# TengdaHan/CoCLR

Measured on AMD Instinct MI355X. Metric: clips/sec (whole node) S3D-InfoNCE seq_len=32 bs=32/GPU, higher is better.
Workload: dtype fp32

## Files before the change

### coclr_amd/_lib.py

```python
import ctypes as C
import os

_HERE = os.path.dirname(os.path.abspath(__file__))
LIB_PATH = os.environ.get("COCLR_LIB_PATH") or os.path.join(_HERE, "libcoclr_hip.so")
ABI_VERSION = 22

i32, i64, f32, f64, vp = C.c_int32, C.c_int64, C.c_float, C.c_double, C.c_void_p


class ConvDesc(C.Structure):
    _fields_ = [(n, i32) for n in (
        "N", "Cin", "Cout", "Ti", "Hi", "Wi", "To", "Ho", "Wo", "kt", "kh", "kw",
        "st", "sh", "sw", "pt", "ph", "pw", "dt", "dh", "dw")] + [
        ("x_nstride", i64), ("y_nstride", i64)] + [(n, i32) for n in (
        "ys_t", "ys_h", "ys_w", "yo_t", "yo_h", "yo_w", "yT", "yH", "yW", "Nx", "algo")]


class PoolDesc(C.Structure):
    _fields_ = [(n, i32) for n in (
        "N", "C", "Ti", "Hi", "Wi", "To", "Ho", "Wo", "kt", "kh", "kw",
        "st", "sh", "sw", "pt", "ph", "pw")] + [("x_nstride", i64), ("y_nstride", i64)]


class ConvCall(C.Structure):
    _fields_ = [("d", C.POINTER(ConvDesc)), ("x", vp), ("w_packed", vp), ("y", vp), ("stats", vp),
                ("bias", vp), ("ep_scale", vp), ("ep_shift", vp), ("n_index", vp), ("relu", i32),
                ("accumulate", i32), ("bwd_y", vp), ("bwd_scale", vp), ("bwd_shift", vp), ("bwd_mean", vp),
                ("bwd_invstd", vp), ("bwd_relu", i32), ("in_relu", i32), ("in_scale", vp), ("in_shift", vp)]


class BnFwdCall(C.Structure):
    _fields_ = [(n, vp) for n in ("sum", "sumsq", "gamma", "beta", "running_mean", "running_var",
                                  "num_batches_tracked", "mean", "invstd", "scale", "shift", "y", "z")] + [
        ("count", f64), ("S", i64), ("y_nstride", i64), ("z_nstride", i64), ("C", i32), ("ntiles", i32),
        ("N", i32), ("relu", i32), ("momentum", f32), ("eps", f32)]


class BnBwdCall(C.Structure):
    _fields_ = [(n, vp) for n in ("dz", "y", "scale", "shift", "mean", "invstd", "sums_ws", "dy", "dgamma",
                                  "dbeta")] + [
        ("S", i64), ("dz_nstride", i64), ("y_nstride", i64), ("dy_nstride", i64), ("N", i32), ("C", i32),
        ("relu", i32), ("training", i32), ("part", vp * 2), ("part_ntiles", i32 * 2)]


class GemmEpilogue(C.Structure):
    _fields_ = [("mode", i32), ("S", i32), ("a", vp), ("lda", i64), ("b", vp), ("y", vp), ("inv_norm", vp),
                ("out2", vp), ("f", f32), ("rowsum", vp)]


_P = C.POINTER
_SIGNATURES = {
    "coclr_abi_version": [],
    "coclr_conv_packed_size": [i32, i32, i32, i32, _P(i64)],
    "coclr_conv_pack_weights": [vp, vp, i32, i32, i32, i64, i64, i32, i32, i32, i32, i32, i32, i32, vp],
    "coclr_conv_pack_describe": [vp, vp, i32, i32, i32, i64, i64, i32, i32, i32, i32, i32, i32, i32,
                                 _P(i64), _P(i32)],
    "coclr_conv_pack_batch": [vp, vp, i32, vp],
    "coclr_conv3d_ntiles": [_P(ConvDesc), _P(i32)],
    "coclr_conv3d_bwd_sums_ok": [_P(ConvDesc), _P(i32)],
    "coclr_conv3d_fwd": [_P(ConvDesc), vp, vp, vp, vp, vp, vp, vp, vp, i32, i32, vp],
    "coclr_conv3d_fwd_multi": [_P(ConvCall), i32, vp],
    "coclr_conv3d_wgrad_workspace": [_P(ConvDesc), _P(i64)],
    "coclr_conv3d_wgrad": [_P(ConvDesc), vp, vp, vp, vp, i64, i64, i32, i32, vp],
    "coclr_conv3d_wgrad_multi": [_P(ConvDesc), vp, vp, vp, vp, i32, vp, i64, i64, i32, i32, vp],
    "coclr_conv3d_wgrad_bn_ok": [_P(ConvDesc), _P(i32)],
    "coclr_conv3d_wgrad_bn": [_P(ConvDesc), vp, vp, vp, i64, vp, i32, vp, vp, i64, i64, i32, i32, vp],
    "coclr_bn_finalize": [vp, vp, i32, i32, f64, vp, vp, vp, vp, vp, f32, f32, vp, vp, vp, vp, vp],
    "coclr_bn_finalize_apply": [vp, vp, i32, i32, f64, vp, vp, vp, vp, vp, f32, f32, vp, vp, vp, vp,
                                vp, vp, i32, i64, i64, i64, i32, vp],
    "coclr_bn_finalize_apply_multi": [_P(BnFwdCall), i32, vp],
    "coclr_bn_act_backward_multi": [_P(BnBwdCall), i32, vp],
    "coclr_bn_eval_affine": [vp, vp, vp, vp, f32, i32, vp, vp, vp, vp, vp],
    "coclr_bn_act_apply": [vp, vp, vp, vp, vp, i32, i32, i64, i64, i64, i64, i32, vp],
    "coclr_bn_backward_workspace": [i32, i32, _P(i64)],
    "coclr_bn_act_backward": [vp, vp, vp, vp, vp, vp, vp, vp, vp, vp, vp, vp, i32, i32, i64,
                              i64, i64, i64, i64, i64, i32, i32, i32, vp],
    "coclr_bn_act_backward_coeffs": [vp, vp, vp, vp, vp, vp, vp, vp, vp, vp, i32, i32, i64, i64, i64, i32,
                                     i32, vp],
    "coclr_maxpool3d_fwd": [_P(PoolDesc), vp, vp, vp, vp, vp, i32, vp],
    "coclr_maxpool3d_bwd": [_P(PoolDesc), vp, vp, vp, i64, i64, i32, vp],
    "coclr_bn_act_backward_pooled": [_P(PoolDesc), vp, vp, vp, vp, vp, vp, vp, vp, vp, vp, vp, i64, i64, i64,
                                     i32, i32, vp],
    "coclr_bn_act_backward_pooled_fits": [_P(PoolDesc), _P(i32)],
    "coclr_global_avgpool_fwd": [vp, vp, i64, i64, vp],
    "coclr_global_avgpool_bwd": [vp, vp, i64, i64, vp],
    "coclr_gemm_workspace": [i32, i32, i32, i32, _P(i64)],
    "coclr_gemm": [vp, i64, i64, vp, i64, i64, vp, i64, vp, i32, i32, i32, f32, i32, i32, i32, vp,
                   vp],
    "coclr_gemm_fused": [vp, i64, i64, vp, i64, i64, vp, i64, vp, i32, i32, i32, f32, i32, i32, vp,
                         _P(GemmEpilogue), vp],
    "coclr_l2norm_fwd": [vp, vp, vp, i32, i32, f32, vp],
    "coclr_l2norm_bwd": [vp, vp, vp, vp, i32, i32, vp],
    "coclr_nce_logits_fwd": [vp, vp, vp, vp, i32, i32, i32, f32, vp],
    "coclr_nce_logits_bwd": [vp, vp, vp, vp, vp, i32, i32, i32, f32, i32, vp],
    "coclr_momentum_update": [vp, i32, f32, f32, vp],
    "coclr_queue_enqueue": [vp, vp, i32, i32, i32, vp, vp],
    "coclr_queue_fill_i64": [vp, vp, i64, i32, i32, vp, vp],
    "coclr_queue_advance": [vp, i32, i32, vp],
    "coclr_positive_mask": [vp, vp, vp, vp, i32, i32, i32, vp],
    "coclr_mine_positives": [vp, vp, vp, vp, vp, vp, vp, vp, vp, i32, i32, i32, i32, vp],
    "coclr_gather_rows": [vp, vp, vp, i32, i64, i64, vp],
    "coclr_pull_rows": [vp, vp, i32, i64, vp],
    "coclr_relu_fwd": [vp, vp, i64, vp],
    "coclr_relu_bwd": [vp, vp, vp, i64, vp],
    "coclr_colsum": [vp, vp, i32, i32, vp],
    "coclr_sigmoid_fwd": [vp, vp, i64, vp],
    "coclr_sigmoid_bwd": [vp, vp, vp, i64, vp],
    "coclr_plane_scale": [vp, vp, vp, vp, i32, i32, i64, i64, i64, i32, vp],
    "coclr_plane_dot": [vp, vp, vp, i32, i32, i64, i64, i64, vp],
    "coclr_adam_step": [vp, i32, vp, vp, vp, i32, f32, f32, vp],
    "coclr_sgd_step": [vp, i32, vp, vp],
    "coclr_nce_loss_fwd": [vp, vp, vp, vp, vp, vp, i32, i32, i32, i32, i32, i32, vp],
    "coclr_nce_loss_bwd": [vp, vp, vp, vp, vp, vp, vp, i32, i32, i32, vp],
    "coclr_stage_clips": [vp, i32, vp, i32, i32, i32, i64, _P(f32), _P(f32), vp],
    "coclr_colstats_workspace": [i32, i32, _P(i64)],
    "coclr_bn1d_stats": [vp, vp, vp, i32, i32, vp],
    "coclr_center_rows": [vp, vp, vp, i32, i32, vp],
    "coclr_retrieval_hits": [vp, vp, vp, vp, i32, vp, vp, i32, i32, i32, vp],
    "coclr_segment_softmax_accum": [vp, _P(i32), _P(f32), vp, i32, i32, i32, i32, vp],
    "coclr_segment_accum": [vp, _P(i32), _P(f32), vp, i32, i32, i32, i32, vp],
}

EXPORTED_SYMBOLS = tuple(_SIGNATURES)

_lib = None


class HipLibraryError(RuntimeError):
    pass


def load():
    global _lib
    if _lib is not None:
        return _lib
    import torch
    if not os.path.exists(LIB_PATH):
        raise HipLibraryError(
            "coclr_amd: %s not found -- build it with `python -c 'import __graft_entry__ as g; "
            "g.build()'` (or coclr_amd/csrc/build.sh). There is no fallback path." % LIB_PATH)
    lib = C.CDLL(LIB_PATH)
    for name, argtypes in _SIGNATURES.items():
        fn = getattr(lib, name)
        fn.argtypes = argtypes
        fn.restype = C.c_int
    got = lib.coclr_abi_version()
    if got != ABI_VERSION:
        raise HipLibraryError("coclr_amd: ABI version mismatch (lib %d, python %d); rebuild" %
                              (got, ABI_VERSION))
    _lib = lib
    return lib


CALLS = [0]


def check(rc, what, detail=None):
    CALLS[0] += 1
    if rc != 0:
        if detail is not None:
            what = "%s %s" % (what, detail)
        raise HipLibraryError("coclr_amd: %s failed with hipError %d" % (what, rc))
```

### coclr_amd/backbone/s3dg.py

```python
import os

import torch
import torch.nn as nn

from .. import engine

_SPLIT_MODE = os.environ.get("COCLR_SPLIT_STAGES", "auto")


def _split_stages():
    if _SPLIT_MODE in ("0", "1"):
        return _SPLIT_MODE == "1"
    import torch.distributed as dist
    return dist.is_available() and dist.is_initialized() and dist.get_world_size() > 1


class _Emitter(nn.Module):

    def forward(self, x, **kw):
        return engine.run_module(self, x, **kw)


def _conv_bn(cin, cout, kernel, stride, padding):
    conv = nn.Conv3d(cin, cout, kernel_size=kernel, stride=stride, padding=padding, bias=False)
    bn = nn.BatchNorm3d(cout)
    return conv, bn


def _init_conv_bn(conv, bn):
    conv.weight.data.normal_(mean=0, std=0.01)
    bn.weight.data.fill_(1)
    bn.bias.data.zero_()


class BasicConv3d(_Emitter):

    def __init__(self, in_planes, out_planes, kernel_size, stride, padding=0):
        super().__init__()
        self.conv, self.bn = _conv_bn(in_planes, out_planes, kernel_size, stride, padding)
        self.relu = nn.ReLU(inplace=True)
        _init_conv_bn(self.conv, self.bn)

    def _emit(self, run, x, out=None, n_index=None):
        return engine.conv_bn_act(run, x, self.conv, self.bn, relu=True, out=out, n_index=n_index)

    def _emit_gen(self, run, x, out=None):
        return (yield from engine.conv_bn_act_gen(run, x, self.conv, self.bn, relu=True, out=out))


class STConv3d(_Emitter):

    def __init__(self, in_planes, out_planes, kernel_size, stride, padding=0):
        super().__init__()
        if isinstance(stride, tuple):
            t_stride, s_stride = stride[0], stride[-1]
        else:
            t_stride = s_stride = stride
        self.conv1 = nn.Conv3d(in_planes, out_planes, kernel_size=(1, kernel_size, kernel_size),
                               stride=(1, s_stride, s_stride), padding=(0, padding, padding),
                               bias=False)
        self.conv2 = nn.Conv3d(out_planes, out_planes, kernel_size=(kernel_size, 1, 1),
                               stride=(t_stride, 1, 1), padding=(padding, 0, 0), bias=False)
        self.bn1 = nn.BatchNorm3d(out_planes)
        self.bn2 = nn.BatchNorm3d(out_planes)
        self.relu = nn.ReLU(inplace=True)
        self.conv1.weight.data.normal_(mean=0, std=0.01)
        self.conv2.weight.data.normal_(mean=0, std=0.01)
        for bn in (self.bn1, self.bn2):
            bn.weight.data.fill_(1)
            bn.bias.data.zero_()

    def _emit(self, run, x, out=None, n_index=None):
        mid = engine.conv_bn_act(run, x, self.conv1, self.bn1, relu=True, n_index=n_index)
        return engine.conv_bn_act(run, mid, self.conv2, self.bn2, relu=True, out=out)

    def _emit_gen(self, run, x, out=None):
        mid = yield from engine.conv_bn_act_gen(run, x, self.conv1, self.bn1, relu=True)
        return (yield from engine.conv_bn_act_gen(run, mid, self.conv2, self.bn2, relu=True, out=out))


class SelfGating(_Emitter):
    def __init__(self, input_dim):
        super().__init__()
        self.fc = nn.Linear(input_dim, input_dim)

    def _emit(self, run, x, out=None):
        return engine.self_gating(run, x, self.fc, out=out)


class _Pool(nn.MaxPool3d):

    def forward(self, x):
        return engine.run_module(self, x)

    def _emit(self, run, x):
        return engine.max_pool(run, x, self.kernel_size, self.stride, self.padding)


class _Chain(nn.Sequential):

    def forward(self, x, **kw):
        return engine.run_module(self, x, **kw)

    def _emit(self, run, x, out=None, n_index=None):
        mods = list(self)
        for i, m in enumerate(mods):
            kw = {}
            if i == 0 and n_index is not None:
                kw["n_index"] = n_index
            if i == len(mods) - 1 and out is not None:
                kw["out"] = out
            x = m._emit(run, x, **kw)
        return x


class SepInception(_Emitter):

    def __init__(self, in_planes, out_planes, gating=False):
        super().__init__()
        assert isinstance(out_planes, list) and len(out_planes) == 6
        b0, b1a, b1b, b2a, b2b, b3b = out_planes
        self.branch0 = _Chain(BasicConv3d(in_planes, b0, kernel_size=1, stride=1))
        self.branch1 = _Chain(BasicConv3d(in_planes, b1a, kernel_size=1, stride=1),
                              STConv3d(b1a, b1b, kernel_size=3, stride=1, padding=1))
        self.branch2 = _Chain(BasicConv3d(in_planes, b2a, kernel_size=1, stride=1),
                              STConv3d(b2a, b2b, kernel_size=3, stride=1, padding=1))
        self.branch3 = _Chain(_Pool(kernel_size=(3, 3, 3), stride=1, padding=1),
                              BasicConv3d(in_planes, b3b, kernel_size=1, stride=1))
        self._widths = (b0, b1b, b2b, b3b)
        self.out_channels = sum(self._widths)
        self.gating = gating
        if gating:
            self.gating_b0 = SelfGating(b0)
            self.gating_b1 = SelfGating(b1b)
            self.gating_b2 = SelfGating(b2b)
            self.gating_b3 = SelfGating(b3b)

    def _emit(self, run, x):
        N, _, T, H, W = x.shape
        odim = (T, H, W)
        block = run.empty(N, self.out_channels, *odim)
        dst, c0 = [], 0
        for width in self._widths:
            dst.append(engine.Val(block, c0, width))
            c0 += width
        b0, b1a, b2a = self.branch0[0], self.branch1[0], self.branch2[0]
        head_units = [(b0.conv, b0.bn, None if self.gating else dst[0]), (b1a.conv, b1a.bn, None),
                      (b2a.conv, b2a.bn, None)]
        tails = (None, self.branch1[1], self.branch2[1])
        if engine.PAIR_UNITS and not self.gating:
            pooled = self.branch3[0]._emit(run, x)
            heads, _ = engine.drive_pair(run, engine.pointwise_group_gen(run, x, head_units),
                                         self.branch3[1]._emit_gen(run, pooled, out=dst[3]))
            engine.drive_pair(run, tails[1]._emit_gen(run, heads[1], out=dst[1]),
                              tails[2]._emit_gen(run, heads[2], out=dst[2]))
            return engine.Val(block)
        heads = engine.pointwise_group(run, x, head_units)
        if self.gating:
            getattr(self, "gating_b0")._emit(run, heads[0], out=dst[0])
        for i in (1, 2, 3):
            if i == 3:
                y = self.branch3._emit(run, x, out=None if self.gating else dst[3])
            else:
                y = tails[i]._emit(run, heads[i], out=None if self.gating else dst[i])
            if self.gating:
                getattr(self, "gating_b%d" % i)._emit(run, y, out=dst[i])
        return engine.Val(block)


_INCEPTION = {
    "Mixed_3b": (192, [64, 96, 128, 16, 32, 32]),
    "Mixed_3c": (256, [128, 128, 192, 32, 96, 64]),
    "Mixed_4b": (480, [192, 96, 208, 16, 48, 64]),
    "Mixed_4c": (512, [160, 112, 224, 24, 64, 64]),
    "Mixed_4d": (512, [128, 128, 256, 24, 64, 64]),
    "Mixed_4e": (512, [112, 144, 288, 32, 64, 64]),
    "Mixed_4f": (528, [256, 160, 320, 32, 128, 128]),
    "Mixed_5b": (832, [256, 160, 320, 32, 128, 128]),
    "Mixed_5c": (832, [384, 192, 384, 48, 128, 128]),
}


class S3D(_Emitter):
    def __init__(self, input_channel=3, gating=False, slow=False):
        super().__init__()
        self.gating = gating
        self.slow = slow

        stem_stride = (1, 2, 2) if slow else 2
        self.Conv_1a = STConv3d(input_channel, 64, kernel_size=7, stride=stem_stride, padding=3)
        self.block1 = _Chain(self.Conv_1a)

        self.MaxPool_2a = _Pool(kernel_size=(1, 3, 3), stride=(1, 2, 2), padding=(0, 1, 1))
        self.Conv_2b = BasicConv3d(64, 64, kernel_size=1, stride=1)
        self.Conv_2c = STConv3d(64, 192, kernel_size=3, stride=1, padding=1)
        self.block2 = _Chain(self.MaxPool_2a, self.Conv_2b, self.Conv_2c)

        self.MaxPool_3a = _Pool(kernel_size=(1, 3, 3), stride=(1, 2, 2), padding=(0, 1, 1))
        self._add_inceptions("Mixed_3b", "Mixed_3c")
        self.block3 = _Chain(self.MaxPool_3a, self.Mixed_3b, self.Mixed_3c)

        self.MaxPool_4a = _Pool(kernel_size=(3, 3, 3), stride=(2, 2, 2), padding=(1, 1, 1))
        self._add_inceptions("Mixed_4b", "Mixed_4c", "Mixed_4d", "Mixed_4e", "Mixed_4f")
        self.block4 = _Chain(self.MaxPool_4a, self.Mixed_4b, self.Mixed_4c, self.Mixed_4d,
                             self.Mixed_4e, self.Mixed_4f)

        self.MaxPool_5a = _Pool(kernel_size=(2, 2, 2), stride=(2, 2, 2), padding=(0, 0, 0))
        self._add_inceptions("Mixed_5b", "Mixed_5c")
        self.block5 = _Chain(self.MaxPool_5a, self.Mixed_5b, self.Mixed_5c)

    def _add_inceptions(self, *names):
        for name in names:
            cin, widths = _INCEPTION[name]
            setattr(self, name, SepInception(in_planes=cin, out_planes=list(widths),
                                             gating=self.gating))

    def _emit(self, run, x, n_index=None):
        x = self.block1._emit(run, x, n_index=n_index)
        for blk in (self.block2, self.block3, self.block4, self.block5):
            x = blk._emit(run, x)
        return x

    def _stage_groups(self):
        groups = self.__dict__.get("_coclr_groups")
        if groups is None:
            b2, b3, b4, b5 = list(self.block2), list(self.block3), list(self.block4), list(self.block5)
            groups = self.__dict__["_coclr_groups"] = [
                _Group(list(self.block1) + b2[:1]), _Group(b2[1:] + b3[:1]), _Group(b3[1:] + b4[:1]),
                _Group(b4[1:] + b5[:1]), _Group(b5[1:])]
            for grp in groups[1:]:
                grp.__dict__["_coclr_defer_join"] = True
        return groups

    def forward(self, x, n_index=None):
        if not (torch.is_grad_enabled() and _split_stages()):
            return engine.run_module(self, x, n_index=n_index) if n_index is not None \
                else engine.run_module(self, x)
        groups = self._stage_groups()
        x = engine.run_module(groups[0], x, n_index=n_index) if n_index is not None \
            else engine.run_module(groups[0], x)
        for grp in groups[1:]:
            x = engine.run_module(grp, x)
        return x


class _Group:

    def __init__(self, mods):
        self.mods = mods

    def parameters(self):
        for m in self.mods:
            yield from m.parameters()

    def modules(self):
        for m in self.mods:
            yield from m.modules()

    def _emit(self, run, x, n_index=None):
        for i, m in enumerate(self.mods):
            x = m._emit(run, x, n_index=n_index) if (i == 0 and n_index is not None) else m._emit(run, x)
        return x
```

### coclr_amd/csrc/bn.hip

```cpp
#include "common.h"
#include "../../include/coclr_hip.h"

namespace {


__global__ void __launch_bounds__(256)
bn_finalize_kernel(const float* __restrict__ sum, const float* __restrict__ sumsq, int C,
                   int ntiles, double count,
                   const float* __restrict__ gamma, const float* __restrict__ beta,
                   float* running_mean, float* running_var, int64_t* num_batches_tracked,
                   float momentum, float eps, float* mean_out, float* invstd_out,
                   float* scale_out, float* shift_out) {
  __shared__ double red[4];
  const int c = blockIdx.x;
  const float* ps = sum + (long)c * ntiles;
  const float* pq = sumsq + (long)c * ntiles;
  double s = 0.0, q = 0.0;
  for (int i = threadIdx.x; i < ntiles; i += 256) { s += (double)ps[i]; q += (double)pq[i]; }
  s = block256_sum_d(s, red);
  q = block256_sum_d(q, red);
  if (threadIdx.x == 0) {
    const double mean = s / count;
    double var = q / count - mean * mean;
    if (var < 0.0) var = 0.0;
    const float invstd = (float)(1.0 / sqrt(var + (double)eps));
    const float g = gamma ? gamma[c] : 1.f, b = beta ? beta[c] : 0.f;
    const float sc = g * invstd;
    mean_out[c] = (float)mean;
    invstd_out[c] = invstd;
    scale_out[c] = sc;
    shift_out[c] = b - (float)mean * sc;
    if (running_mean) {
      const double unbiased = count > 1.0 ? var * count / (count - 1.0) : var;
      running_mean[c] = (1.f - momentum) * running_mean[c] + momentum * (float)mean;
      running_var[c] = (1.f - momentum) * running_var[c] + momentum * (float)unbiased;
    }
    if (c == 0 && num_batches_tracked) *num_batches_tracked += 1;
  }
}

__global__ void bn_eval_affine_kernel(const float* __restrict__ gamma, const float* __restrict__ beta,
                                      const float* __restrict__ rm, const float* __restrict__ rv,
                                      float eps, int C, float* mean_out, float* invstd_out,
                                      float* scale_out, float* shift_out) {
  const int c = blockIdx.x * blockDim.x + threadIdx.x;
  if (c >= C) return;
  const float invstd = 1.f / sqrtf(rv[c] + eps);
  const float sc = gamma[c] * invstd;
  mean_out[c] = rm[c];
  invstd_out[c] = invstd;
  scale_out[c] = sc;
  shift_out[c] = beta[c] - rm[c] * sc;
}

typedef float nt_f32x4 __attribute__((ext_vector_type(4)));

inline long bn_nt_bytes() {
  const char* e = getenv("COCLR_BN_NT_MB");
  const long mb = e ? atol(e) : 0;
  return mb < 0 ? -1 : (mb << 20);
}

__device__ __forceinline__ float4 ld4(const float* p, int i, bool nt) {
  if (nt) {
    const nt_f32x4 t = __builtin_nontemporal_load(reinterpret_cast<const nt_f32x4*>(p) + i);
    return make_float4(t.x, t.y, t.z, t.w);
  }
  return reinterpret_cast<const float4*>(p)[i];
}
__device__ __forceinline__ void st4(float* p, int i, const float4& w, bool nt) {
  if (nt) {
    nt_f32x4 t; t.x = w.x; t.y = w.y; t.z = w.z; t.w = w.w;
    __builtin_nontemporal_store(t, reinterpret_cast<nt_f32x4*>(p) + i);
  } else {
    reinterpret_cast<float4*>(p)[i] = w;
  }
}

template <bool VEC, bool NT = false>
__global__ void __launch_bounds__(256)
bn_act_apply_kernel(const float* __restrict__ y, const float* __restrict__ scale,
                    const float* __restrict__ shift, const float* __restrict__ res, float* z,
                    int N, int C, int S, long y_nstride, long z_nstride, long res_nstride,
                    int relu) {
  const int c = blockIdx.y % C, sg = blockIdx.y / C, nsg = gridDim.y / C;
  const float sc = scale[c], sf = shift[c];
  for (int n = sg; n < N; n += nsg) {
    const float* yp = y + (long)n * y_nstride + (long)c * S;
    float* zp = z + (long)n * z_nstride + (long)c * S;
    const float* rp = res ? res + (long)n * res_nstride + (long)c * S : nullptr;
    if (VEC) {
      const int S4 = S >> 2, stride = gridDim.x * 256;
      for (int i0 = blockIdx.x * 256 + threadIdx.x; i0 < S4; i0 += 4 * stride) {
        float4 v[4], r[4];
#pragma unroll
        for (int k = 0; k < 4; ++k) {
          const int i = i0 + k * stride;
          if (i < S4) {
            if (NT) {
              const nt_f32x4 t = __builtin_nontemporal_load(reinterpret_cast<const nt_f32x4*>(yp) + i);
              v[k] = make_float4(t.x, t.y, t.z, t.w);
            } else {
              v[k] = reinterpret_cast<const float4*>(yp)[i];
            }
            if (rp) r[k] = reinterpret_cast<const float4*>(rp)[i];
          }
        }
#pragma unroll
        for (int k = 0; k < 4; ++k) {
          const int i = i0 + k * stride;
          if (i < S4) {
            float4 w = v[k];
            w.x = fmaf(w.x, sc, sf); w.y = fmaf(w.y, sc, sf);
            w.z = fmaf(w.z, sc, sf); w.w = fmaf(w.w, sc, sf);
            if (rp) { w.x += r[k].x; w.y += r[k].y; w.z += r[k].z; w.w += r[k].w; }
            if (relu) {
              w.x = fmaxf(w.x, 0.f); w.y = fmaxf(w.y, 0.f);
              w.z = fmaxf(w.z, 0.f); w.w = fmaxf(w.w, 0.f);
            }
            if (NT) {
              nt_f32x4 t; t.x = w.x; t.y = w.y; t.z = w.z; t.w = w.w;
              __builtin_nontemporal_store(t, reinterpret_cast<nt_f32x4*>(zp) + i);
            } else {
              reinterpret_cast<float4*>(zp)[i] = w;
            }
          }
        }
      }
    } else {
      for (int i = blockIdx.x * 256 + threadIdx.x; i < S; i += gridDim.x * 256) {
        float v = fmaf(yp[i], sc, sf);
        if (rp) v += rp[i];
        if (relu) v = fmaxf(v, 0.f);
        zp[i] = v;
      }
    }
  }
}


template <bool VEC>
__global__ void __launch_bounds__(256)
bn_act_bwd_reduce_kernel(const float* __restrict__ dz, const float* __restrict__ y,
                         const float* __restrict__ z, const float* __restrict__ scale,
                         const float* __restrict__ shift, const float* __restrict__ mean,
                         const float* __restrict__ invstd, double* sums, int N, int C, int S,
                         long dz_nstride, long y_nstride, long z_nstride, int relu_nt) {
  __shared__ double red[4];
  const int relu = relu_nt & 1;
  const bool nt = (relu_nt & 2) != 0;
  const int c = blockIdx.x;
  const float sc = scale[c], sf = shift[c], mu = mean[c], is = invstd[c];
  double sg = 0.0, sgx = 0.0;
  for (int n = blockIdx.y; n < N; n += gridDim.y) {
    const float* dzp = dz + (long)n * dz_nstride + (long)c * S;
    const float* yp = y + (long)n * y_nstride + (long)c * S;
    const float* zp = z ? z + (long)n * z_nstride + (long)c * S : nullptr;
    float ag = 0.f, agx = 0.f;
    if (VEC) {
      const int S4 = S >> 2;
      for (int i0 = threadIdx.x; i0 < S4; i0 += 512) {
        float4 dd[2], vv[2], zq[2];
        bool ok[2];
#pragma unroll
        for (int k = 0; k < 2; ++k) {
          const int i = i0 + k * 256;
          ok[k] = i < S4;
          if (ok[k]) {
            dd[k] = ld4(dzp, i, nt);
            vv[k] = ld4(yp, i, nt);
            if (relu && zp) zq[k] = reinterpret_cast<const float4*>(zp)[i];
          }
        }
#pragma unroll
        for (int k = 0; k < 2; ++k) {
          if (!ok[k]) continue;
          const float4 d = dd[k], v = vv[k];
          float g0 = d.x, g1 = d.y, g2 = d.z, g3 = d.w;
          if (relu) {
            if (zp) {
              const float4 zz = zq[k];
              g0 = zz.x > 0.f ? g0 : 0.f; g1 = zz.y > 0.f ? g1 : 0.f;
              g2 = zz.z > 0.f ? g2 : 0.f; g3 = zz.w > 0.f ? g3 : 0.f;
            } else {
              g0 = fmaf(v.x, sc, sf) > 0.f ? g0 : 0.f; g1 = fmaf(v.y, sc, sf) > 0.f ? g1 : 0.f;
              g2 = fmaf(v.z, sc, sf) > 0.f ? g2 : 0.f; g3 = fmaf(v.w, sc, sf) > 0.f ? g3 : 0.f;
            }
          }
          ag += (g0 + g1) + (g2 + g3);
          agx += g0 * ((v.x - mu) * is) + g1 * ((v.y - mu) * is) + g2 * ((v.z - mu) * is) +
                 g3 * ((v.w - mu) * is);
        }
      }
    } else {
      for (int i = threadIdx.x; i < S; i += 256) {
        float g = dzp[i];
        const float v = yp[i];
        if (relu) g = (zp ? zp[i] > 0.f : fmaf(v, sc, sf) > 0.f) ? g : 0.f;
        ag += g;
        agx += g * ((v - mu) * is);
      }
    }
    sg += (double)ag;
    sgx += (double)agx;
  }
  sg = block256_sum_d(sg, red);
  sgx = block256_sum_d(sgx, red);
  if (threadIdx.x == 0) {
    sums[((long)c * gridDim.y + blockIdx.y) * 2] = sg;
    sums[((long)c * gridDim.y + blockIdx.y) * 2 + 1] = sgx;
  }
}

__global__ void __launch_bounds__(256)
bn_bwd_fold_kernel(const float* __restrict__ p0, int n0, const float* __restrict__ p1, int n1, int C,
                   double* sums) {
  __shared__ double red[4];
  const int c = blockIdx.x;
  double sg = 0.0, sgx = 0.0;
  for (int i = threadIdx.x; i < n0; i += 256) {
    sg += (double)p0[(long)c * n0 + i];
    sgx += (double)p0[((long)C + c) * n0 + i];
  }
  if (p1)
    for (int i = threadIdx.x; i < n1; i += 256) {
      sg += (double)p1[(long)c * n1 + i];
      sgx += (double)p1[((long)C + c) * n1 + i];
    }
  sg = block256_sum_d(sg, red);
  sgx = block256_sum_d(sgx, red);
  if (threadIdx.x == 0) { sums[(long)c * 2] = sg; sums[(long)c * 2 + 1] = sgx; }
}

template <bool VEC>
__global__ void __launch_bounds__(256)
bn_act_bwd_apply_kernel(const float* __restrict__ dz, const float* __restrict__ y,
                        const float* __restrict__ z, const float* __restrict__ scale,
                        const float* __restrict__ shift, const float* __restrict__ mean,
                        const float* __restrict__ invstd, const double* __restrict__ sums,
                        int groups, double count, int training, float* dgamma, float* dbeta,
                        float* dy, float* dres, int N, int C, int S, long dz_nstride,
                        long y_nstride, long dy_nstride, long z_nstride, long dres_nstride,
                        int relu_nt, int dres_accumulate) {
  __shared__ double tot[2];
  const int relu = relu_nt & 1;
  const bool nt = (relu_nt & 2) != 0;
  const int c = blockIdx.y % C, sgrp = blockIdx.y / C, nsg = gridDim.y / C;
  if (threadIdx.x < 64) {
    double a0 = 0.0, a1 = 0.0;
    for (int g = threadIdx.x; g < groups; g += 64) {
      a0 += sums[((long)c * groups + g) * 2];
      a1 += sums[((long)c * groups + g) * 2 + 1];
    }
    a0 = wave_sum_d(a0);
    a1 = wave_sum_d(a1);
    if (threadIdx.x == 0) { tot[0] = a0; tot[1] = a1; }
  }
  __syncthreads();
  const double sg = tot[0], sgx = tot[1];
  const float sc = scale[c], sf = shift[c];
  float A = sc, B = 0.f, D = 0.f;
  if (training) {
    const float mg = (float)(sg / count), mgx = (float)(sgx / count);
    B = -sc * invstd[c] * mgx;
    D = sc * (mean[c] * invstd[c] * mgx - mg);
  }
  if (sgrp == 0 && blockIdx.x == 0 && threadIdx.x == 0) {
    if (dgamma) dgamma[c] = (float)sgx;
    if (dbeta) dbeta[c] = (float)sg;
  }
  for (int n = sgrp; n < N; n += nsg) {
    const float* dzp = dz + (long)n * dz_nstride + (long)c * S;
    const float* yp = y + (long)n * y_nstride + (long)c * S;
    const float* zp = z ? z + (long)n * z_nstride + (long)c * S : nullptr;
    float* dyp = dy + (long)n * dy_nstride + (long)c * S;
    float* drp = dres ? dres + (long)n * dres_nstride + (long)c * S : nullptr;
    if (VEC) {
      const int S4 = S >> 2, stride = gridDim.x * 256;
      for (int i0 = blockIdx.x * 256 + threadIdx.x; i0 < S4; i0 += 2 * stride) {
        float4 dd[2], vv[2], zq[2];
        bool ok[2];
#pragma unroll
        for (int k = 0; k < 2; ++k) {
          const int i = i0 + k * stride;
          ok[k] = i < S4;
          if (ok[k]) {
            dd[k] = ld4(dzp, i, nt);
            vv[k] = ld4(yp, i, nt);
            if (relu && zp) zq[k] = reinterpret_cast<const float4*>(zp)[i];
          }
        }
#pragma unroll
        for (int k = 0; k < 2; ++k) {
          if (!ok[k]) continue;
          const int i = i0 + k * stride;
          const float4 v = vv[k];
          float4 g = dd[k];
          if (relu) {
            if (zp) {
              const float4 zz = zq[k];
              g.x = zz.x > 0.f ? g.x : 0.f; g.y = zz.y > 0.f ? g.y : 0.f;
              g.z = zz.z > 0.f ? g.z : 0.f; g.w = zz.w > 0.f ? g.w : 0.f;
            } else {
              g.x = fmaf(v.x, sc, sf) > 0.f ? g.x : 0.f; g.y = fmaf(v.y, sc, sf) > 0.f ? g.y : 0.f;
              g.z = fmaf(v.z, sc, sf) > 0.f ? g.z : 0.f; g.w = fmaf(v.w, sc, sf) > 0.f ? g.w : 0.f;
            }
          }
          if (drp) {
            float4 r = g;
            if (dres_accumulate) {
              const float4 o = reinterpret_cast<const float4*>(drp)[i];
              r.x += o.x; r.y += o.y; r.z += o.z; r.w += o.w;
            }
            reinterpret_cast<float4*>(drp)[i] = r;
          }
          float4 o;
          o.x = fmaf(A, g.x, fmaf(B, v.x, D)); o.y = fmaf(A, g.y, fmaf(B, v.y, D));
          o.z = fmaf(A, g.z, fmaf(B, v.z, D)); o.w = fmaf(A, g.w, fmaf(B, v.w, D));
          st4(dyp, i, o, nt);
        }
      }
    } else {
      for (int i = blockIdx.x * 256 + threadIdx.x; i < S; i += gridDim.x * 256) {
        float g = dzp[i];
        const float v = yp[i];
        if (relu) g = (zp ? zp[i] > 0.f : fmaf(v, sc, sf) > 0.f) ? g : 0.f;
        if (drp) drp[i] = dres_accumulate ? drp[i] + g : g;
        dyp[i] = fmaf(A, g, fmaf(B, v, D));
      }
    }
  }
}

__global__ void __launch_bounds__(64)
bn_bwd_coeffs_kernel(const float* __restrict__ scale, const float* __restrict__ shift,
                     const float* __restrict__ mean, const float* __restrict__ invstd,
                     const double* __restrict__ sums, int groups, double count, int training, int C,
                     float* __restrict__ coef, float* dgamma, float* dbeta) {
  const int c = blockIdx.x;
  double a0 = 0.0, a1 = 0.0;
  for (int g = threadIdx.x; g < groups; g += 64) {
    a0 += sums[((long)c * groups + g) * 2];
    a1 += sums[((long)c * groups + g) * 2 + 1];
  }
  a0 = wave_sum_d(a0);
  a1 = wave_sum_d(a1);
  if (threadIdx.x != 0) return;
  const double sg = a0, sgx = a1;
  const float sc = scale[c];
  float A = sc, B = 0.f, D = 0.f;
  if (training) {
    const float mg = (float)(sg / count), mgx = (float)(sgx / count);
    B = -sc * invstd[c] * mgx;
    D = sc * (mean[c] * invstd[c] * mgx - mg);
  }
  coef[c] = A; coef[C + c] = B; coef[2 * C + c] = D; coef[3 * C + c] = sc; coef[4 * C + c] = shift[c];
  if (dgamma) dgamma[c] = (float)sgx;
  if (dbeta) dbeta[c] = (float)sg;
}


template <bool VEC>
__device__ __forceinline__ void
bn_fwd_fused_body(const int c, const float* __restrict__ sum, const float* __restrict__ sumsq, int ntiles,
                  double count, const float* __restrict__ gamma, const float* __restrict__ beta,
                  float* running_mean, float* running_var, int64_t* num_batches_tracked,
                  float momentum, float eps, float* mean_out, float* invstd_out, float* scale_out,
                  float* shift_out, const float* __restrict__ y, float* z, int N, int S,
                  long y_nstride, long z_nstride, int relu) {
  __shared__ double red[4];
  __shared__ float coef[2];
  const float* ps = sum + (long)c * ntiles;
  const float* pq = sumsq + (long)c * ntiles;
  double s = 0.0, q = 0.0;
  for (int i = threadIdx.x; i < ntiles; i += 256) { s += (double)ps[i]; q += (double)pq[i]; }
  s = block256_sum_d(s, red);
  q = block256_sum_d(q, red);
  if (threadIdx.x == 0) {
    const double mean = s / count;
    double var = q / count - mean * mean;
    if (var < 0.0) var = 0.0;
    const float invstd = (float)(1.0 / sqrt(var + (double)eps));
    const float g = gamma ? gamma[c] : 1.f, b = beta ? beta[c] : 0.f;
    const float sc = g * invstd, sf = b - (float)mean * sc;
    mean_out[c] = (float)mean;
    invstd_out[c] = invstd;
    scale_out[c] = sc;
    shift_out[c] = sf;
    coef[0] = sc; coef[1] = sf;
    if (running_mean) {
      const double unbiased = count > 1.0 ? var * count / (count - 1.0) : var;
      running_mean[c] = (1.f - momentum) * running_mean[c] + momentum * (float)mean;
      running_var[c] = (1.f - momentum) * running_var[c] + momentum * (float)unbiased;
    }
    if (c == 0 && num_batches_tracked) *num_batches_tracked += 1;
  }
  __syncthreads();
  const float sc = coef[0], sf = coef[1];
  if (VEC) {
    const int S4 = S >> 2, total = N * S4;
    for (int e0 = threadIdx.x; e0 < total; e0 += 1024) {
      float4 v[4];
      long zo[4];
#pragma unroll
      for (int k = 0; k < 4; ++k) {
        const int e = e0 + k * 256;
        zo[k] = -1;
        if (e < total) {
          const int n = e / S4, i = e - n * S4;
          v[k] = reinterpret_cast<const float4*>(y + (long)n * y_nstride + (long)c * S)[i];
          zo[k] = (long)n * z_nstride + (long)c * S + 4 * i;
        }
      }
#pragma unroll
      for (int k = 0; k < 4; ++k) {
        if (zo[k] < 0) continue;
        float4 w = v[k];
        w.x = fmaf(w.x, sc, sf); w.y = fmaf(w.y, sc, sf); w.z = fmaf(w.z, sc, sf); w.w = fmaf(w.w, sc, sf);
        if (relu) {
          w.x = fmaxf(w.x, 0.f); w.y = fmaxf(w.y, 0.f); w.z = fmaxf(w.z, 0.f); w.w = fmaxf(w.w, 0.f);
        }
        *reinterpret_cast<float4*>(z + zo[k]) = w;
      }
    }
  } else {
    const int total = N * S;
    for (int e = threadIdx.x; e < total; e += 256) {
      const int n = e / S, i = e - n * S;
      float v = fmaf(y[(long)n * y_nstride + (long)c * S + i], sc, sf);
      if (relu) v = fmaxf(v, 0.f);
      z[(long)n * z_nstride + (long)c * S + i] = v;
    }
  }
}

template <bool VEC>
__global__ void __launch_bounds__(256)
bn_fwd_fused_kernel(const float* __restrict__ sum, const float* __restrict__ sumsq, int ntiles,
                    double count, const float* __restrict__ gamma, const float* __restrict__ beta,
                    float* running_mean, float* running_var, int64_t* num_batches_tracked,
                    float momentum, float eps, float* mean_out, float* invstd_out, float* scale_out,
                    float* shift_out, const float* __restrict__ y, float* z, int N, int S,
                    long y_nstride, long z_nstride, int relu) {
  bn_fwd_fused_body<VEC>((int)blockIdx.x, sum, sumsq, ntiles, count, gamma, beta, running_mean, running_var,
                         num_batches_tracked, momentum, eps, mean_out, invstd_out, scale_out, shift_out, y,
                         z, N, S, y_nstride, z_nstride, relu);
}

struct BnFwdUnit {
  const float* sum; const float* sumsq; const float* gamma; const float* beta;
  float* running_mean; float* running_var; int64_t* nbt;
  float* mean; float* invstd; float* scale; float* shift;
  const float* y; float* z;
  double count;
  long y_nstride, z_nstride;
  int C, ntiles, N, S, relu;
  float momentum, eps;
};
struct BnFwdTable { BnFwdUnit u[4]; int n; };

template <bool VEC>
__global__ void __launch_bounds__(256)
bn_fwd_fused_multi_kernel(const BnFwdTable t) {
  int c = (int)blockIdx.x;
#define COCLR_BN_FWD_UNIT(k)                                                                              \
  if (k < t.n) {                                                                                         \
    if (c < t.u[k].C) {                                                                                  \
      bn_fwd_fused_body<VEC>(c, t.u[k].sum, t.u[k].sumsq, t.u[k].ntiles, t.u[k].count, t.u[k].gamma,     \
                             t.u[k].beta, t.u[k].running_mean, t.u[k].running_var, t.u[k].nbt,           \
                             t.u[k].momentum, t.u[k].eps, t.u[k].mean, t.u[k].invstd, t.u[k].scale,      \
                             t.u[k].shift, t.u[k].y, t.u[k].z, t.u[k].N, t.u[k].S, t.u[k].y_nstride,     \
                             t.u[k].z_nstride, t.u[k].relu);                                             \
      return;                                                                                            \
    }                                                                                                    \
    c -= t.u[k].C;                                                                                       \
  }
  COCLR_BN_FWD_UNIT(0)
  COCLR_BN_FWD_UNIT(1)
  COCLR_BN_FWD_UNIT(2)
  COCLR_BN_FWD_UNIT(3)
#undef COCLR_BN_FWD_UNIT
}

template <bool VEC>
__device__ __forceinline__ void
bn_bwd_fused_body(const int c, const float* __restrict__ dz, const float* __restrict__ y,
                  const float* __restrict__ scale, const float* __restrict__ shift,
                  const float* __restrict__ mean, const float* __restrict__ invstd, int training,
                  float* dgamma, float* dbeta, float* dy, int N, int S, long dz_nstride,
                  long y_nstride, long dy_nstride, int relu) {
  __shared__ double red[4];
  const float sc = scale[c], sf = shift[c], mu = mean[c], is = invstd[c];
  double sg = 0.0, sgx = 0.0;
  if (VEC) {
    const int S4 = S >> 2, total = N * S4;
    float ag = 0.f, agx = 0.f;
    for (int e0 = threadIdx.x; e0 < total; e0 += 1024) {
      float4 dd[4], vv[4];
#pragma unroll
      for (int k = 0; k < 4; ++k) {
        const int e = e0 + k * 256;
        if (e < total) {
          const int n = e / S4, i = e - n * S4;
          dd[k] = reinterpret_cast<const float4*>(dz + (long)n * dz_nstride + (long)c * S)[i];
          vv[k] = reinterpret_cast<const float4*>(y + (long)n * y_nstride + (long)c * S)[i];
        }
      }
#pragma unroll
      for (int k = 0; k < 4; ++k) {
        const int e = e0 + k * 256;
        if (e >= total) break;
        const float4 d = dd[k], v = vv[k];
        float g0 = d.x, g1 = d.y, g2 = d.z, g3 = d.w;
        if (relu) {
          g0 = fmaf(v.x, sc, sf) > 0.f ? g0 : 0.f; g1 = fmaf(v.y, sc, sf) > 0.f ? g1 : 0.f;
          g2 = fmaf(v.z, sc, sf) > 0.f ? g2 : 0.f; g3 = fmaf(v.w, sc, sf) > 0.f ? g3 : 0.f;
        }
        ag += (g0 + g1) + (g2 + g3);
        agx += g0 * ((v.x - mu) * is) + g1 * ((v.y - mu) * is) + g2 * ((v.z - mu) * is) +
               g3 * ((v.w - mu) * is);
        if ((e & 0xfff) == 0xfff) { sg += (double)ag; sgx += (double)agx; ag = agx = 0.f; }
      }
    }
    sg += (double)ag; sgx += (double)agx;
  } else {
    const int total = N * S;
    for (int e = threadIdx.x; e < total; e += 256) {
      const int n = e / S, i = e - n * S;
      float g = dz[(long)n * dz_nstride + (long)c * S + i];
      const float v = y[(long)n * y_nstride + (long)c * S + i];
      if (relu) g = fmaf(v, sc, sf) > 0.f ? g : 0.f;
      sg += (double)g;
      sgx += (double)(g * ((v - mu) * is));
    }
  }
  sg = block256_sum_d(sg, red);
  sgx = block256_sum_d(sgx, red);
  float A = sc, B = 0.f, D = 0.f;
  if (training) {
    const double count = (double)N * (double)S;
    const float mg = (float)(sg / count), mgx = (float)(sgx / count);
    B = -sc * is * mgx;
    D = sc * (mu * is * mgx - mg);
  }
  if (threadIdx.x == 0) {
    if (dgamma) dgamma[c] = (float)sgx;
    if (dbeta) dbeta[c] = (float)sg;
  }
  if (VEC) {
    const int S4 = S >> 2, total = N * S4;
    for (int e0 = threadIdx.x; e0 < total; e0 += 1024) {
      float4 dd[4], vv[4];
      long yo[4];
#pragma unroll
      for (int k = 0; k < 4; ++k) {
        const int e = e0 + k * 256;
        yo[k] = -1;
        if (e < total) {
          const int n = e / S4, i = e - n * S4;
          dd[k] = reinterpret_cast<const float4*>(dz + (long)n * dz_nstride + (long)c * S)[i];
          vv[k] = reinterpret_cast<const float4*>(y + (long)n * y_nstride + (long)c * S)[i];
          yo[k] = (long)n * dy_nstride + (long)c * S + 4 * i;
        }
      }
#pragma unroll
      for (int k = 0; k < 4; ++k) {
        if (yo[k] < 0) continue;
        const float4 v = vv[k];
        float4 g = dd[k];
        if (relu) {
          g.x = fmaf(v.x, sc, sf) > 0.f ? g.x : 0.f; g.y = fmaf(v.y, sc, sf) > 0.f ? g.y : 0.f;
          g.z = fmaf(v.z, sc, sf) > 0.f ? g.z : 0.f; g.w = fmaf(v.w, sc, sf) > 0.f ? g.w : 0.f;
        }
        float4 o;
        o.x = fmaf(A, g.x, fmaf(B, v.x, D)); o.y = fmaf(A, g.y, fmaf(B, v.y, D));
        o.z = fmaf(A, g.z, fmaf(B, v.z, D)); o.w = fmaf(A, g.w, fmaf(B, v.w, D));
        *reinterpret_cast<float4*>(dy + yo[k]) = o;
      }
    }
  } else {
    const int total = N * S;
    for (int e = threadIdx.x; e < total; e += 256) {
      const int n = e / S, i = e - n * S;
      float g = dz[(long)n * dz_nstride + (long)c * S + i];
      const float v = y[(long)n * y_nstride + (long)c * S + i];
      if (relu) g = fmaf(v, sc, sf) > 0.f ? g : 0.f;
      dy[(long)n * dy_nstride + (long)c * S + i] = fmaf(A, g, fmaf(B, v, D));
    }
  }
}

template <bool VEC>
__global__ void __launch_bounds__(256)
bn_bwd_fused_kernel(const float* __restrict__ dz, const float* __restrict__ y,
                    const float* __restrict__ scale, const float* __restrict__ shift,
                    const float* __restrict__ mean, const float* __restrict__ invstd, int training,
                    float* dgamma, float* dbeta, float* dy, int N, int S, long dz_nstride,
                    long y_nstride, long dy_nstride, int relu) {
  bn_bwd_fused_body<VEC>((int)blockIdx.x, dz, y, scale, shift, mean, invstd, training, dgamma, dbeta, dy, N, S,
                         dz_nstride, y_nstride, dy_nstride, relu);
}

struct BnBwdUnit {
  const float* dz; const float* y; const float* scale; const float* shift; const float* mean;
  const float* invstd;
  float* dgamma; float* dbeta; float* dy;
  long dz_nstride, y_nstride, dy_nstride;
  int C, N, S, relu, training;
};
struct BnBwdTable { BnBwdUnit u[4]; int n; };

template <bool VEC>
__global__ void __launch_bounds__(256)
bn_bwd_fused_multi_kernel(const BnBwdTable t) {
  int c = (int)blockIdx.x;
#define COCLR_BN_BWD_UNIT(k)                                                                              \
  if (k < t.n) {                                                                                         \
    if (c < t.u[k].C) {                                                                                  \
      bn_bwd_fused_body<VEC>(c, t.u[k].dz, t.u[k].y, t.u[k].scale, t.u[k].shift, t.u[k].mean,            \
                             t.u[k].invstd, t.u[k].training, t.u[k].dgamma, t.u[k].dbeta, t.u[k].dy,     \
                             t.u[k].N, t.u[k].S, t.u[k].dz_nstride, t.u[k].y_nstride,                    \
                             t.u[k].dy_nstride, t.u[k].relu);                                            \
      return;                                                                                            \
    }                                                                                                    \
    c -= t.u[k].C;                                                                                       \
  }
  COCLR_BN_BWD_UNIT(0)
  COCLR_BN_BWD_UNIT(1)
  COCLR_BN_BWD_UNIT(2)
  COCLR_BN_BWD_UNIT(3)
#undef COCLR_BN_BWD_UNIT
}

constexpr long kSmallChannel = 32768;

inline dim3 plane_grid(int N, int C, int S) {
  int gx = cdiv(S >> 2 ? S >> 2 : S, 256 * 4);
  if (gx < 1) gx = 1;
  if (gx > 64) gx = 64;
  int nsg = N;
  if (S < 4096) {
    const long per = 4096 / S;
    nsg = cdiv(N, per);
  }
  if ((long)nsg * C > 65535) nsg = 65535 / C;
  if (nsg < 1) nsg = 1;
  while ((long)gx * nsg * C > 262144 && gx > 1) gx >>= 1;
  return dim3(gx, nsg * C);
}

inline int reduce_groups(int N, int S) {
  if (S >= 4096) return N;
  int g = cdiv(N, 4096 / S);
  return g < 1 ? 1 : g;
}

}

extern "C" int coclr_bn_finalize(const float* sum, const float* sumsq, int C, int ntiles,
                                 double count, const float* gamma, const float* beta,
                                 float* running_mean, float* running_var,
                                 int64_t* num_batches_tracked, float momentum, float eps, float* mean,
                                 float* invstd, float* scale, float* shift, void* stream) {
  if (C <= 0 || ntiles <= 0) return COCLR_EINVAL;
  hipLaunchKernelGGL(bn_finalize_kernel, dim3(C), dim3(256), 0, (hipStream_t)stream, sum, sumsq, C,
                     ntiles, count, gamma, beta, running_mean, running_var, num_batches_tracked,
                     momentum, eps, mean, invstd, scale, shift);
  COCLR_LAUNCH_CHECK();
  return 0;
}

extern "C" int coclr_bn_finalize_apply(const float* sum, const float* sumsq, int C, int ntiles,
                                       double count, const float* gamma, const float* beta,
                                       float* running_mean, float* running_var,
                                       int64_t* num_batches_tracked, float momentum, float eps,
                                       float* mean, float* invstd, float* scale, float* shift,
                                       const float* y, float* z, int N, int64_t S, int64_t y_nstride,
                                       int64_t z_nstride, int relu, void* stream_) {
  hipStream_t stream = (hipStream_t)stream_;
  if (C <= 0 || ntiles <= 0 || N <= 0 || S <= 0 || !y || !z) return COCLR_EINVAL;
  if ((long)N * S > kSmallChannel) {
    int rc = coclr_bn_finalize(sum, sumsq, C, ntiles, count, gamma, beta, running_mean, running_var,
                               num_batches_tracked, momentum, eps, mean, invstd, scale, shift, stream_);
    if (rc) return rc;
    return coclr_bn_act_apply(y, scale, shift, nullptr, z, N, C, S, y_nstride, z_nstride, 0, relu,
                              stream_);
  }
  const bool vec = (S % 4 == 0) && (y_nstride % 4 == 0) && (z_nstride % 4 == 0);
  if (vec)
    hipLaunchKernelGGL(bn_fwd_fused_kernel<true>, dim3(C), dim3(256), 0, stream, sum, sumsq, ntiles,
                       count, gamma, beta, running_mean, running_var, num_batches_tracked, momentum,
                       eps, mean, invstd, scale, shift, y, z, N, (int)S, (long)y_nstride,
                       (long)z_nstride, relu);
  else
    hipLaunchKernelGGL(bn_fwd_fused_kernel<false>, dim3(C), dim3(256), 0, stream, sum, sumsq, ntiles,
                       count, gamma, beta, running_mean, running_var, num_batches_tracked, momentum,
                       eps, mean, invstd, scale, shift, y, z, N, (int)S, (long)y_nstride,
                       (long)z_nstride, relu);
  COCLR_LAUNCH_CHECK();
  return 0;
}

extern "C" int coclr_bn_finalize_apply_multi(const coclr_bn_fwd_call* calls, int n, void* stream_) {
  hipStream_t stream = (hipStream_t)stream_;
  if (!calls || n < 1) return COCLR_EINVAL;
  const char* env = getenv("COCLR_PAIR");
  const bool fuse = !(env && env[0] == '0');
  int i = 0;
  while (i < n) {
    BnFwdTable t;
    t.n = 0;
    long blocks = 0;
    bool vec0 = false;
    int j = i;
    for (; j < n && t.n < 4; ++j) {
      const coclr_bn_fwd_call& c = calls[j];
      if (c.C <= 0 || c.ntiles <= 0 || c.N <= 0 || c.S <= 0 || !c.y || !c.z) return COCLR_EINVAL;
      const bool small = (long)c.N * c.S <= kSmallChannel;
      const bool vec = (c.S % 4 == 0) && (c.y_nstride % 4 == 0) && (c.z_nstride % 4 == 0);
      if (!small || !fuse) break;
      if (t.n == 0) vec0 = vec;
      else if (vec != vec0) break;
      BnFwdUnit& u = t.u[t.n++];
      u.sum = c.sum; u.sumsq = c.sumsq; u.gamma = c.gamma; u.beta = c.beta;
      u.running_mean = c.running_mean; u.running_var = c.running_var; u.nbt = c.num_batches_tracked;
      u.mean = c.mean; u.invstd = c.invstd; u.scale = c.scale; u.shift = c.shift;
      u.y = c.y; u.z = c.z; u.count = c.count;
      u.y_nstride = (long)c.y_nstride; u.z_nstride = (long)c.z_nstride;
      u.C = c.C; u.ntiles = c.ntiles; u.N = c.N; u.S = (int)c.S; u.relu = c.relu;
      u.momentum = c.momentum; u.eps = c.eps;
      blocks += c.C;
    }
    if (t.n >= 2) {
      if (vec0)
        hipLaunchKernelGGL(bn_fwd_fused_multi_kernel<true>, dim3((unsigned)blocks), dim3(256), 0, stream, t);
      else
        hipLaunchKernelGGL(bn_fwd_fused_multi_kernel<false>, dim3((unsigned)blocks), dim3(256), 0, stream, t);
      COCLR_LAUNCH_CHECK();
      i = j;
      continue;
    }
    const coclr_bn_fwd_call& c = calls[i];
    int rc = coclr_bn_finalize_apply(c.sum, c.sumsq, c.C, c.ntiles, c.count, c.gamma, c.beta,
                                     c.running_mean, c.running_var, c.num_batches_tracked, c.momentum,
                                     c.eps, c.mean, c.invstd, c.scale, c.shift, c.y, c.z, c.N, c.S,
                                     c.y_nstride, c.z_nstride, c.relu, stream_);
    if (rc) return rc;
    ++i;
  }
  return 0;
}

extern "C" int coclr_bn_eval_affine(const float* gamma, const float* beta, const float* running_mean,
                                    const float* running_var, float eps, int C, float* mean,
                                    float* invstd, float* scale, float* shift, void* stream) {
  if (C <= 0) return COCLR_EINVAL;
  hipLaunchKernelGGL(bn_eval_affine_kernel, dim3(cdiv(C, 256)), dim3(256), 0, (hipStream_t)stream,
                     gamma, beta, running_mean, running_var, eps, C, mean, invstd, scale, shift);
  COCLR_LAUNCH_CHECK();
  return 0;
}

extern "C" int coclr_bn_act_apply(const float* y, const float* scale, const float* shift,
                                  const float* residual, float* z, int N, int C, int64_t S,
                                  int64_t y_nstride, int64_t z_nstride, int64_t res_nstride,
                                  int relu, void* stream) {
  if (N <= 0 || C <= 0 || S <= 0) return COCLR_EINVAL;
  const bool vec = (S % 4 == 0) && (y_nstride % 4 == 0) && (z_nstride % 4 == 0) &&
                   (!residual || res_nstride % 4 == 0);
  dim3 grid = plane_grid(N, C, (int)S);
  static const long nt_bytes = bn_nt_bytes();
  if (vec && nt_bytes >= 0 && (long)N * C * S * 4 >= nt_bytes)
    hipLaunchKernelGGL((bn_act_apply_kernel<true, true>), grid, dim3(256), 0, (hipStream_t)stream, y, scale,
                       shift, residual, z, N, C, (int)S, (long)y_nstride, (long)z_nstride,
                       (long)res_nstride, relu);
  else if (vec)
    hipLaunchKernelGGL(bn_act_apply_kernel<true>, grid, dim3(256), 0, (hipStream_t)stream, y, scale,
                       shift, residual, z, N, C, (int)S, (long)y_nstride, (long)z_nstride,
                       (long)res_nstride, relu);
  else
    hipLaunchKernelGGL(bn_act_apply_kernel<false>, grid, dim3(256), 0, (hipStream_t)stream, y, scale,
                       shift, residual, z, N, C, (int)S, (long)y_nstride, (long)z_nstride,
                       (long)res_nstride, relu);
  COCLR_LAUNCH_CHECK();
  return 0;
}

extern "C" int coclr_bn_backward_workspace(int N, int C, int64_t* doubles) {
  if (N <= 0 || C <= 0) return COCLR_EINVAL;
  *doubles = (int64_t)2 * C * N;
  return 0;
}

extern "C" int coclr_bn_act_backward(const float* dz, const float* y, const float* z,
                                     const float* scale, const float* shift, const float* mean,
                                     const float* invstd, double* sums_ws, float* dy, float* dres,
                                     float* dgamma, float* dbeta, int N, int C, int64_t S,
                                     int64_t dz_nstride, int64_t y_nstride, int64_t dy_nstride,
                                     int64_t z_nstride, int64_t dres_nstride, int relu,
                                     int training, int dres_accumulate, void* stream_) {
  hipStream_t stream = (hipStream_t)stream_;
  if (N <= 0 || C <= 0 || S <= 0) return COCLR_EINVAL;
  const bool vec = (S % 4 == 0) && (dz_nstride % 4 == 0) && (y_nstride % 4 == 0) &&
                   (dy_nstride % 4 == 0) && (!z || z_nstride % 4 == 0) &&
                   (!dres || dres_nstride % 4 == 0);
  if (!z && !dres && (long)N * S <= kSmallChannel) {
    if (vec)
      hipLaunchKernelGGL(bn_bwd_fused_kernel<true>, dim3(C), dim3(256), 0, stream, dz, y, scale, shift,
                         mean, invstd, training, dgamma, dbeta, dy, N, (int)S, (long)dz_nstride,
                         (long)y_nstride, (long)dy_nstride, relu);
    else
      hipLaunchKernelGGL(bn_bwd_fused_kernel<false>, dim3(C), dim3(256), 0, stream, dz, y, scale,
                         shift, mean, invstd, training, dgamma, dbeta, dy, N, (int)S,
                         (long)dz_nstride, (long)y_nstride, (long)dy_nstride, relu);
    COCLR_LAUNCH_CHECK();
    return 0;
  }
  static const long nt_bytes_b = bn_nt_bytes();
  relu = relu ? 1 : 0;
  if (nt_bytes_b >= 0 && vec && (long)N * C * S * 4 >= nt_bytes_b) relu |= 2;
  const int groups = reduce_groups(N, (int)S);
  dim3 rgrid(C, groups);
  if (vec)
    hipLaunchKernelGGL(bn_act_bwd_reduce_kernel<true>, rgrid, dim3(256), 0, stream, dz, y, z, scale,
                       shift, mean, invstd, sums_ws, N, C, (int)S, (long)dz_nstride,
                       (long)y_nstride, (long)z_nstride, relu);
  else
    hipLaunchKernelGGL(bn_act_bwd_reduce_kernel<false>, rgrid, dim3(256), 0, stream, dz, y, z,
                       scale, shift, mean, invstd, sums_ws, N, C, (int)S, (long)dz_nstride,
                       (long)y_nstride, (long)z_nstride, relu);
  COCLR_LAUNCH_CHECK();
  const double count = (double)N * (double)S;
  dim3 grid = plane_grid(N, C, (int)S);
  if (vec)
    hipLaunchKernelGGL(bn_act_bwd_apply_kernel<true>, grid, dim3(256), 0, stream, dz, y, z, scale,
                       shift, mean, invstd, sums_ws, groups, count, training, dgamma, dbeta, dy, dres,
                       N, C, (int)S, (long)dz_nstride, (long)y_nstride, (long)dy_nstride,
                       (long)z_nstride, (long)dres_nstride, relu, dres_accumulate);
  else
    hipLaunchKernelGGL(bn_act_bwd_apply_kernel<false>, grid, dim3(256), 0, stream, dz, y, z, scale,
                       shift, mean, invstd, sums_ws, groups, count, training, dgamma, dbeta, dy, dres,
                       N, C, (int)S, (long)dz_nstride, (long)y_nstride, (long)dy_nstride,
                       (long)z_nstride, (long)dres_nstride, relu, dres_accumulate);
  COCLR_LAUNCH_CHECK();
  return 0;
}

extern "C" int coclr_bn_act_backward_coeffs(const float* dz, const float* y, const float* scale,
                                            const float* shift, const float* mean, const float* invstd,
                                            double* sums_ws, float* coef, float* dgamma, float* dbeta,
                                            int N, int C, int64_t S, int64_t dz_nstride, int64_t y_nstride,
                                            int relu, int training, void* stream_) {
  hipStream_t stream = (hipStream_t)stream_;
  if (N <= 0 || C <= 0 || S <= 0 || !coef || !sums_ws) return COCLR_EINVAL;
  const bool vec = (S % 4 == 0) && (dz_nstride % 4 == 0) && (y_nstride % 4 == 0);
  static const long nt_bytes_c = bn_nt_bytes();
  relu = relu ? 1 : 0;
  if (nt_bytes_c >= 0 && vec && (long)N * C * S * 4 >= nt_bytes_c) relu |= 2;
  const int groups = reduce_groups(N, (int)S);
  dim3 rgrid(C, groups);
  const float* noz = nullptr;
  if (vec)
    hipLaunchKernelGGL(bn_act_bwd_reduce_kernel<true>, rgrid, dim3(256), 0, stream, dz, y, noz, scale,
                       shift, mean, invstd, sums_ws, N, C, (int)S, (long)dz_nstride, (long)y_nstride, 0L,
                       relu);
  else
    hipLaunchKernelGGL(bn_act_bwd_reduce_kernel<false>, rgrid, dim3(256), 0, stream, dz, y, noz, scale,
                       shift, mean, invstd, sums_ws, N, C, (int)S, (long)dz_nstride, (long)y_nstride, 0L,
                       relu);
  COCLR_LAUNCH_CHECK();
  hipLaunchKernelGGL(bn_bwd_coeffs_kernel, dim3(C), dim3(64), 0, stream, scale, shift, mean, invstd, sums_ws,
                     groups, (double)N * (double)S, training, C, coef, dgamma, dbeta);
  COCLR_LAUNCH_CHECK();
  return 0;
}

namespace {
int bn_backward_from_partials(const coclr_bn_bwd_call& c, hipStream_t stream) {
  if (!c.sums_ws || c.part_ntiles[0] <= 0 || (c.part[1] && c.part_ntiles[1] <= 0)) return COCLR_EINVAL;
  hipLaunchKernelGGL(bn_bwd_fold_kernel, dim3(c.C), dim3(256), 0, stream, c.part[0], c.part_ntiles[0],
                     c.part[1], c.part[1] ? c.part_ntiles[1] : 0, c.C, c.sums_ws);
  COCLR_LAUNCH_CHECK();
  const bool vec = (c.S % 4 == 0) && (c.dz_nstride % 4 == 0) && (c.y_nstride % 4 == 0) &&
                   (c.dy_nstride % 4 == 0);
  const double count = (double)c.N * (double)c.S;
  dim3 grid = plane_grid(c.N, c.C, (int)c.S);
  const float* nof = nullptr;
  float* nod = nullptr;
  if (vec)
    hipLaunchKernelGGL(bn_act_bwd_apply_kernel<true>, grid, dim3(256), 0, stream, c.dz, c.y, nof, c.scale,
                       c.shift, c.mean, c.invstd, c.sums_ws, 1, count, c.training, c.dgamma, c.dbeta, c.dy, nod,
                       c.N, c.C, (int)c.S, (long)c.dz_nstride, (long)c.y_nstride, (long)c.dy_nstride, 0L, 0L,
                       c.relu, 0);
  else
    hipLaunchKernelGGL(bn_act_bwd_apply_kernel<false>, grid, dim3(256), 0, stream, c.dz, c.y, nof, c.scale,
                       c.shift, c.mean, c.invstd, c.sums_ws, 1, count, c.training, c.dgamma, c.dbeta, c.dy, nod,
                       c.N, c.C, (int)c.S, (long)c.dz_nstride, (long)c.y_nstride, (long)c.dy_nstride, 0L, 0L,
                       c.relu, 0);
  COCLR_LAUNCH_CHECK();
  return 0;
}
}

extern "C" int coclr_bn_act_backward_multi(const coclr_bn_bwd_call* calls, int n, void* stream_) {
  hipStream_t stream = (hipStream_t)stream_;
  if (!calls || n < 1) return COCLR_EINVAL;
  const char* env = getenv("COCLR_PAIR");
  const bool fuse = !(env && env[0] == '0');
  int i = 0;
  while (i < n) {
    BnBwdTable t;
    t.n = 0;
    long blocks = 0;
    bool vec0 = false;
    int j = i;
    for (; j < n && t.n < 4; ++j) {
      const coclr_bn_bwd_call& c = calls[j];
      if (c.N <= 0 || c.C <= 0 || c.S <= 0 || !c.dz || !c.y || !c.dy) return COCLR_EINVAL;
      const bool small = (long)c.N * c.S <= kSmallChannel;
      const bool vec = (c.S % 4 == 0) && (c.dz_nstride % 4 == 0) && (c.y_nstride % 4 == 0) &&
                       (c.dy_nstride % 4 == 0);
      if (!small || !fuse || c.part[0]) break;
      if (t.n == 0) vec0 = vec;
      else if (vec != vec0) break;
      BnBwdUnit& u = t.u[t.n++];
      u.dz = c.dz; u.y = c.y; u.scale = c.scale; u.shift = c.shift; u.mean = c.mean; u.invstd = c.invstd;
      u.dgamma = c.dgamma; u.dbeta = c.dbeta; u.dy = c.dy;
      u.dz_nstride = (long)c.dz_nstride; u.y_nstride = (long)c.y_nstride; u.dy_nstride = (long)c.dy_nstride;
      u.C = c.C; u.N = c.N; u.S = (int)c.S; u.relu = c.relu; u.training = c.training;
      blocks += c.C;
    }
    if (t.n >= 2) {
      if (vec0)
        hipLaunchKernelGGL(bn_bwd_fused_multi_kernel<true>, dim3((unsigned)blocks), dim3(256), 0, stream, t);
      else
        hipLaunchKernelGGL(bn_bwd_fused_multi_kernel<false>, dim3((unsigned)blocks), dim3(256), 0, stream, t);
      COCLR_LAUNCH_CHECK();
      i = j;
      continue;
    }
    const coclr_bn_bwd_call& c = calls[i];
    if (c.part[0]) {
      int rc = bn_backward_from_partials(c, stream);
      if (rc) return rc;
      ++i;
      continue;
    }
    int rc = coclr_bn_act_backward(c.dz, c.y, nullptr, c.scale, c.shift, c.mean, c.invstd, c.sums_ws, c.dy,
                                   nullptr, c.dgamma, c.dbeta, c.N, c.C, c.S, c.dz_nstride, c.y_nstride,
                                   c.dy_nstride, 0, 0, c.relu, c.training, 0, stream_);
    if (rc) return rc;
    ++i;
  }
  return 0;
}
```

### coclr_amd/engine.py

```python
import os
import weakref

import torch

from . import ops
from . import plan as _plan


_PACK_STORE = {}
BATCH_PACK = os.environ.get("COCLR_BATCH_PACK", "1") != "0"
WGRAD_STREAM = os.environ.get("COCLR_WGRAD_STREAM", "1") != "0"
DECISION_PROBE = None


def _probe_relu(bn, y, scale, shift, residual=None):
    sh = (1, -1, 1, 1, 1)
    z = torch.addcmul(shift.double().view(sh), y.double(), scale.double().view(sh)).float()
    if residual is not None:
        z = z + residual
    DECISION_PROBE("relu", bn, z > 0)


_SIDE = {}
_PENDING_SIDE = {}
DEFER_JOIN = os.environ.get("COCLR_DEFER_JOIN", "1") != "0"
DEFERRED = [0]
_SIDE_EVENTS = {}
_CALLBACK_QUEUED = {}


def _note(fn):
    fn()
    if _plan._ACTIVE is not None:
        rec = _plan.active()
        if rec is not None:
            rec.py(fn)


def side_stream_of(device):
    return _SIDE.get(device)


def side_events_for(params):
    evs = []
    for p in params:
        ev = _SIDE_EVENTS.pop(id(p), None)
        if ev is not None and not any(ev is e for e in evs):
            evs.append(ev)
    return evs


def _end_of_backward(device):
    _CALLBACK_QUEUED[device] = False
    _PENDING_SIDE.pop(device, None)
    if device in _SIDE:
        torch.cuda.current_stream(device).wait_stream(_SIDE[device])


_SIDE_PRIORITY = int(os.environ.get("COCLR_WGRAD_PRIORITY", "-1"))
_SIDE_WINDOW = int(os.environ.get("COCLR_SIDE_WINDOW", "12"))


_GRAD_SLOTS = {}
_SLOTS_VERIFIED = set()


def set_grad_slot(param, view):
    _SLOTS_VERIFIED.discard(id(param))
    if view is None:
        _GRAD_SLOTS.pop(id(param), None)
        return
    _GRAD_SLOTS[id(param)] = (weakref.ref(param), view)
    if len(_GRAD_SLOTS) > 8192:
        for k_ in [k_ for k_, v_ in _GRAD_SLOTS.items() if v_[0]() is None]:
            del _GRAD_SLOTS[k_]


_HEAD_SLOTS_OUT = set()


def new_pass(device):
    _CALLBACK_QUEUED[device] = False
    _HEAD_SLOTS_OUT.clear()


def grad_out_for(p):
    slot = _GRAD_SLOTS.get(id(p)) if _GRAD_SLOTS else None
    if slot is not None and slot[0]() is p and p.grad is None and id(p) not in _HEAD_SLOTS_OUT:
        v = slot[1]
        if v.device == p.device and v.shape == p.shape and v.dtype == p.dtype:
            _HEAD_SLOTS_OUT.add(id(p))
            return v.view_as(v)
    return torch.empty_like(p)


class PackPlan:

    def __init__(self):
        self.requests = {}
        self.table = None
        self.blockmap = None
        self.dirty = False

    def note(self, key, args, kw):
        if key not in self.requests:
            self.requests[key] = (args, kw)
            self.dirty = True

    def reset(self):
        self.requests.clear()
        self.table = self.blockmap = None
        self.dirty = False

    def build(self, device):
        rows, bmap = [], []
        self._ptrs = []
        for i, (args, kw) in enumerate(self.requests.values()):
            row, nb = ops.conv_pack_describe(*args, **kw)
            rows.append(row)
            bmap.extend((i, b) for b in range(nb))
            self._ptrs.append((args[0], args[0].data_ptr(), args[1], args[1].data_ptr()))
        self.table = torch.tensor(rows, dtype=torch.int64).to(device)
        self.blockmap = torch.tensor(bmap, dtype=torch.int32).to(device)
        self.dirty = False

    def launch(self, device):
        if not self.requests:
            return False
        capturing = device.type == "cuda" and torch.cuda.is_current_stream_capturing()
        if self.dirty or self.table is None:
            if capturing:
                return False
            self.build(device)
        for w, wp, buf, bp in self._ptrs:
            if w.data_ptr() != wp or buf.data_ptr() != bp:
                self.reset()
                return False
        ops.conv_pack_batch(self.table, self.blockmap, list(self.requests.values()))
        return True


def _stream_key(device):
    if device.type != "cuda":
        return 0
    return torch.cuda.current_stream(device).cuda_stream


def _plan_for(module, save, device):
    if not BATCH_PACK:
        return None
    plans = module.__dict__.get("_coclr_packplans")
    if plans is None:
        plans = module.__dict__["_coclr_packplans"] = {}
    stream = _stream_key(device)
    key = (bool(save), stream, device)
    plan = plans.get(key)
    if plan is None:
        plan = plans[key] = PackPlan()
    return plan


class Val:
    __slots__ = ("base", "c0", "C", "lazy")

    def __init__(self, base, c0=0, C=None):
        self.base = base
        self.c0 = c0
        self.C = base.shape[1] - c0 if C is None else C
        self.lazy = None

    @property
    def whole(self):
        return self.c0 == 0 and self.C == self.base.shape[1]

    def view(self):
        v = self.base if self.whole else self.base[:, self.c0:self.c0 + self.C]
        if self.lazy is not None:
            if self.lazy == "consumed":
                raise RuntimeError("coclr_amd: activation was consumed in fused form (its tensor "
                                   "was never written) and cannot be read again")
            y, scale, shift, relu = self.lazy
            self.lazy = None
            ops.bn_act_apply(y, scale, shift, None, v, relu)
        return v

    @property
    def shape(self):
        b = self.base.shape
        return (b[0], self.C, b[2], b[3], b[4])


def _triple(v):
    return tuple(v) if isinstance(v, (tuple, list)) else (v, v, v)


class Run:

    def __init__(self, device, save, need_input_grad=False):
        self.device = device
        self.save = save
        self.need_input_grad = need_input_grad
        self.tape = []
        self.pooled = {}
        self.bn_src = {}
        self.bn_parts = {}
        self.grad_writes = {}
        self.grads = {}
        self.param_grads = {}
        self._slots_out = set()
        self.no_grad_bases = set()
        self.out = None
        self.plan = None
        self.batched = False
        self._side_used = False
        self._side_keep = []
        self._side_windows = []
        self._side_calls = 0
        if device.type == "cuda" and device.index is not None and \
                device.index != torch.cuda.current_device():
            raise RuntimeError("coclr_amd: tensors live on %s but the current device is cuda:%d; "
                               "call torch.cuda.set_device first" % (device, torch.cuda.current_device()))

    def begin(self, module):
        self.plan = _plan_for(module, self.save, self.device)
        if self.plan is not None:
            self.batched = self.plan.launch(self.device)

    def empty(self, *shape, dtype=torch.float32):
        return torch.empty(shape, dtype=dtype, device=self.device)

    def needs_grad(self, val):
        return self.save and id(val.base) not in self.no_grad_bases

    def grad_target(self, val):
        if not val.whole:
            raise RuntimeError("coclr_amd: gradient into a channel slice is not supported")
        self.grad_writes[id(val.base)] = self.grad_writes.get(id(val.base), 0) + 1
        g = self.grads.get(id(val.base))
        if g is None:
            g = torch.empty_like(val.base)
            self.grads[id(val.base)] = g
            return g, False
        return g, True

    def grad_of(self, val):
        g = self.grads.get(id(val.base))
        if g is None:
            raise RuntimeError("coclr_amd: activation has no gradient (unused output?)")
        return g if val.whole else g[:, val.c0:val.c0 + val.C]

    def grad_out(self, p):
        slot = _GRAD_SLOTS.get(id(p)) if _GRAD_SLOTS else None
        if slot is not None and slot[0]() is p and p.grad is None and id(p) not in self.param_grads \
                and id(p) not in self._slots_out:
            v = slot[1]
            if v.device == p.device and v.shape == p.shape and v.dtype == p.dtype:
                self._slots_out.add(id(p))
                return v.view_as(v)
        return torch.empty_like(p)

    def add_param_grad(self, p, g):
        old = self.param_grads.get(id(p))
        if old is not None and _plan._ACTIVE is not None and _plan.active() is not None:
            _plan.active().taint("a parameter used twice in one pass (its gradients are added by an ATen launch)")
        self.param_grads[id(p)] = g if old is None else old.add_(g)

    def record(self, fn):
        self.tape.append(fn)

    def backward(self, dout, defer_join=False):
        out = self.out
        self.grads[id(out.base)] = dout.contiguous()
        while self.tape:
            _run_closure(self.tape.pop(), self)
        if defer_join and self._side_used and self.param_grads and \
                all(k in self._slots_out and k in _SLOTS_VERIFIED for k in self.param_grads):
            self.defer_side()
        else:
            self.join_side()
        return self.grads

    def side_stream(self, *inputs):
        if not (WGRAD_STREAM and self.device.type == "cuda"):
            return None
        st = _SIDE.get(self.device)
        if st is None:
            st = _SIDE[self.device] = torch.cuda.Stream(device=self.device, priority=_SIDE_PRIORITY)
        cur = torch.cuda.current_stream(self.device)
        _note(lambda st=st, cur=cur: st.wait_stream(cur))
        self._side_calls += 1
        if _SIDE_WINDOW and self._side_calls % _SIDE_WINDOW == 0 and self._side_keep and \
                not torch.cuda.is_current_stream_capturing() and \
                not (_plan._ACTIVE is not None and _plan.active() is not None):
            ev = torch.cuda.Event()
            ev.record(st)
            self._side_windows.append((ev, self._side_keep))
            self._side_keep = []
            while self._side_windows and self._side_windows[0][0].query():
                self._side_windows.pop(0)
        self._side_keep.extend(inputs)
        self._side_used = True
        return st

    def join_side(self):
        pending = _PENDING_SIDE.get(self.device)
        if self._side_used or pending:
            dev, keys = self.device, tuple(self.param_grads)

            def join(dev=dev, keys=keys):
                _PENDING_SIDE.pop(dev, None)
                torch.cuda.current_stream(dev).wait_stream(_SIDE[dev])
                if _SIDE_EVENTS:
                    for k in keys:
                        _SIDE_EVENTS.pop(k, None)
            _note(join)
            self._side_used = False
        elif _SIDE_EVENTS:
            for k in self.param_grads:
                _SIDE_EVENTS.pop(k, None)
        self._side_keep = []
        self._side_windows = []

    def defer_side(self):
        keep = _PENDING_SIDE.setdefault(self.device, [])
        keep.extend(self._side_keep)
        for _, ts in self._side_windows:
            keep.extend(ts)
        self._side_keep = []
        self._side_windows = []
        self._side_used = False
        dev, keys = self.device, tuple(self.param_grads)

        def publish(dev=dev, keys=keys):
            DEFERRED[0] += 1
            ev = torch.cuda.Event()
            ev.record(_SIDE[dev])
            for k in keys:
                _SIDE_EVENTS[k] = ev
            if not _CALLBACK_QUEUED.get(dev):
                _CALLBACK_QUEUED[dev] = True
                torch.autograd.Variable._execution_engine.queue_callback(lambda: _end_of_backward(dev))
        _note(publish)

    def _packed_buffer(self, owner, tag, n, zero):
        store = _PACK_STORE.get(id(owner))
        if store is None or store[0]() is not owner:
            store = _PACK_STORE[id(owner)] = (weakref.ref(owner), {})
            if len(_PACK_STORE) > 4096:
                for k_ in [k_ for k_, v_ in _PACK_STORE.items() if v_[0]() is None]:
                    del _PACK_STORE[k_]
        key = (tag, n, _stream_key(self.device), self.device)
        buf = store[1].get(key)
        if buf is None:
            buf = (torch.zeros if zero else torch.empty)(n, dtype=torch.float32, device=self.device)
            store[1][key] = buf
        return buf

    def pack(self, w, transpose, kt_slice=None, taps=None, tap_base=0, tap_step=1, algo=0):
        cout, cin, kt, kh, kw = w.shape
        if algo >= 1 and taps is not None:
            vt = {3: 6, 4: 5}[taps]
            n = ops.conv_packed_size(cin, cout, vt, transpose)
            packed = self._packed_buffer(w, ("wino", bool(transpose), vt, tap_base, tap_step), n, False)
            self._relayout(w, packed, (cout, cin, vt, cin * kt * kh * kw, kt * kh * kw, tap_base,
                                       int(bool(transpose)) | 2, tap_step), {})
            return packed
        if algo >= 1:
            vt = (6 if algo == 2 else 4) if kt == 3 else (9 if kt == 7 else 16)
            n = ops.conv_packed_size(cin, cout, vt, transpose)
            packed = self._packed_buffer(w, ("wino", bool(transpose), vt), n, False)
            self._relayout(w, packed, (cout, cin, vt, cin * kt * kh * kw, kt * kh * kw, 0,
                                       int(bool(transpose)) | 2, 1), {})
            return packed
        if taps is not None:
            base = tap_base
        elif kt_slice is None:
            taps, base = kt * kh * kw, 0
        else:
            taps, base = kh * kw, kt_slice * kh * kw
        n = ops.conv_packed_size(cin, cout, taps, transpose)
        packed = self._packed_buffer(w, (bool(transpose), taps, base, tap_step), n, False)
        self._relayout(w, packed, (cout, cin, taps, cin * kt * kh * kw, kt * kh * kw, base,
                                   int(bool(transpose)), tap_step), {})
        return packed

    def pack_concat(self, weights, transpose):
        cin = weights[0].shape[1]
        ctot = sum(w.shape[0] for w in weights)
        n = ops.conv_packed_size(cin, ctot, 1, transpose)
        packed = self._packed_buffer(weights[0], ("cat", bool(transpose), ctot), n, True)
        c0 = 0
        for w in weights:
            cout = w.shape[0]
            if transpose:
                self._relayout(w, packed, (cout, cin, 1, cin, 1, 0, 1, 1),
                               dict(row0=c0, rows_total=ctot, col0=0, cols_total=cin))
            else:
                self._relayout(w, packed, (cout, cin, 1, cin, 1, 0, 0, 1),
                               dict(row0=0, rows_total=cin, col0=c0, cols_total=ctot))
            c0 += cout
        return packed

    def _relayout(self, w, packed, args, kw):
        plan = self.plan
        if plan is not None:
            key = (id(w), packed.data_ptr(), args, tuple(sorted(kw.items())))
            if self.batched and key in plan.requests:
                return
            plan.note(key, (w, packed) + args, kw)
        ops.conv_pack_weights(w, packed, *args, **kw)



_SLICED = {}


def _sliced_geoms(N, Cin, Cout, idim, k, s, p):
    key = (N, Cin, Cout, tuple(idim), k, s, p)
    g = _SLICED.get(key)
    if g is None:
        odim = ops.ConvGeom(N, Cin, Cout, idim, k, s, p).odim
        g = _SLICED[key] = [ops.ConvGeom(N, Cin, Cout, idim, (1, k[1], k[2]), s,
                                         (p[0] - t, p[1], p[2]), odim=odim) for t in range(k[0])]
    return g


def _is_plain_pointwise(k, s):
    return k == (1, 1, 1) and s != (1, 1, 1)


PAIR_UNITS = os.environ.get("COCLR_PAIR_UNITS", "1") != "0"


def _exec(req):
    kind, c = req
    if kind == "conv":
        stats = nt = None
        if c.get("want_stats"):
            nt = c["geom"].ntiles()
            stats = torch.empty(2 * c["geom"].Cout * nt, dtype=torch.float32, device=c["y"].device)
        if c.get("bwd_bn") is not None or c.get("in_affine") is not None:
            c["stats"] = stats
            ops.conv_fwd_multi([c])
        else:
            ops.conv_fwd(c["geom"], c["x"], c["w"], c["y"], stats=stats, n_index=c.get("n_index"),
                         accumulate=c.get("accumulate", False))
        return stats, nt
    if kind == "bn_fwd":
        if len(c) > 1:
            ops.bn_finalize_apply_multi(c)
            return None
        u = c[0]
        gamma, beta, rm, rv, nbt, momentum, eps = u["bn"]
        mean, invstd, scale, shift = u["small"]
        ops.bn_finalize_apply(u["stats"], u["C"], u["ntiles"], u["count"], gamma, beta, rm, rv, nbt, momentum,
                              eps, mean, invstd, scale, shift, u["y"], u["z"], u["relu"], c0=u.get("c0", 0),
                              c_total=u.get("c_total"))
        return None
    if kind == "bn_bwd":
        if len(c) > 1:
            ops.bn_act_backward_multi(c)
            return None
        u = c[0]
        if u.get("partials"):
            ops.bn_act_backward_multi(c)
            return None
        ops.bn_act_backward(u["dz"], u["y"], None, u["scale"], u["shift"], u["mean"], u["invstd"], u["sums"],
                            u["dy"], None, u["dgamma"], u["dbeta"], u["relu"], u["training"])
        return None
    raise RuntimeError("coclr_amd: unknown launch request %r" % (kind,))


def _exec_pair(ra, rb):
    kind = ra[0]
    if kind != rb[0]:
        return _exec(ra), _exec(rb)
    ca, cb = ra[1], rb[1]
    if kind == "conv":
        res = [(None, None), (None, None)]
        for i, c in enumerate((ca, cb)):
            if c.get("want_stats"):
                nt = c["geom"].ntiles()
                c["stats"] = torch.empty(2 * c["geom"].Cout * nt, dtype=torch.float32, device=c["y"].device)
                res[i] = (c["stats"], nt)
        ops.conv_fwd_multi([ca, cb])
        return res[0], res[1]
    if kind == "bn_fwd":
        ops.bn_finalize_apply_multi(list(ca) + list(cb))
        return None, None
    if kind == "bn_bwd":
        ops.bn_act_backward_multi(list(ca) + list(cb))
        return None, None
    return _exec(ra), _exec(rb)


def _drive(gen):
    try:
        req = next(gen)
        while True:
            req = gen.send(_exec(req))
    except StopIteration as e:
        return e.value


def _run_closure(fn, run):
    r = fn(run)
    if r is not None and hasattr(r, "send"):
        _drive(r)


class _PairedBackward:
    __slots__ = ("fa", "fb")

    def __init__(self, fa, fb):
        self.fa, self.fb = fa, fb

    def __call__(self, run):
        ga, gb = self.fa(run), self.fb(run)
        ga = ga if ga is not None and hasattr(ga, "send") else None
        gb = gb if gb is not None and hasattr(gb, "send") else None
        if ga is not None and gb is not None:
            drive_pair(run, ga, gb)
        else:
            for g in (ga, gb):
                if g is not None:
                    _drive(g)


def drive_pair(run, ga, gb):
    main_tape = run.tape
    tapes = ([], [])
    gens = [ga, gb]
    reqs, vals, done = [None, None], [None, None], [False, False]

    def advance(i, first, value=None):
        run.tape = tapes[i]
        try:
            reqs[i] = next(gens[i]) if first else gens[i].send(value)
        except StopIteration as e:
            done[i], vals[i], reqs[i] = True, e.value, None
        finally:
            run.tape = main_tape

    advance(0, True)
    advance(1, True)
    while not (done[0] and done[1]):
        if not done[0] and not done[1]:
            ra, rb = _exec_pair(reqs[0], reqs[1])
            advance(0, False, ra)
            advance(1, False, rb)
        else:
            i = 0 if not done[0] else 1
            advance(i, False, _exec(reqs[i]))
    ta, tb = tapes
    n = min(len(ta), len(tb))
    main_tape.extend(_PairedBackward(fa, fb) for fa, fb in zip(ta, tb))
    main_tape.extend(ta[n:] + tb[n:])
    return vals[0], vals[1]


def conv_bn_act(run, x, conv, bn, relu=True, out=None, residual=None, n_index=None):
    return _drive(conv_bn_act_gen(run, x, conv, bn, relu=relu, out=out, residual=residual, n_index=n_index))


def conv_bn_act_gen(run, x, conv, bn, relu=True, out=None, residual=None, n_index=None):
    w = conv.weight
    k = tuple(w.shape[2:])
    s, p = _triple(conv.stride), _triple(conv.padding)
    if conv.bias is not None or _triple(conv.dilation) != (1, 1, 1) or conv.groups != 1:
        raise NotImplementedError("coclr_amd: backbone convs are bias-free, dense, undilated")
    if _is_plain_pointwise(k, s):
        x = subsample(run, x, s)
        s = (1, 1, 1)
    N = n_index.shape[0] if n_index is not None else x.shape[0]
    Cin, idim = x.shape[1], x.shape[2:]
    Cout = w.shape[0]
    if w.shape[1] != Cin:
        raise ValueError("coclr_amd: conv expects %d input channels, got %d" % (w.shape[1], Cin))
    training = bn.training or (bn.running_mean is None)

    sliced = k[0] > 3 and k[1] > 1
    if sliced:
        geoms = _sliced_geoms(N, Cin, Cout, idim, k, s, p)
    else:
        geoms = [ops.conv_geom(N, Cin, Cout, idim, k, s, p)]
        if n_index is not None and geoms[0].algo and k[1] > 1:
            geoms = [ops.ConvGeom(N, Cin, Cout, idim, k, s, p)]
    in_affine = None
    if IN_AFFINE and x.lazy is not None and x.lazy != "consumed" and x.whole and not run.save and \
            n_index is None and not sliced and want_in_affine(geoms[0], training or run.save):
        ysrc, sc_in, sh_in, relu_in = x.lazy
        x.lazy = "consumed"
        xv, in_affine = ysrc, (sc_in, sh_in, relu_in)
    else:
        xv = x.view()
    odim = geoms[0].odim
    want_y = training or run.save or residual is not None

    small = run.empty(4, Cout)
    mean, invstd, scale, shift = small[0], small[1], small[2], small[3]
    lazy_ok = out is None
    if out is None:
        out = Val(run.empty(N, Cout, *odim))
    zv = out.base if out.whole else out.view()
    y = None
    if want_y:
        y = run.empty(N, Cout, *odim)
        stats = ntiles = None
        for t, g in enumerate(geoms):
            last = t == len(geoms) - 1
            res = yield ("conv", dict(geom=g, x=xv, w=run.pack(w, False, t if sliced else None, algo=g.algo),
                                      y=y, want_stats=training and last, n_index=n_index, accumulate=t > 0,
                                      in_affine=in_affine))
            if training and last:
                stats, ntiles = res
        count = N * odim[0] * odim[1] * odim[2]
        lazy = LAZY_APPLY and residual is None and lazy_ok and count > ops.SMALL_CHANNEL
        if training:
            if bn.momentum is None:
                raise NotImplementedError("coclr_amd: cumulative-average BatchNorm momentum")
            if residual is None and not lazy:
                yield ("bn_fwd", [dict(stats=stats, C=Cout, ntiles=ntiles, count=count,
                                       bn=(bn.weight, bn.bias, bn.running_mean, bn.running_var,
                                           bn.num_batches_tracked, float(bn.momentum), float(bn.eps)),
                                       small=(mean, invstd, scale, shift), y=y, z=zv, relu=relu)])
            else:
                ops.bn_finalize(stats, Cout, ntiles, count, bn.weight, bn.bias,
                                bn.running_mean, bn.running_var, bn.num_batches_tracked,
                                float(bn.momentum), float(bn.eps), mean, invstd, scale, shift)
        else:
            ops.bn_eval_affine(bn.weight, bn.bias, bn.running_mean, bn.running_var, float(bn.eps),
                               Cout, mean, invstd, scale, shift)
        if lazy:
            out.lazy = (y, scale, shift, relu)
        elif not (training and residual is None):
            ops.bn_act_apply(y, scale, shift, residual.view() if residual is not None else None, zv,
                             relu)
    else:
        ops.bn_eval_affine(bn.weight, bn.bias, bn.running_mean, bn.running_var, float(bn.eps),
                           Cout, mean, invstd, scale, shift)
        for t, g in enumerate(geoms):
            last = t == len(geoms) - 1
            ops.conv_fwd(g, xv, run.pack(w, False, t if sliced else None, algo=g.algo), zv,
                         ep_scale=scale if last else None, ep_shift=shift if last else None,
                         relu=relu and last, n_index=n_index, accumulate=t > 0)

    if run.save and DECISION_PROBE is not None and relu:
        _probe_relu(bn, y, scale, shift, residual.view() if residual is not None else None)

    if run.save:
        x_needs = run.needs_grad(x)
        if n_index is not None and x_needs:
            raise NotImplementedError("coclr_amd: gathered conv input cannot require grad")
        if FUSE_BN_REDUCE and training and residual is None and out.whole and \
                N * odim[0] * odim[1] * odim[2] > ops.SMALL_CHANNEL:
            run.bn_src[id(out.base)] = (y, scale, shift, mean, invstd, relu)

        def backward(run):
            dgb = (run.grad_out(bn.weight), run.grad_out(bn.bias))
            sums = run.empty(ops.bn_backward_workspace(N, Cout), dtype=torch.float64)
            pooled = run.pooled.pop(id(out.base), None)
            fused = WGRAD_BN and pooled is None and residual is None and not x_needs and not sliced and \
                w.requires_grad and id(out.base) not in run.bn_parts and geoms[0].wgrad_bn_ok()
            dy = None if fused else torch.empty_like(y)
            if fused:
                coef = run.empty(5, Cout)
                dz = run.grad_of(out)
                ops.bn_act_backward_coeffs(dz, y, scale, shift, mean, invstd, sums, coef, dgb[0], dgb[1], relu,
                                           training)
            elif pooled is not None:
                ops.bn_act_backward_pooled(pooled[0], pooled[1], pooled[2], y, scale, shift, mean,
                                           invstd, sums, dy, dgb[0], dgb[1], relu, training)
            elif residual is None:
                parts = run.bn_parts.pop(id(out.base), None)
                if parts is not None and run.grad_writes.get(id(out.base), 0) != 1:
                    parts = None
                yield ("bn_bwd", [dict(dz=run.grad_of(out), y=y, scale=scale, shift=shift, mean=mean,
                                       invstd=invstd, sums=sums, dy=dy, dgamma=dgb[0], dbeta=dgb[1], relu=relu,
                                       training=training, partials=parts)])
            else:
                dz = run.grad_of(out)
                dres = None
                dres_acc = False
                if run.needs_grad(residual):
                    dres, dres_acc = run.grad_target(residual)
                ops.bn_act_backward(dz, y, zv, scale, shift, mean, invstd, sums, dy, dres, dgb[0], dgb[1],
                                    relu, training, dres_acc)
            if bn.weight.requires_grad:
                run.add_param_grad(bn.weight, dgb[0])
            if bn.bias.requires_grad:
                run.add_param_grad(bn.bias, dgb[1])
            if fused:
                with torch.cuda.stream(run.side_stream(dz, y, coef, xv)):
                    dw = run.grad_out(w)
                    kk = w.shape[2] * w.shape[3] * w.shape[4]
                    ops.conv_wgrad_bn(geoms[0], xv, dz, y, coef, relu, dw, run.empty(geoms[0].wgrad_workspace()),
                                      Cin * kk, kk)
                run.add_param_grad(w, dw)
            elif w.requires_grad:
                with torch.cuda.stream(run.side_stream(dy, xv)):
                    dw = run.grad_out(w)
                    kk = w.shape[2] * w.shape[3] * w.shape[4]
                    for t, g in enumerate(geoms):
                        ws = run.empty(g.wgrad_workspace())
                        ops.conv_wgrad(g, xv, dy, dw, ws, Cin * kk, kk,
                                       t * k[1] * k[2] if sliced else 0)
                run.add_param_grad(w, dw)
            if x_needs:
                if sliced:
                    raise NotImplementedError("coclr_amd: dgrad of the sliced stem conv")
                dx, acc = run.grad_target(x)
                src = run.bn_src.get(id(x.base)) if (not acc and x.whole) else None
                phases = geoms[0].dgrad_phases()
                if phases is not None:
                    if src is not None and not (len(phases) <= 2 and all(ph[0].bwd_sums_ok() for ph in phases)):
                        src = None
                    for pg, k0, nk, step in phases:
                        wp = run.pack(w, True, taps=nk, tap_base=k0, tap_step=step, algo=pg.algo)
                        if src is not None:
                            nt = pg.ntiles()
                            st = torch.empty(2 * pg.Cout * nt, dtype=torch.float32, device=dx.device)
                            ops.conv_fwd_multi([dict(geom=pg, x=dy, w=wp, y=dx, stats=st, bwd_bn=src)])
                            run.bn_parts.setdefault(id(x.base), []).append((st, nt))
                        else:
                            ops.conv_fwd(pg, dy, wp, dx, accumulate=acc)
                else:
                    dg = geoms[0].dgrad()
                    if src is not None and not dg.bwd_sums_ok():
                        src = None
                    res = yield ("conv", dict(geom=dg, x=dy, w=run.pack(w, True, algo=dg.algo), y=dx,
                                              accumulate=acc, want_stats=src is not None, bwd_bn=src))
                    if src is not None:
                        run.bn_parts.setdefault(id(x.base), []).append(res)

        run.record(backward)
    elif y is not None:
        del y
    return out


LAZY_APPLY = os.environ.get("COCLR_LAZY_APPLY", "1") != "0"
WGRAD_BN = os.environ.get("COCLR_WGRAD_BN", "1") != "0"
IN_AFFINE = os.environ.get("COCLR_IN_AFFINE", "1") != "0"


def want_in_affine(geom, keeps_y):
    return keeps_y and geom.k == (7, 1, 1) and geom.algo == 1
FUSE_BN_REDUCE = os.environ.get("COCLR_FUSE_BN_REDUCE", "0") != "0"
POOLED_BACKWARD = os.environ.get("COCLR_POOLED_BACKWARD", "1") != "0"
FUSE_POINTWISE = True


def pointwise_group(run, x, units):
    return _drive(pointwise_group_gen(run, x, units))


def pointwise_group_gen(run, x, units):
    training = all(bn.training or bn.running_mean is None for _, bn, _ in units)
    if not (training or run.save) or len(units) == 1 or not FUSE_POINTWISE:
        res = []
        for conv, bn, out in units:
            res.append((yield from conv_bn_act_gen(run, x, conv, bn, relu=True, out=out)))
        return res
    for conv, bn, _ in units:
        if tuple(conv.weight.shape[2:]) != (1, 1, 1) or _triple(conv.stride) != (1, 1, 1) or \
                _triple(conv.padding) != (0, 0, 0) or conv.bias is not None or \
                (bn.training or bn.running_mean is None) != training:
            raise NotImplementedError("coclr_amd: pointwise_group takes plain 1x1x1 conv units")
    N, Cin, idim = x.shape[0], x.shape[1], x.shape[2:]
    widths = [conv.weight.shape[0] for conv, _, _ in units]
    Ccat = sum(widths)
    weights = [conv.weight for conv, _, _ in units]
    geom = ops.conv_geom(N, Cin, Ccat, idim, (1, 1, 1), (1, 1, 1), (0, 0, 0))
    xv = x.view()
    y = run.empty(N, Ccat, *idim)
    ntiles = geom.ntiles()
    stats, _ = yield ("conv", dict(geom=geom, x=xv, w=run.pack_concat(weights, False), y=y,
                                   want_stats=training))
    count = N * idim[0] * idim[1] * idim[2]
    outs, saved = [], []
    c0 = 0
    fwd_units = []
    for (conv, bn, out), C_ in zip(units, widths):
        small = run.empty(4, C_)
        mean, invstd, scale, shift = small[0], small[1], small[2], small[3]
        if training:
            if bn.momentum is None:
                raise NotImplementedError("coclr_amd: cumulative-average BatchNorm momentum")
            if out is None:
                out = Val(run.empty(N, C_, *idim))
            fwd_units.append(dict(stats=stats, C=C_, ntiles=ntiles, count=count,
                                  bn=(bn.weight, bn.bias, bn.running_mean, bn.running_var,
                                      bn.num_batches_tracked, float(bn.momentum), float(bn.eps)),
                                  small=(mean, invstd, scale, shift), y=y[:, c0:c0 + C_], z=out.view(),
                                  relu=True, c0=c0, c_total=Ccat))
        else:
            ops.bn_eval_affine(bn.weight, bn.bias, bn.running_mean, bn.running_var, float(bn.eps),
                               C_, mean, invstd, scale, shift)
            if out is None:
                out = Val(run.empty(N, C_, *idim))
            ops.bn_act_apply(y[:, c0:c0 + C_], scale, shift, None, out.view(), True)
        outs.append(out)
        saved.append((c0, C_, mean, invstd, scale, shift))
        c0 += C_
    if fwd_units:
        yield ("bn_fwd", fwd_units)
    if run.save and DECISION_PROBE is not None:
        for (conv, bn, _), (c0_, C_, mean, invstd, scale, shift) in zip(units, saved):
            _probe_relu(bn, y[:, c0_:c0_ + C_], scale, shift)

    if run.save:
        x_needs = run.needs_grad(x)

        def backward(run):
            dy = torch.empty_like(y)
            bwd_units, dgbs = [], []
            for (conv, bn, _), out, (c0, C_, mean, invstd, scale, shift) in zip(units, outs, saved):
                dgb = (run.grad_out(bn.weight), run.grad_out(bn.bias))
                sums = run.empty(ops.bn_backward_workspace(N, C_), dtype=torch.float64)
                bwd_units.append(dict(dz=run.grad_of(out), y=y[:, c0:c0 + C_], scale=scale, shift=shift,
                                      mean=mean, invstd=invstd, sums=sums, dy=dy[:, c0:c0 + C_],
                                      dgamma=dgb[0], dbeta=dgb[1], relu=True, training=training))
                dgbs.append(dgb)
            yield ("bn_bwd", bwd_units)
            for (conv, bn, _), dgb in zip(units, dgbs):
                if bn.weight.requires_grad:
                    run.add_param_grad(bn.weight, dgb[0])
                if bn.bias.requires_grad:
                    run.add_param_grad(bn.bias, dgb[1])
            if any(w.requires_grad for w in weights):
                with torch.cuda.stream(run.side_stream(dy, xv)):
                    ws = run.empty(geom.wgrad_workspace())
                    if len(weights) <= 4:
                        dws = [run.grad_out(w) for w in weights]
                        ops.conv_wgrad(geom, xv, dy, dws, ws, Cin, 1, 0)
                    else:
                        dw = run.empty(Ccat, Cin, 1, 1, 1)
                        ops.conv_wgrad(geom, xv, dy, dw, ws, Cin, 1, 0)
                        dws = list(torch.split(dw, widths))
                for w, dw in zip(weights, dws):
                    if w.requires_grad:
                        run.add_param_grad(w, dw)
            if x_needs:
                dx, acc = run.grad_target(x)
                yield ("conv", dict(geom=geom.dgrad(), x=dy, w=run.pack_concat(weights, True), y=dx,
                                    accumulate=acc))

        run.record(backward)
    return outs



def max_pool(run, x, kernel, stride, padding):
    N, Cc = x.shape[0], x.shape[1]
    g = ops.pool_geom(N, Cc, x.shape[2:], _triple(kernel), _triple(stride), _triple(padding))
    y = run.empty(N, Cc, *g.odim)
    need = run.needs_grad(x)
    idx = run.empty(N, Cc, *g.odim, dtype=torch.int32) if need else None
    fused = False
    if x.lazy is not None and x.whole:
        ysrc, scale, shift, relu = x.lazy
        x.lazy = "consumed"
        ops.maxpool_fwd(g, ysrc, y, idx, in_scale=scale, in_shift=shift, in_relu=relu)
        fused = POOLED_BACKWARD and ops.pooled_backward_fits(g)
    else:
        ops.maxpool_fwd(g, x.view(), y, idx)
    out = Val(y)
    if need and DECISION_PROBE is not None and tuple(g.k) != (1, 1, 1):
        DECISION_PROBE("pool", None, idx)
    if need:
        xid = id(x.base)

        def backward(run):
            if fused:
                run.pooled[xid] = (g, run.grad_of(out), idx)
                return
            dx, acc = run.grad_target(x)
            ops.maxpool_bwd(g, run.grad_of(out), idx, dx, accumulate=acc)
        run.record(backward)
    elif run.save:
        run.no_grad_bases.add(id(y))
    return out


def subsample(run, x, stride):
    return max_pool(run, x, (1, 1, 1), stride, (0, 0, 0))



def self_gating(run, x, fc, out=None):
    xv = x.view()
    N, C_ = xv.shape[0], xv.shape[1]
    S = xv.shape[2] * xv.shape[3] * xv.shape[4]
    if not xv.is_contiguous():
        raise NotImplementedError("coclr_amd: self gating expects a dense input")
    a5 = run.empty(N, C_, 1, 1, 1)
    ops.global_avgpool_fwd(xv, a5)
    a = a5.view(N, C_)
    s_ = run.empty(N, C_)
    W_ = fc.weight
    ops.gemm(a, C_, 1, W_, 1, C_, s_, C_, fc.bias, N, C_, C_)
    wgt = run.empty(N, C_)
    ops.sigmoid_fwd(s_, wgt)
    if out is None:
        out = Val(torch.empty_like(xv))
    ops.plane_scale(xv, wgt, None, out.view())
    if run.save:
        def backward(run):
            dout = run.grad_of(out)
            dwgt = run.empty(N, C_)
            ops.plane_dot(dout, xv, dwgt)
            ds = run.empty(N, C_)
            ops.sigmoid_bwd(dwgt, wgt, ds)
            if fc.weight.requires_grad:
                dW = torch.empty_like(W_)
                ops.gemm(ds, 1, C_, a, C_, 1, dW, C_, None, C_, C_, N)
                db = run.empty(C_)
                ops.colsum(ds, db)
                run.add_param_grad(fc.weight, dW)
                run.add_param_grad(fc.bias, db)
            if run.needs_grad(x):
                back = run.empty(N, C_)
                ops.gemm(ds, C_, 1, W_, C_, 1, back, C_, None, N, C_, C_, alpha=1.0 / S)
                g, acc = run.grad_target(x)
                ops.plane_scale(dout, wgt, back, g, accumulate=acc)
        run.record(backward)
    return out



class EngineFn(torch.autograd.Function):

    @staticmethod
    def forward(ctx, module, kwargs, x, *params):
        need_dx = x.requires_grad
        new_pass(x.device)
        run = Run(x.device, save=True, need_input_grad=need_dx)
        xin = Val(x if _dense5(x) else x.contiguous())
        if not need_dx:
            run.no_grad_bases.add(id(xin.base))
        run.begin(module)
        run.out = module._emit(run, xin, **kwargs)
        ctx.run = run
        ctx.xin = xin
        ctx.params = params
        ctx.need_dx = need_dx
        ctx.module_defer = getattr(module, "__dict__", {}).get("_coclr_defer_join", False)
        out = run.out.view()
        return out.detach() if out.is_contiguous() else out.contiguous()

    @staticmethod
    def backward(ctx, dout):
        run = ctx.run
        if run is None:
            raise RuntimeError("coclr_amd: backbone backward called twice (graph not retained)")
        ctx.run = None
        run.backward(dout, defer_join=DEFER_JOIN and bool(ctx.module_defer))
        dx = run.grads.pop(id(ctx.xin.base), None) if ctx.need_dx else None
        grads = tuple(run.param_grads.pop(id(p), None) if p.requires_grad else None
                      for p in ctx.params)
        run.param_grads.clear()
        run.grads.clear()
        return (None, None, dx) + grads


PLAN = os.environ.get("COCLR_PLAN", "1") != "0" and hasattr(torch.cuda, "MemPool") and \
    hasattr(torch.cuda, "use_mem_pool")
_PLAN_WARMUP = 4
_PLAN_MAX_SHAPES = 3
PLAN_STATS = {"recorded": 0, "replayed": 0, "disabled": [], "infer_recorded": 0, "infer_replayed": 0}
_STATIC_PTRS = set()


class _PlanEntry:
    __slots__ = ("sig", "seen", "pool", "fwd", "bwd", "run", "xin", "x_ptr", "x_span", "x_refs", "x_fixed",
                 "out", "dout", "grads", "dx", "params", "need_dx", "version", "disabled", "static_dout", "defer",
                 "stream")

    def __init__(self, sig):
        self.sig, self.seen = sig, 0
        self.pool = self.fwd = self.bwd = self.run = self.xin = None
        self.x_ptr = self.x_span = 0
        self.x_refs, self.x_fixed = None, False
        self.out = self.dout = self.grads = self.dx = None
        self.params, self.need_dx = (), False
        self.version = 0
        self.disabled = False
        self.static_dout = None
        self.defer = False
        self.stream = 0


def _plan_signature(module, x, params):
    bns = module.__dict__.get("_coclr_bn_list")
    if bns is None:
        bns = module.__dict__["_coclr_bn_list"] = [
            m for m in module.modules() if isinstance(m, torch.nn.modules.batchnorm._BatchNorm)]
    slots = tuple(_GRAD_SLOTS[id(p)][1].data_ptr() if id(p) in _GRAD_SLOTS else 0 for p in params)
    return (tuple(x.shape), x.dtype, x.device, bool(x.requires_grad),
            tuple(p.data_ptr() for p in params), tuple(bool(p.requires_grad) for p in params), slots,
            tuple((m.training, m.momentum, m.eps, m.running_mean.data_ptr()) for m in bns),
            tuple(x.stride()), WGRAD_STREAM, DEFER_JOIN, PAIR_UNITS, FUSE_BN_REDUCE, LAZY_APPLY, POOLED_BACKWARD,
        BATCH_PACK, tuple(id(p) in _SLOTS_VERIFIED for p in params))


def _plan_drop(ent):
    for t in (ent.out, ent.dx):
        if t is not None:
            _STATIC_PTRS.discard(t.data_ptr())


def _plan_entry(module, x, params, kwargs):
    if kwargs or not x.is_cuda or x.dim() != 5 or not _dense5(x) or DECISION_PROBE is not None or \
            torch.cuda.is_current_stream_capturing():
        return None
    store = module.__dict__.get("_coclr_plan_entries")
    if store is None:
        store = module.__dict__["_coclr_plan_entries"] = {}
    sig = _plan_signature(module, x, params)
    key = (tuple(x.shape), bool(x.requires_grad))
    ent = store.get(key)
    if ent is None and len(store) >= _PLAN_MAX_SHAPES:
        return None
    if ent is None or ent.sig != sig:
        if ent is not None:
            _plan_drop(ent)
        ent = store[key] = _PlanEntry(sig)
    if ent.disabled:
        return None
    ent.seen += 1
    if ent.seen <= _PLAN_WARMUP:
        return None
    stream = torch.cuda.current_stream(x.device).cuda_stream
    if ent.fwd is not None:
        if stream != ent.stream:
            return None
        if x.data_ptr() != ent.x_ptr and (ent.x_fixed or ent.run is not None):
            return None
    return ent


def _record_forward(ent, module, x, defer):
    dev = x.device
    need_dx = bool(x.requires_grad)
    ent.pool = torch.cuda.MemPool()
    ent.stream = torch.cuda.current_stream(dev).cuda_stream
    rec = _plan.Recorder(ent.stream)
    with torch.cuda.use_mem_pool(ent.pool, device=dev), rec:
        run = Run(dev, save=True, need_input_grad=need_dx)
        xin = Val(x.detach())
        if not need_dx:
            run.no_grad_bases.add(id(xin.base))
        run.begin(module)
        run.out = module._emit(run, xin)
        out = run.out.view()
        if not out.is_contiguous():
            rec.taint("the node's output is a channel slice")
            out = out.contiguous()
    n, c, t, h, w = x.shape
    ent.x_ptr = x.data_ptr()
    ent.x_span = ((n - 1) * x.stride(0) + c * t * h * w) * x.element_size()
    ent.fwd, ent.run, ent.xin, ent.out = rec.plan, run, xin, out
    ent.params, ent.need_dx, ent.defer = None, need_dx, defer
    ent.x_refs = [rec.plan.pointer_refs(ent.x_ptr, ent.x_ptr + ent.x_span), None]
    ent.x_fixed = rec.plan.embedded_refs(ent.x_ptr, ent.x_ptr + ent.x_span)
    if rec.tainted:
        ent.disabled = True
        PLAN_STATS["disabled"].append(rec.tainted)
    PLAN_STATS["recorded"] += 1
    _STATIC_PTRS.add(out.data_ptr())


def _record_backward(ent, dout, params):
    dev = dout.device
    if dout.is_contiguous() and dout.data_ptr() in _STATIC_PTRS:
        static_dout, ent.static_dout = dout.detach(), True
    else:
        static_dout, ent.static_dout = None, None
    run = ent.run
    rec = _plan.Recorder(torch.cuda.current_stream(dev).cuda_stream)
    with torch.cuda.use_mem_pool(ent.pool, device=dev):
        if static_dout is None:
            static_dout = torch.empty(ent.out.shape, dtype=dout.dtype, device=dev)
            static_dout.copy_(dout)
        with rec:
            run.backward(static_dout, defer_join=DEFER_JOIN and ent.defer)
            dx = run.grads.pop(id(ent.xin.base), None) if ent.need_dx else None
            grads = tuple(run.param_grads.pop(id(p), None) if p.requires_grad else None for p in params)
            run.param_grads.clear()
            run.grads.clear()
    if rec.plan.stream != ent.stream:
        rec.taint("backward ran on another stream than the forward")
    ent.bwd, ent.dout, ent.grads, ent.dx = rec.plan, static_dout, grads, dx
    ent.run = None
    ent.x_refs[1] = rec.plan.pointer_refs(ent.x_ptr, ent.x_ptr + ent.x_span)
    ent.x_fixed = ent.x_fixed or rec.plan.embedded_refs(ent.x_ptr, ent.x_ptr + ent.x_span)
    if rec.tainted:
        ent.disabled = True
        PLAN_STATS["disabled"].append(rec.tainted)
    if dx is not None:
        _STATIC_PTRS.add(dx.data_ptr())


class PlanFn(torch.autograd.Function):

    @staticmethod
    def forward(ctx, ent, module, x, *params):
        new_pass(x.device)
        if ent.fwd is None:
            _record_forward(ent, module, x, getattr(module, "__dict__", {}).get("_coclr_defer_join", False))
        else:
            p = x.data_ptr()
            if p != ent.x_ptr:
                ent.fwd.patch(ent.x_refs[0], p)
                if ent.bwd is not None:
                    ent.bwd.patch(ent.x_refs[1], p)
                ent.x_ptr = p
            ent.fwd.replay()
            PLAN_STATS["replayed"] += 1
        ent.version += 1
        ctx.ent, ctx.version, ctx.params = ent, ent.version, params
        return ent.out.detach()

    @staticmethod
    def backward(ctx, dout):
        ent = ctx.ent
        if ent is None:
            raise RuntimeError("coclr_amd: backbone backward called twice (graph not retained)")
        if ctx.version != ent.version:
            raise RuntimeError(
                "coclr_amd: backward through a planned encoder pass whose activations a later forward has "
                "overwritten (two forwards, then two backwards); set COCLR_PLAN=0")
        ctx.ent = None
        params = ctx.params
        if ent.grads is not None:
            for p, g in zip(params, ent.grads):
                if g is not None and p.grad is not None and p.grad.data_ptr() == g.data_ptr():
                    p.grad = p.grad.clone()
        if ent.bwd is None:
            _record_backward(ent, dout, params)
        else:
            if torch.cuda.current_stream(dout.device).cuda_stream != ent.stream:
                raise RuntimeError("coclr_amd: planned backward called on another stream than it was recorded on")
            if ent.static_dout is None or dout.data_ptr() != ent.dout.data_ptr():
                ent.dout.copy_(dout)
            ent.bwd.replay()
        grads = tuple(None if g is None else g.view_as(g) for g in ent.grads)
        dx = ent.dx.view_as(ent.dx) if ent.dx is not None else None
        return (None, None, dx) + grads


def _dense5(t):
    n, c, d, h, w = t.shape
    s = t.stride()
    return s[4] == 1 and s[3] == w and s[2] == h * w and s[1] == d * h * w


PLAN_INFER = os.environ.get("COCLR_PLAN_INFER", "1") != "0" and hasattr(torch.cuda, "MemPool") and \
    hasattr(torch.cuda, "use_mem_pool")
_INFER_MAX_SHAPES = 3
_INFER_STORE = "_coclr_infer_plans"


class _InferEntry:
    __slots__ = ("sig", "seen", "pool", "fwd", "out", "x_ptr", "x_refs", "x_fixed", "disabled", "stream", "keep")

    def __init__(self, sig):
        self.sig, self.seen = sig, 0
        self.pool = self.fwd = self.out = self.x_refs = self.keep = None
        self.x_ptr, self.x_fixed = 0, False
        self.disabled = False
        self.stream = 0


def enable_inference_plans(module):
    module.__dict__.setdefault(_INFER_STORE, {})
    return module


def release_inference_plans(module):
    store = module.__dict__.get(_INFER_STORE)
    if store:
        store.clear()


def inference_plan_pools(module):
    return sum(1 for e in module.__dict__.get(_INFER_STORE, {}).values() if e.pool is not None)


def _bn_list(module):
    bns = module.__dict__.get("_coclr_bn_list")
    if bns is None:
        bns = module.__dict__["_coclr_bn_list"] = [
            m for m in module.modules() if isinstance(m, torch.nn.modules.batchnorm._BatchNorm)]
    return bns


def _infer_signature(module, x, params, bns):
    return (x.dtype, x.device, tuple(p.data_ptr() for p in params),
            tuple((m.momentum, m.eps, m.running_mean.data_ptr(), m.running_var.data_ptr()) for m in bns),
            PAIR_UNITS, LAZY_APPLY, IN_AFFINE, BATCH_PACK)


def _infer_record(ent, module, x):
    dev = x.device
    pool = torch.cuda.MemPool()
    ent.stream = torch.cuda.current_stream(dev).cuda_stream
    rec = _plan.Recorder(ent.stream)
    ent.disabled = True
    with torch.cuda.use_mem_pool(pool, device=dev), rec:
        run = Run(dev, save=False)
        run.begin(module)
        out = module._emit(run, Val(x)).view()
        if not out.is_contiguous():
            rec.taint("the module's output is a channel slice")
    PLAN_STATS["infer_recorded"] += 1
    if rec.tainted:
        PLAN_STATS["disabled"].append(rec.tainted)
        return out.contiguous()
    n, c, t, h, w = x.shape
    lo = x.data_ptr()
    hi = lo + ((n - 1) * x.stride(0) + c * t * h * w) * x.element_size()
    ent.x_ptr, ent.x_refs, ent.x_fixed = lo, rec.plan.pointer_refs(lo, hi), rec.plan.embedded_refs(lo, hi)
    ent.fwd, ent.out, ent.pool = rec.plan, out, pool
    ent.keep = None if run.plan is None else (run.plan.table, run.plan.blockmap)
    ent.disabled = False
    return out.clone()


def _infer_pass(module, x, params):
    if not x.is_cuda or DECISION_PROBE is not None or _plan._ACTIVE is not None or \
            torch.cuda.is_current_stream_capturing():
        return None
    store = module.__dict__[_INFER_STORE]
    bns = _bn_list(module)
    key = (tuple(x.shape), tuple(x.stride()), tuple(m.training for m in bns))
    sig = _infer_signature(module, x, params, bns)
    ent = store.get(key)
    if ent is None and len(store) >= _INFER_MAX_SHAPES:
        return None
    if ent is None or ent.sig != sig:
        ent = store[key] = _InferEntry(sig)
    if ent.disabled:
        return None
    ent.seen += 1
    if ent.seen <= _PLAN_WARMUP:
        return None
    if ent.fwd is None:
        return _infer_record(ent, module, x)
    if torch.cuda.current_stream(x.device).cuda_stream != ent.stream:
        return None
    p = x.data_ptr()
    if p != ent.x_ptr:
        if ent.x_fixed:
            return None
        ent.fwd.patch(ent.x_refs, p)
        ent.x_ptr = p
    ent.fwd.replay()
    PLAN_STATS["infer_replayed"] += 1
    return ent.out.clone()


def run_module(module, x, **kwargs):
    params = module.__dict__.get("_coclr_params")
    if params is None:
        params = module.__dict__["_coclr_params"] = list(module.parameters())
    if torch.is_grad_enabled() and (x.requires_grad or any(p.requires_grad for p in params)):
        if PLAN:
            ent = _plan_entry(module, x, params, kwargs)
            if ent is not None:
                return PlanFn.apply(ent, module, x, *params)
        return EngineFn.apply(module, kwargs, x, *params)
    if not _dense5(x):
        x = x.contiguous()
    if PLAN_INFER and not kwargs and _INFER_STORE in module.__dict__:
        out = _infer_pass(module, x, params)
        if out is not None:
            return out
    run = Run(x.device, save=False)
    xin = Val(x)
    run.begin(module)
    out = module._emit(run, xin, **kwargs).view()
    plan = run.plan
    if plan is not None and plan.dirty and not (
            x.device.type == "cuda" and torch.cuda.is_current_stream_capturing()):
        plan.build(x.device)
    return out if out.is_contiguous() else out.contiguous()
```

### coclr_amd/ops.py

```python
import ctypes as C
import os
import threading

import torch

from . import _lib
from . import plan as _plan
from ._lib import BnBwdCall, BnFwdCall, ConvCall, ConvDesc, PoolDesc


_HANDLE = None
_MAIN_THREAD = threading.get_ident()


def _desc(geom):
    if threading.get_ident() == _MAIN_THREAD:
        return geom.desc
    d = geom.desc_bw
    if d is None:
        d = geom.desc_bw = type(geom.desc).from_buffer_copy(geom.desc)
    return d


def _L():
    global _HANDLE
    if _HANDLE is None:
        _HANDLE = _lib.load()
    if _plan._ACTIVE is not None:
        rec = _plan.active()
        if rec is not None:
            return rec.proxy
    return _HANDLE


_HOST_DELAY = float(os.environ.get("COCLR_HOST_DELAY_US", "0")) * 1e-6


def _stream():
    if _HOST_DELAY:
        import time
        t = time.perf_counter() + _HOST_DELAY
        while time.perf_counter() < t:
            pass
    return torch.cuda.current_stream().cuda_stream


def _p(t, dtype=torch.float32):
    if t is None:
        return None
    if not t.is_cuda:
        raise _lib.HipLibraryError(
            "coclr_amd: kernels need device tensors (got %s); there is no CPU fallback" % t.device)
    if t.dtype != dtype:
        raise TypeError("coclr_amd: expected %s tensor, got %s" % (dtype, t.dtype))
    return t.data_ptr()


def _chk5(t, name):
    n, c, d, h, w = t.shape
    s = t.stride()
    if not (s[4] == 1 and s[3] == w and s[2] == h * w and s[1] == d * h * w) and t.numel() > 0:
        raise ValueError("coclr_amd: %s must be dense in (C,T,H,W); strides %s shape %s" %
                         (name, s, tuple(t.shape)))
    return s[0] if n > 1 else max(s[0], c * d * h * w)


WINOGRAD = os.environ.get("COCLR_WINOGRAD", "1") != "0"
WINOGRAD_HW = os.environ.get("COCLR_WINOGRAD_HW", "1") != "0"
WINOGRAD_T4 = os.environ.get("COCLR_WINO_T4", "1") != "0"
WINOGRAD_POLY7 = os.environ.get("COCLR_WINO_POLY7", "1") != "0"
WINOGRAD_PHASES = os.environ.get("COCLR_WINO_PHASES", "1") != "0"
_WINO_HW_MIN = int(os.environ.get("COCLR_WINO_HW_MIN", "16"))
_WINO_T4_MIN = int(os.environ.get("COCLR_WINO_T4_MIN", "16"))


def winograd_ok(cin, k, s, p, d, lattice, odim=None, idim=None, algo=1):
    k, p = tuple(k), tuple(p)
    if k == (7, 1, 1):
        return (WINOGRAD and WINOGRAD_POLY7 and tuple(s) == (2, 1, 1) and p == (3, 0, 0) and
                tuple(d) == (1, 1, 1) and lattice is None and cin >= 16 and odim is not None and
                idim is not None and idim[0] == 2 * odim[0] and odim[0] >= 8)
    if lattice is not None:
        ys, yo = tuple(lattice[0]), tuple(lattice[1])
        if not (algo == 2 and ys[1:] == (1, 1) and yo[1:] == (0, 0)):
            return False
    if not (WINOGRAD and tuple(s) == (1, 1, 1) and tuple(d) == (1, 1, 1)):
        return False
    if k == (4, 1, 1):
        return algo == 2 and p == (1, 0, 0) and cin >= 16 and odim is not None and idim is not None and \
            odim[0] == idim[0]
    if k == (3, 1, 1):
        return p == (1, 0, 0) and cin >= 16
    if k == (1, 3, 3):
        return (WINOGRAD_HW and p == (0, 1, 1) and cin >= 16 and odim is not None
                and odim[1] % 2 == 0 and odim[2] % 2 == 0 and odim[1] >= 4 and odim[2] >= 4)
    return False


def winograd_pays(cin, k, s, p, odim, idim=None):
    if not winograd_ok(cin, k, s, p, (1, 1, 1), None, odim, idim):
        return False
    if tuple(k) == (7, 1, 1):
        return odim[0] >= 16
    return tuple(k) != (1, 3, 3) or (odim[1] >= _WINO_HW_MIN and odim[2] >= _WINO_HW_MIN)


def winograd_t4_pays(odim):
    return WINOGRAD_T4 and odim[0] >= _WINO_T4_MIN


class ConvGeom:

    __slots__ = ("N", "Cin", "Cout", "idim", "odim", "k", "s", "p", "d", "lattice", "algo", "desc",
                 "desc_bw", "_cache")

    def __init__(self, N, Cin, Cout, idim, k, s, p, d=(1, 1, 1), odim=None, lattice=None, algo=0):
        self.N, self.Cin, self.Cout = int(N), int(Cin), int(Cout)
        self.idim = tuple(int(v) for v in idim)
        self.k, self.s, self.p, self.d = (tuple(int(v) for v in t) for t in (k, s, p, d))
        if odim is None:
            odim = tuple(((self.idim[i] - 1) * self.d[i] + 1 + 2 * self.p[i] - self.k[i]) //
                         self.s[i] + 1 for i in range(3))
        self.odim = tuple(int(v) for v in odim)
        if min(self.odim) <= 0:
            raise ValueError("coclr_amd: convolution output would be empty: in %s k %s s %s p %s" %
                             (self.idim, self.k, self.s, self.p))
        self.lattice = lattice
        lat = (0,) * 9 if lattice is None else tuple(lattice[0]) + tuple(lattice[1]) + \
            tuple(lattice[2])
        self.algo = int(algo)
        if self.algo not in (0, 1, 2):
            raise ValueError("coclr_amd: unknown convolution algorithm %d" % self.algo)
        if self.algo == 2 and self.k not in ((3, 1, 1), (4, 1, 1)):
            raise ValueError("coclr_amd: algorithm 2 is F(4,3) of a (3,1,1) stencil or F(2,4) of a (4,1,1) one")
        if self.algo >= 1 and not winograd_ok(self.Cin, self.k, self.s, self.p, self.d, lattice,
                                              self.odim, self.idim, self.algo):
            raise ValueError("coclr_amd: Winograd needs a (3,1,1) or (1,3,3) stride-1 'same' stencil, or the "
                             "(7,1,1) stride-2 pad-3 temporal stem conv on an even frame count")
        self.desc = ConvDesc(self.N, self.Cin, self.Cout, *self.idim, *self.odim, *self.k,
                             *self.s, *self.p, *self.d, 0, 0, *lat, 0, self.algo)
        self.desc_bw = None
        self._cache = {}

    @property
    def taps(self):
        return self.k[0] * self.k[1] * self.k[2]

    def dgrad(self):
        g = self._cache.get("dgrad")
        if g is None:
            pad = tuple(self.k[i] - 1 - self.p[i] for i in range(3))
            if min(pad) < 0:
                raise ValueError("coclr_amd: padding larger than kernel-1 is not supported")
            algo = self.algo if self.algo >= 1 and winograd_ok(self.Cout, self.k, (1, 1, 1), pad,
                                                               self.s, None, self.idim) else 0
            g = ConvGeom(self.N, self.Cout, self.Cin, self.odim, self.k, (1, 1, 1), pad,
                         d=self.s, odim=self.idim, algo=algo)
            self._cache["dgrad"] = g
        return g

    def dgrad_phases(self):
        g = self._cache.get("phases", False)
        if g is not False:
            return g
        out = None
        axes = [i for i in range(3) if self.s[i] > 1]
        if len(axes) == 1 and self.d == (1, 1, 1):
            ax = axes[0]
            others = [i for i in range(3) if i != ax]
            if all(self.k[i] == 1 and self.p[i] == 0 for i in others) and ax == 0:
                st, K, P = self.s[ax], self.k[ax], self.p[ax]
                out = []
                for phi in range(st):
                    k0 = (phi + P) % st
                    nk = (K - k0 + st - 1) // st
                    m_phi = (self.idim[ax] - phi + st - 1) // st
                    if nk not in (1, 3, 4) or m_phi <= 0:
                        out = None
                        break
                    c = (phi + P - k0) // st
                    kk, pp, od, ys, yo = [1, 1, 1], [0, 0, 0], list(self.idim), [1, 1, 1], [0, 0, 0]
                    kk[ax], pp[ax], od[ax], ys[ax], yo[ax] = nk, nk - 1 - c, m_phi, st, phi
                    lat = (ys, yo, self.idim)
                    algo = 2 if (WINOGRAD_PHASES and winograd_t4_pays(od) and nk in (3, 4) and
                                 winograd_ok(self.Cout, tuple(kk), (1, 1, 1), tuple(pp), (1, 1, 1), lat,
                                             tuple(od), self.odim, 2)) else 0
                    geom = ConvGeom(self.N, self.Cout, self.Cin, self.odim, kk, (1, 1, 1), pp,
                                    odim=od, lattice=lat, algo=algo)
                    out.append((geom, k0, nk, st))
        self._cache["phases"] = out
        return out

    def ntiles(self):
        v = self._cache.get("ntiles")
        if v is None:
            out = C.c_int32(0)
            _lib.check(_L().coclr_conv3d_ntiles(C.byref(self.desc), C.byref(out)),
                       "conv3d_ntiles", self)
            v = self._cache["ntiles"] = out.value
        return v

    def bwd_sums_ok(self):
        v = self._cache.get("bwd_sums_ok")
        if v is None:
            out = C.c_int32(0)
            _lib.check(_L().coclr_conv3d_bwd_sums_ok(C.byref(self.desc), C.byref(out)),
                       "conv3d_bwd_sums_ok", self)
            v = self._cache["bwd_sums_ok"] = bool(out.value)
        return v

    def wgrad_bn_ok(self):
        v = self._cache.get("wgrad_bn_ok")
        if v is None:
            out = C.c_int32(0)
            _lib.check(_L().coclr_conv3d_wgrad_bn_ok(C.byref(self.desc), C.byref(out)),
                       "conv3d_wgrad_bn_ok", self)
            v = self._cache["wgrad_bn_ok"] = bool(out.value)
        return v

    def wgrad_workspace(self):
        v = self._cache.get("wgws")
        if v is None:
            out = C.c_int64(0)
            _lib.check(_L().coclr_conv3d_wgrad_workspace(C.byref(self.desc), C.byref(out)),
                       "conv3d_wgrad_workspace", self)
            v = self._cache["wgws"] = out.value
        return v

    def __repr__(self):
        return "ConvGeom(N=%d, %d->%d, in=%s, out=%s, k=%s, s=%s, p=%s, d=%s)" % (
            self.N, self.Cin, self.Cout, self.idim, self.odim, self.k, self.s, self.p, self.d)


_GEOMS = {}


def conv_geom(N, Cin, Cout, idim, k, s, p):
    key = (N, Cin, Cout, tuple(idim), tuple(k), tuple(s), tuple(p))
    g = _GEOMS.get(key)
    if g is None:
        if len(_GEOMS) > 8192:
            _GEOMS.clear()
        g = ConvGeom(N, Cin, Cout, idim, k, s, p)
        if winograd_pays(Cin, k, s, p, g.odim, g.idim):
            g = ConvGeom(N, Cin, Cout, idim, k, s, p,
                         algo=2 if (tuple(k) == (3, 1, 1) and winograd_t4_pays(g.odim)) else 1)
        _GEOMS[key] = g
    return g


def pool_geom(N, Cc, idim, k, s, p):
    key = ("pool", N, Cc, tuple(idim), tuple(k), tuple(s), tuple(p))
    g = _GEOMS.get(key)
    if g is None:
        g = _GEOMS[key] = PoolGeom(N, Cc, idim, k, s, p)
    return g


class PoolGeom:
    __slots__ = ("N", "C", "idim", "odim", "k", "s", "p", "desc", "desc_bw", "_pooled_fits")

    def __init__(self, N, Cc, idim, k, s, p):
        self.N, self.C = int(N), int(Cc)
        self.idim = tuple(int(v) for v in idim)
        self.k, self.s, self.p = (tuple(int(v) for v in t) for t in (k, s, p))
        self.odim = tuple((self.idim[i] + 2 * self.p[i] - self.k[i]) // self.s[i] + 1
                          for i in range(3))
        if min(self.odim) <= 0:
            raise ValueError("coclr_amd: pooling output would be empty")
        self.desc = PoolDesc(self.N, self.C, *self.idim, *self.odim, *self.k, *self.s, *self.p, 0, 0)
        self.desc_bw = None
        self._pooled_fits = None



_PACKED = {}


def conv_packed_size(cin, cout, taps, transpose):
    key = (cin, cout, taps, bool(transpose))
    v = _PACKED.get(key)
    if v is not None:
        return v
    v = _PACKED[key] = _conv_packed_size(cin, cout, taps, transpose)
    return v


def _conv_packed_size(cin, cout, taps, transpose):
    out = C.c_int64(0)
    _lib.check(_L().coclr_conv_packed_size(cin, cout, taps, int(transpose), C.byref(out)),
               "conv_packed_size")
    return out.value


def conv_pack_weights(w, packed, cout, cin, taps, co_stride, ci_stride, tap_base, transpose,
                      tap_step=1, row0=0, rows_total=0, col0=0, cols_total=0):
    _lib.check(_L().coclr_conv_pack_weights(
        _p(w), _p(packed), cout, cin, taps, co_stride, ci_stride, tap_base, tap_step,
        int(transpose), row0, rows_total, col0, cols_total, _stream()), "conv_pack_weights")


def conv_pack_describe(w, packed, cout, cin, taps, co_stride, ci_stride, tap_base, transpose,
                       tap_step=1, row0=0, rows_total=0, col0=0, cols_total=0):
    entry = (C.c_int64 * 16)()
    nb = C.c_int32()
    _lib.check(_L().coclr_conv_pack_describe(
        _p(w), _p(packed), cout, cin, taps, co_stride, ci_stride, tap_base, tap_step,
        int(transpose), row0, rows_total, col0, cols_total, entry, C.byref(nb)), "conv_pack_describe")
    return list(entry), nb.value


def conv_pack_batch(table, blockmap, requests=None):
    _lib.check(_L().coclr_conv_pack_batch(_p(table, torch.int64), _p(blockmap, torch.int32),
                                          blockmap.shape[0], _stream()), "conv_pack_batch")


def conv_fwd(geom, x, w_packed, y, stats=None, bias=None, ep_scale=None, ep_shift=None,
             n_index=None, relu=False, accumulate=False):
    d = _desc(geom)
    d.x_nstride = _chk5(x, "x")
    d.y_nstride = _chk5(y, "y")
    d.Nx = x.shape[0]
    _lib.check(_L().coclr_conv3d_fwd(
        C.byref(d), _p(x), _p(w_packed), _p(y), _p(stats), _p(bias), _p(ep_scale), _p(ep_shift),
        _p(n_index, torch.int64), int(relu), int(accumulate), _stream()), "conv3d_fwd", geom)


def conv_fwd_multi(calls):
    n = len(calls)
    arr = (ConvCall * n)()
    descs = []
    for i, c in enumerate(calls):
        geom, x, y = c["geom"], c["x"], c["y"]
        d = type(geom.desc).from_buffer_copy(_desc(geom))
        d.x_nstride = _chk5(x, "x")
        d.y_nstride = _chk5(y, "y")
        d.Nx = x.shape[0]
        descs.append(d)
        a = arr[i]
        a.d = C.pointer(d)
        a.x, a.w_packed, a.y = _p(x), _p(c["w"]), _p(y)
        a.stats = _p(c.get("stats"))
        a.bias = a.ep_scale = a.ep_shift = None
        a.n_index = _p(c.get("n_index"), torch.int64)
        a.relu = 0
        a.accumulate = int(bool(c.get("accumulate", False)))
        ia = c.get("in_affine")
        if ia is not None:
            a.in_scale, a.in_shift, a.in_relu = _p(ia[0]), _p(ia[1]), int(bool(ia[2]))
        bb = c.get("bwd_bn")
        if bb is not None:
            by = bb[0]
            if by.shape != y.shape or _chk5(by, "bwd_y") != d.y_nstride or not y.is_contiguous():
                raise ValueError("coclr_amd: bwd_bn's conv output must be laid out like the destination")
            a.bwd_y, a.bwd_scale, a.bwd_shift = _p(by), _p(bb[1]), _p(bb[2])
            a.bwd_mean, a.bwd_invstd, a.bwd_relu = _p(bb[3]), _p(bb[4]), int(bool(bb[5]))
    _lib.check(_L().coclr_conv3d_fwd_multi(arr, n, _stream()), "conv3d_fwd_multi",
               [c["geom"] for c in calls])


def conv_wgrad(geom, x, dy, dw, workspace, co_stride, ci_stride, tap_base, accumulate=False):
    d = _desc(geom)
    d.x_nstride = _chk5(x, "x")
    d.y_nstride = _chk5(dy, "dy")
    if isinstance(dw, (list, tuple)):
        n = len(dw)
        ptrs = (C.c_void_p * n)(*[_p(t) for t in dw])
        ends, tot = [], 0
        for t in dw:
            tot += t.shape[0]
            ends.append(tot)
        _lib.check(_L().coclr_conv3d_wgrad_multi(
            C.byref(d), _p(x), _p(dy), ptrs, (C.c_int32 * n)(*ends), n, _p(workspace), co_stride,
            ci_stride, tap_base, int(accumulate), _stream()), "conv3d_wgrad_multi", geom)
        return
    _lib.check(_L().coclr_conv3d_wgrad(
        C.byref(d), _p(x), _p(dy), _p(dw), _p(workspace), co_stride, ci_stride, tap_base,
        int(accumulate), _stream()), "conv3d_wgrad", geom)


def conv_wgrad_bn(geom, x, dz, y, coef, relu, dw, workspace, co_stride, ci_stride, tap_base=0,
                  accumulate=False):
    d = _desc(geom)
    d.x_nstride = _chk5(x, "x")
    d.y_nstride = _chk5(dz, "dz")
    _lib.check(_L().coclr_conv3d_wgrad_bn(
        C.byref(d), _p(x), _p(dz), _p(y), _chk5(y, "y"), _p(coef), int(relu), _p(dw), _p(workspace),
        co_stride, ci_stride, tap_base, int(accumulate), _stream()), "conv3d_wgrad_bn", geom)



def bn_finalize(stats, C_, ntiles, count, gamma, beta, running_mean, running_var, nbt, momentum,
                eps, mean, invstd, scale, shift, c0=0, c_total=None):
    c_total = C_ if c_total is None else c_total
    base = _p(stats)
    _lib.check(_L().coclr_bn_finalize(
        base + 4 * c0 * ntiles, base + 4 * (c_total + c0) * ntiles, C_, ntiles, float(count),
        _p(gamma), _p(beta), _p(running_mean), _p(running_var), _p(nbt, torch.int64), momentum, eps,
        _p(mean), _p(invstd), _p(scale), _p(shift), _stream()), "bn_finalize")


def bn_finalize_apply(stats, C_, ntiles, count, gamma, beta, running_mean, running_var, nbt,
                      momentum, eps, mean, invstd, scale, shift, y, z, relu, c0=0, c_total=None):
    c_total = C_ if c_total is None else c_total
    base = _p(stats)
    N, _, T, H, W = y.shape
    _lib.check(_L().coclr_bn_finalize_apply(
        base + 4 * c0 * ntiles, base + 4 * (c_total + c0) * ntiles, C_, ntiles, float(count),
        _p(gamma), _p(beta), _p(running_mean), _p(running_var), _p(nbt, torch.int64), momentum, eps,
        _p(mean), _p(invstd), _p(scale), _p(shift), _p(y), _p(z), N, T * H * W, _chk5(y, "y"),
        _chk5(z, "z"), int(relu), _stream()), "bn_finalize_apply")


def bn_finalize_apply_multi(units):
    n = len(units)
    arr = (BnFwdCall * n)()
    for a, u in zip(arr, units):
        C_, ntiles = u["C"], u["ntiles"]
        c0 = u.get("c0", 0)
        c_total = u.get("c_total") or C_
        base = _p(u["stats"])
        gamma, beta, rm, rv, nbt, momentum, eps = u["bn"]
        mean, invstd, scale, shift = u["small"]
        y, z = u["y"], u["z"]
        N, _, T, H, W = y.shape
        a.sum = base + 4 * c0 * ntiles
        a.sumsq = base + 4 * (c_total + c0) * ntiles
        a.gamma, a.beta, a.running_mean, a.running_var = _p(gamma), _p(beta), _p(rm), _p(rv)
        a.num_batches_tracked = _p(nbt, torch.int64)
        a.mean, a.invstd, a.scale, a.shift = _p(mean), _p(invstd), _p(scale), _p(shift)
        a.y, a.z = _p(y), _p(z)
        a.count = float(u["count"])
        a.S = T * H * W
        a.y_nstride, a.z_nstride = _chk5(y, "y"), _chk5(z, "z")
        a.C, a.ntiles, a.N, a.relu = C_, ntiles, N, int(u["relu"])
        a.momentum, a.eps = momentum, eps
    _lib.check(_L().coclr_bn_finalize_apply_multi(arr, n, _stream()), "bn_finalize_apply_multi")


def bn_act_backward_multi(units):
    n = len(units)
    arr = (BnBwdCall * n)()
    for a, u in zip(arr, units):
        y = u["y"]
        N, C_, T, H, W = y.shape
        if u["sums"].numel() < 2 * C_ * N:
            raise ValueError("coclr_amd: bn_act_backward workspace too small")
        a.dz, a.y, a.scale, a.shift = _p(u["dz"]), _p(y), _p(u["scale"]), _p(u["shift"])
        a.mean, a.invstd = _p(u["mean"]), _p(u["invstd"])
        a.sums_ws = _p(u["sums"], torch.float64)
        a.dy, a.dgamma, a.dbeta = _p(u["dy"]), _p(u["dgamma"]), _p(u["dbeta"])
        a.S = T * H * W
        a.dz_nstride, a.y_nstride, a.dy_nstride = _chk5(u["dz"], "dz"), _chk5(y, "y"), _chk5(u["dy"], "dy")
        a.N, a.C, a.relu, a.training = N, C_, int(u["relu"]), int(u["training"])
        parts = u.get("partials")
        if parts:
            if len(parts) > 2:
                raise ValueError("coclr_amd: at most two partial-sum arrays per BatchNorm backward")
            for i, (st, nt) in enumerate(parts):
                if st.numel() != 2 * C_ * nt:
                    raise ValueError("coclr_amd: partial sums do not match the unit's channels")
                a.part[i] = _p(st)
                a.part_ntiles[i] = nt
    _lib.check(_L().coclr_bn_act_backward_multi(arr, n, _stream()), "bn_act_backward_multi")


SMALL_CHANNEL = 32768


def bn_eval_affine(gamma, beta, running_mean, running_var, eps, C_, mean, invstd, scale, shift):
    _lib.check(_L().coclr_bn_eval_affine(
        _p(gamma), _p(beta), _p(running_mean), _p(running_var), eps, C_, _p(mean), _p(invstd),
        _p(scale), _p(shift), _stream()), "bn_eval_affine")


def bn_act_apply(y, scale, shift, residual, z, relu):
    N, C_, T, H, W = y.shape
    S = T * H * W
    _lib.check(_L().coclr_bn_act_apply(
        _p(y), _p(scale), _p(shift), _p(residual), _p(z), N, C_, S, _chk5(y, "y"), _chk5(z, "z"),
        _chk5(residual, "residual") if residual is not None else 0, int(relu), _stream()),
        "bn_act_apply")


def bn_backward_workspace(N, C_):
    return 2 * C_ * N


def bn_act_backward(dz, y, z, scale, shift, mean, invstd, sums_ws, dy, dres, dgamma, dbeta, relu,
                    training, dres_accumulate=False):
    N, C_, T, H, W = y.shape
    S = T * H * W
    if sums_ws.numel() < 2 * C_ * N:
        raise ValueError("coclr_amd: bn_act_backward workspace too small")
    _lib.check(_L().coclr_bn_act_backward(
        _p(dz), _p(y), _p(z), _p(scale), _p(shift), _p(mean), _p(invstd),
        _p(sums_ws, torch.float64), _p(dy), _p(dres), _p(dgamma), _p(dbeta), N, C_, S,
        _chk5(dz, "dz"), _chk5(y, "y"), _chk5(dy, "dy"), _chk5(z, "z") if z is not None else 0,
        _chk5(dres, "dres") if dres is not None else 0, int(relu), int(training),
        int(dres_accumulate), _stream()), "bn_act_backward")


def bn_act_backward_coeffs(dz, y, scale, shift, mean, invstd, sums_ws, coef, dgamma, dbeta, relu, training):
    N, C_, T, H, W = y.shape
    if sums_ws.numel() < 2 * C_ * N:
        raise ValueError("coclr_amd: bn_act_backward workspace too small")
    if coef.numel() < 5 * C_:
        raise ValueError("coclr_amd: bn_act_backward_coeffs needs 5 x C coefficients")
    _lib.check(_L().coclr_bn_act_backward_coeffs(
        _p(dz), _p(y), _p(scale), _p(shift), _p(mean), _p(invstd), _p(sums_ws, torch.float64), _p(coef),
        _p(dgamma), _p(dbeta), N, C_, T * H * W, _chk5(dz, "dz"), _chk5(y, "y"), int(relu), int(training),
        _stream()), "bn_act_backward_coeffs")



def maxpool_fwd(geom, x, y, indices=None, in_scale=None, in_shift=None, in_relu=False):
    d = _desc(geom)
    d.x_nstride = _chk5(x, "x")
    d.y_nstride = _chk5(y, "y")
    _lib.check(_L().coclr_maxpool3d_fwd(C.byref(d), _p(x), _p(y), _p(indices, torch.int32),
                                        _p(in_scale), _p(in_shift), int(in_relu), _stream()),
               "maxpool3d_fwd")


def maxpool_bwd(geom, dy, indices, dx, accumulate=False):
    _lib.check(_L().coclr_maxpool3d_bwd(
        C.byref(_desc(geom)), _p(dy), _p(indices, torch.int32), _p(dx), _chk5(dy, "dy"),
        _chk5(dx, "dx"), int(accumulate), _stream()), "maxpool3d_bwd")


def bn_act_backward_pooled(geom, pool_dy, indices, y, scale, shift, mean, invstd, sums_ws, dy, dgamma,
                           dbeta, relu, training):
    N, C_ = y.shape[0], y.shape[1]
    if sums_ws.numel() < 2 * C_ * N:
        raise ValueError("coclr_amd: bn_act_backward_pooled workspace too small")
    _lib.check(_L().coclr_bn_act_backward_pooled(
        C.byref(_desc(geom)), _p(pool_dy), _p(indices, torch.int32), _p(y), _p(scale), _p(shift),
        _p(mean), _p(invstd), _p(sums_ws, torch.float64), _p(dy), _p(dgamma), _p(dbeta),
        _chk5(pool_dy, "pool_dy"), _chk5(y, "y"), _chk5(dy, "dy"), int(relu), int(training),
        _stream()), "bn_act_backward_pooled")


def pooled_backward_fits(geom):
    v = getattr(geom, "_pooled_fits", None)
    if v is None:
        out = C.c_int32(0)
        _lib.check(_L().coclr_bn_act_backward_pooled_fits(C.byref(geom.desc), C.byref(out)),
                   "bn_act_backward_pooled_fits")
        v = bool(out.value)
        try:
            geom._pooled_fits = v
        except AttributeError:
            pass
    return v


def global_avgpool_fwd(x, y):
    planes = x.shape[0] * x.shape[1]
    _lib.check(_L().coclr_global_avgpool_fwd(_p(x), _p(y), planes, x.numel() // planes,
                                                    _stream()), "global_avgpool_fwd")


def global_avgpool_bwd(dy, dx):
    planes = dx.shape[0] * dx.shape[1]
    _lib.check(_L().coclr_global_avgpool_bwd(_p(dy), _p(dx), planes, dx.numel() // planes,
                                                    _stream()), "global_avgpool_bwd")



def gemm_workspace(M, N, K, splits):
    out = C.c_int64(0)
    _lib.check(_L().coclr_gemm_workspace(M, N, K, splits, C.byref(out)), "gemm_workspace")
    return out.value


def gemm(a, sam, sak, b, sbk, sbn, c, ldc, bias, M, N, K, alpha=1.0, relu=False, accumulate=False,
         splits=1, workspace=None):
    _lib.check(_L().coclr_gemm(
        _p(a), sam, sak, _p(b), sbk, sbn, _p(c), ldc, _p(bias), M, N, K, alpha, int(relu),
        int(accumulate), splits, _p(workspace), _stream()), "gemm")


def gemm_fused_workspace(M, N, K, splits):
    return M * N * max(1, splits)


def gemm_fused(a, sam, sak, b, sbk, sbn, c, ldc, bias, M, N, K, alpha=1.0, relu=False, splits=1,
               workspace=None, mode=0, S=0, ep_a=None, lda=0, ep_b=None, ep_y=None, inv_norm=None, out2=None,
               f=0.0, rowsum=None):
    ep = _lib.GemmEpilogue(int(mode), int(S), _p(ep_a), int(lda), _p(ep_b), _p(ep_y), _p(inv_norm), _p(out2),
                           float(f), _p(rowsum))
    _lib.check(_L().coclr_gemm_fused(
        _p(a), sam, sak, _p(b), sbk, sbn, _p(c), ldc, _p(bias), M, N, K, alpha, int(relu), splits,
        _p(workspace), C.byref(ep), _stream()), "gemm_fused")


def l2norm_fwd(x, y, inv_norm, eps=1e-12):
    rows, D = x.shape
    _lib.check(_L().coclr_l2norm_fwd(_p(x), _p(y), _p(inv_norm), rows, D, eps, _stream()),
               "l2norm_fwd")


def l2norm_bwd(dy, y, inv_norm, dx):
    rows, D = y.shape
    _lib.check(_L().coclr_l2norm_bwd(_p(dy), _p(y), _p(inv_norm), _p(dx), rows, D,
                                            _stream()), "l2norm_bwd")


def nce_logits_fwd(q, k, queue, logits, T):
    B, D = q.shape
    K = queue.shape[1]
    _lib.check(_L().coclr_nce_logits_fwd(_p(q), _p(k), _p(queue), _p(logits), B, D, K, T,
                                                _stream()), "nce_logits_fwd")


def nce_logits_bwd(dlogits, k, queue, dq, workspace, T, splits):
    B, D = dq.shape
    K = queue.shape[1]
    _lib.check(_L().coclr_nce_logits_bwd(_p(dlogits), _p(k), _p(queue), _p(dq),
                                                _p(workspace), B, D, K, T, splits, _stream()),
               "nce_logits_bwd")


def momentum_update(table, nchunks, m, one_minus_m, pairs=None):
    _lib.check(_L().coclr_momentum_update(_p(table, torch.int64), nchunks, m, one_minus_m,
                                                 _stream()), "momentum_update")


def queue_enqueue(queue, keys, ptr):
    D, K = queue.shape
    BW = keys.shape[0]
    _lib.check(_L().coclr_queue_enqueue(_p(queue), _p(keys), D, K, BW,
                                               _p(ptr, torch.int64), _stream()), "queue_enqueue")


def queue_fill_i64(queue, vals, const_val, BW, ptr):
    _lib.check(_L().coclr_queue_fill_i64(
        _p(queue, torch.int64), _p(vals, torch.int64), const_val, queue.shape[0], BW,
        _p(ptr, torch.int64), _stream()), "queue_fill_i64")


def queue_advance(ptr, BW, K):
    _lib.check(_L().coclr_queue_advance(_p(ptr, torch.int64), BW, K, _stream()),
               "queue_advance")


def positive_mask(sim, src, names, mask, topk):
    B, K1 = mask.shape
    _lib.check(_L().coclr_positive_mask(
        _p(sim), _p(src, torch.int64), _p(names, torch.int64), _p(mask, torch.uint8), B, K1 - 1,
        topk, _stream()), "positive_mask")


def mine_workspace(B, K, topk, device):
    nt = (K + 63) // 64
    return (torch.empty(B * nt * max(topk, 1), dtype=torch.float32, device=device),
            torch.empty(B * nt * max(topk, 1), dtype=torch.int32, device=device),
            torch.zeros((B + 31) // 32, dtype=torch.int32, device=device))


def mine_positives(kf, queue_second, src, names, mask, topk, workspace, sim_out=None):
    B, D = kf.shape
    K = queue_second.shape[1]
    cv, ci, cnt = workspace
    nt = (K + 63) // 64
    if cv.numel() < B * nt * max(topk, 1) or cnt.numel() < (B + 31) // 32:
        raise ValueError("coclr_amd: mine_positives workspace too small")
    _lib.check(_L().coclr_mine_positives(
        _p(kf), _p(queue_second), _p(src, torch.int64), _p(names, torch.int64), _p(mask, torch.uint8),
        _p(cv), _p(ci, torch.int32), _p(cnt, torch.int32), _p(sim_out), B, D, K, topk, _stream()),
        "mine_positives")


def gather_rows(inp, idx, out):
    rows = out.shape[0]
    row_elems = out.numel() // rows
    if inp.dim() > 1 and inp[0].numel() == row_elems and inp[0].is_contiguous():
        in_stride = inp.stride(0) if inp.shape[0] > 1 else row_elems
    else:
        raise ValueError("coclr_amd: gather_rows needs dense source rows")
    _lib.check(_L().coclr_gather_rows(_p(inp), _p(idx, torch.int64), _p(out), rows,
                                             row_elems, max(in_stride, row_elems), _stream()),
               "gather_rows")


def pull_rows(row_ptrs, out, keep=None):
    rows = out.shape[0]
    _lib.check(_L().coclr_pull_rows(_p(row_ptrs, torch.int64), _p(out), rows, out.numel() // rows,
                                    _stream()), "pull_rows")


def relu_fwd(x, y):
    _lib.check(_L().coclr_relu_fwd(_p(x), _p(y), x.numel(), _stream()), "relu_fwd")


def relu_bwd(dy, y, dx):
    _lib.check(_L().coclr_relu_bwd(_p(dy), _p(y), _p(dx), y.numel(), _stream()), "relu_bwd")


def colsum(x, out):
    rows, cols = x.shape
    _lib.check(_L().coclr_colsum(_p(x), _p(out), rows, cols, _stream()), "colsum")



def sigmoid_fwd(s_, w):
    _lib.check(_L().coclr_sigmoid_fwd(_p(s_), _p(w), s_.numel(), _stream()), "sigmoid_fwd")


def sigmoid_bwd(dw, w, ds):
    _lib.check(_L().coclr_sigmoid_bwd(_p(dw), _p(w), _p(ds), w.numel(), _stream()), "sigmoid_bwd")


def plane_scale(a, gain, bias, out, accumulate=False):
    N, C_, T, H, W = a.shape
    _lib.check(_L().coclr_plane_scale(_p(a), _p(gain), _p(bias), _p(out), N, C_, T * H * W,
                                      _chk5(a, "a"), _chk5(out, "out"), int(accumulate), _stream()),
               "plane_scale")


def plane_dot(a, b, out):
    N, C_, T, H, W = a.shape
    _lib.check(_L().coclr_plane_dot(_p(a), _p(b), _p(out), N, C_, T * H * W, _chk5(a, "a"),
                                    _chk5(b, "b"), _stream()), "plane_dot")



def adam_step(table, nchunks, hyper, steps, groups, ngroups, mom_m=0.0, mom_1m=0.0, keep=None):
    _lib.check(_L().coclr_adam_step(_p(table, torch.int64), nchunks, _p(hyper, torch.float64), _p(steps),
                                    _p(groups, torch.int32), ngroups, mom_m, mom_1m, _stream()),
               "adam_step")


def sgd_step(table, nchunks, hyper, keep=None):
    _lib.check(_L().coclr_sgd_step(_p(table, torch.int64), nchunks, _p(hyper, torch.float64), _stream()),
               "sgd_step")


def nce_loss_fwd(logits, mask, target, rowstats, flags, scalars, mode, drop_self=False, k1=1, k2=5):
    B, N1 = logits.shape
    _lib.check(_L().coclr_nce_loss_fwd(
        _p(logits), _p(mask, torch.uint8), _p(target, torch.int64), _p(rowstats),
        _p(flags, torch.uint8), _p(scalars), B, N1, mode, int(drop_self), k1, k2, _stream()),
        "nce_loss_fwd")


def nce_loss_bwd(logits, mask, target, rowstats, flags, dloss, dlogits, mode):
    B, N1 = logits.shape
    _lib.check(_L().coclr_nce_loss_bwd(
        _p(logits), _p(mask, torch.uint8), _p(target, torch.int64), _p(rowstats),
        _p(flags, torch.uint8), _p(dloss), _p(dlogits), B, N1, mode, _stream()), "nce_loss_bwd")


def stage_clips(frames, out, S, mean, std):
    B, Cc = frames.shape[0], frames.shape[1]
    thw = frames[0, 0].numel() // S
    if frames.dtype == torch.uint8:
        src, u8 = _p(frames, torch.uint8), 1
    else:
        src, u8 = _p(frames), 0
    m = (C.c_float * Cc)(*[float(v) for v in mean])
    s = (C.c_float * Cc)(*[float(v) for v in std])
    _lib.check(_L().coclr_stage_clips(src, u8, _p(out), B, Cc, S, thw, m, s, _stream()),
               "stage_clips")



def colstats_workspace(rows, cols):
    out = C.c_int64(0)
    _lib.check(_L().coclr_colstats_workspace(rows, cols, C.byref(out)), "colstats_workspace")
    return out.value


def bn1d_stats(x, stats, workspace):
    rows, cols = x.shape
    _lib.check(_L().coclr_bn1d_stats(_p(x), _p(stats), _p(workspace), rows, cols, _stream()),
               "bn1d_stats")


def center_rows(x, out, workspace):
    rows, cols = x.shape
    _lib.check(_L().coclr_center_rows(_p(x), _p(out), _p(workspace), rows, cols, _stream()),
               "center_rows")


def retrieval_hits(sim, train_label, test_label, ks, hits, topidx=None):
    B, N = sim.shape
    if topidx is None:
        raise ValueError("coclr_amd: retrieval_hits needs the topidx buffer (B, kmax)")
    kmax = int(topidx.shape[1])
    _lib.check(_L().coclr_retrieval_hits(
        _p(sim), _p(train_label, torch.int64), _p(test_label, torch.int64), _p(ks, torch.int32),
        ks.shape[0], _p(hits), _p(topidx, torch.int32), B, N, kmax, _stream()),
        "retrieval_hits")


SEGMENT_MAX_C = 4096


def _segment_call(name, x, segs, weight, out):
    R, C_ = x.shape
    V = out.shape[0]
    if out.dim() != 2 or out.shape[1] != C_ or not x.is_contiguous() or not out.is_contiguous():
        raise ValueError("coclr_amd: %s takes dense (R, C) rows and a dense (V, C) output" % name)
    if not 1 <= C_ <= SEGMENT_MAX_C:
        raise ValueError("coclr_amd: %s takes rows of 1..%d columns, got %d" % (name, SEGMENT_MAX_C, C_))
    segs = [tuple(int(v) for v in sg) for sg in segs]
    weight = [float(w) for w in weight]
    S = len(segs)
    if S == 0 or len(weight) != S or any(len(sg) != 3 for sg in segs):
        raise ValueError("coclr_amd: %s needs S >= 1 segments (first row, rows, out row) and S weights" % name)
    seg_arr = (C.c_int32 * (3 * S))(*[v for sg in segs for v in sg])
    w_arr = (C.c_float * S)(*weight)
    _lib.check(getattr(_L(), "coclr_" + name)(_p(x), seg_arr, w_arr, _p(out), R, C_, S, V, _stream()), name,
               segs)


def segment_softmax_accum(logits, segs, weight, out):
    _segment_call("segment_softmax_accum", logits, segs, weight, out)


def segment_accum(x, segs, weight, out):
    _segment_call("segment_accum", x, segs, weight, out)
```

### include/coclr_hip.h

```cpp
#ifndef COCLR_HIP_H_
#define COCLR_HIP_H_

#include <stdint.h>

#ifdef __cplusplus
extern "C" {
#endif


typedef struct coclr_conv_desc {
  int32_t N, Cin, Cout;
  int32_t Ti, Hi, Wi;
  int32_t To, Ho, Wo;
  int32_t kt, kh, kw;
  int32_t st, sh, sw;
  int32_t pt, ph, pw;
  int32_t dt, dh, dw;
  int64_t x_nstride;
  int64_t y_nstride;
  int32_t ys_t, ys_h, ys_w;
  int32_t yo_t, yo_h, yo_w;
  int32_t yT, yH, yW;
  int32_t Nx;
  int32_t algo;
} coclr_conv_desc;

int coclr_conv_packed_size(int cin, int cout, int taps, int transpose, int64_t* elems);

int coclr_conv_pack_weights(const float* w, float* packed, int cout, int cin, int taps,
                            int64_t co_stride, int64_t ci_stride, int tap_base, int tap_step,
                            int transpose, int row0, int rows_total, int col0, int cols_total,
                            void* stream);

int coclr_conv_pack_describe(const float* w, float* packed, int cout, int cin, int taps,
                             int64_t co_stride, int64_t ci_stride, int tap_base, int tap_step,
                             int transpose, int row0, int rows_total, int col0, int cols_total,
                             int64_t* entry, int32_t* nblocks);
int coclr_conv_pack_batch(const int64_t* table, const int32_t* blockmap, int nblocks,
                          void* stream);

int coclr_conv3d_ntiles(const coclr_conv_desc* d, int* ntiles);

int coclr_conv3d_fwd(const coclr_conv_desc* d, const float* x, const float* w_packed, float* y,
                     float* stats, const float* bias, const float* ep_scale,
                     const float* ep_shift, const int64_t* n_index, int relu, int accumulate,
                     void* stream);

typedef struct coclr_conv_call {
  const coclr_conv_desc* d;
  const float* x;
  const float* w_packed;
  float* y;
  float* stats;
  const float* bias;
  const float* ep_scale;
  const float* ep_shift;
  const int64_t* n_index;
  int32_t relu, accumulate;
  const float* bwd_y;
  const float* bwd_scale;
  const float* bwd_shift;
  const float* bwd_mean;
  const float* bwd_invstd;
  int32_t bwd_relu;
  int32_t in_relu;
  const float* in_scale;
  const float* in_shift;
} coclr_conv_call;
int coclr_conv3d_fwd_multi(const coclr_conv_call* calls, int n, void* stream);
int coclr_conv3d_bwd_sums_ok(const coclr_conv_desc* d, int* ok);

int coclr_conv3d_wgrad_workspace(const coclr_conv_desc* d, int64_t* elems);

int coclr_conv3d_wgrad(const coclr_conv_desc* d, const float* x, const float* dy, float* dw,
                       float* workspace, int64_t w_co_stride, int64_t w_ci_stride, int tap_base,
                       int accumulate, void* stream);

int coclr_conv3d_wgrad_bn_ok(const coclr_conv_desc* d, int* ok);
int coclr_conv3d_wgrad_bn(const coclr_conv_desc* d, const float* x, const float* dz, const float* y,
                          int64_t y_nstride, const float* coef, int relu, float* dw, float* workspace,
                          int64_t w_co_stride, int64_t w_ci_stride, int tap_base, int accumulate,
                          void* stream);

int coclr_conv3d_wgrad_multi(const coclr_conv_desc* d, const float* x, const float* dy,
                             float* const* dw_list, const int32_t* row_end, int nseg,
                             float* workspace, int64_t w_co_stride, int64_t w_ci_stride,
                             int tap_base, int accumulate, void* stream);


int coclr_bn_finalize(const float* sum, const float* sumsq, int C, int ntiles, double count,
                      const float* gamma, const float* beta, float* running_mean,
                      float* running_var, int64_t* num_batches_tracked, float momentum, float eps,
                      float* mean, float* invstd, float* scale, float* shift, void* stream);

int coclr_bn_finalize_apply(const float* sum, const float* sumsq, int C, int ntiles, double count,
                            const float* gamma, const float* beta, float* running_mean,
                            float* running_var, int64_t* num_batches_tracked, float momentum,
                            float eps, float* mean, float* invstd, float* scale, float* shift,
                            const float* y, float* z, int N, int64_t S, int64_t y_nstride,
                            int64_t z_nstride, int relu, void* stream);

int coclr_bn_eval_affine(const float* gamma, const float* beta, const float* running_mean,
                         const float* running_var, float eps, int C, float* mean, float* invstd,
                         float* scale, float* shift, void* stream);

int coclr_bn_act_apply(const float* y, const float* scale, const float* shift,
                       const float* residual, float* z, int N, int C, int64_t S, int64_t y_nstride,
                       int64_t z_nstride, int64_t res_nstride, int relu, void* stream);

int coclr_bn_backward_workspace(int N, int C, int64_t* doubles);
int coclr_bn_act_backward(const float* dz, const float* y, const float* z, const float* scale,
                          const float* shift, const float* mean, const float* invstd,
                          double* sums_ws, float* dy, float* dres, float* dgamma, float* dbeta,
                          int N, int C, int64_t S, int64_t dz_nstride, int64_t y_nstride,
                          int64_t dy_nstride, int64_t z_nstride, int64_t dres_nstride, int relu,
                          int training, int dres_accumulate, void* stream);

int coclr_bn_act_backward_coeffs(const float* dz, const float* y, const float* scale, const float* shift,
                                 const float* mean, const float* invstd, double* sums_ws, float* coef,
                                 float* dgamma, float* dbeta, int N, int C, int64_t S,
                                 int64_t dz_nstride, int64_t y_nstride, int relu, int training,
                                 void* stream);


typedef struct coclr_pool_desc {
  int32_t N, C;
  int32_t Ti, Hi, Wi, To, Ho, Wo;
  int32_t kt, kh, kw, st, sh, sw, pt, ph, pw;
  int64_t x_nstride, y_nstride;
} coclr_pool_desc;

int coclr_maxpool3d_fwd(const coclr_pool_desc* d, const float* x, float* y, int32_t* indices,
                        const float* in_scale, const float* in_shift, int in_relu, void* stream);
int coclr_maxpool3d_bwd(const coclr_pool_desc* d, const float* dy, const int32_t* indices, float* dx,
                        int64_t dy_nstride, int64_t dx_nstride, int accumulate, void* stream);

typedef struct coclr_bn_fwd_call {
  const float* sum; const float* sumsq; const float* gamma; const float* beta;
  float* running_mean; float* running_var; int64_t* num_batches_tracked;
  float* mean; float* invstd; float* scale; float* shift;
  const float* y; float* z;
  double count;
  int64_t S, y_nstride, z_nstride;
  int32_t C, ntiles, N, relu;
  float momentum, eps;
} coclr_bn_fwd_call;
typedef struct coclr_bn_bwd_call {
  const float* dz; const float* y; const float* scale; const float* shift; const float* mean;
  const float* invstd;
  double* sums_ws; float* dy; float* dgamma; float* dbeta;
  int64_t S, dz_nstride, y_nstride, dy_nstride;
  int32_t N, C, relu, training;
  const float* part[2];
  int32_t part_ntiles[2];
} coclr_bn_bwd_call;
int coclr_bn_finalize_apply_multi(const coclr_bn_fwd_call* calls, int n, void* stream);
int coclr_bn_act_backward_multi(const coclr_bn_bwd_call* calls, int n, void* stream);

int coclr_bn_act_backward_pooled(const coclr_pool_desc* d, const float* pool_dy,
                                 const int32_t* pool_idx, const float* y, const float* scale,
                                 const float* shift, const float* mean, const float* invstd,
                                 double* sums, float* dy, float* dgamma, float* dbeta,
                                 int64_t pool_dy_nstride, int64_t y_nstride, int64_t dy_nstride,
                                 int relu, int training, void* stream);
int coclr_bn_act_backward_pooled_fits(const coclr_pool_desc* d, int* fits);
int coclr_global_avgpool_fwd(const float* x, float* y, int64_t planes, int64_t S, void* stream);
int coclr_global_avgpool_bwd(const float* dy, float* dx, int64_t planes, int64_t S, void* stream);


int coclr_gemm_workspace(int M, int N, int K, int splits, int64_t* elems);
int coclr_gemm(const float* a, int64_t sam, int64_t sak, const float* b, int64_t sbk, int64_t sbn,
               float* c, int64_t ldc, const float* bias, int M, int N, int K, float alpha, int relu,
               int accumulate, int splits, float* workspace, void* stream);

typedef struct coclr_gemm_epilogue {
  int32_t mode;
  int32_t S;
  const float* a;
  int64_t lda;
  const float* b;
  const float* y;
  const float* inv_norm;
  float* out2;
  float f;
  float* rowsum;
} coclr_gemm_epilogue;
int coclr_gemm_fused(const float* a, int64_t sam, int64_t sak, const float* b, int64_t sbk, int64_t sbn,
                     float* c, int64_t ldc, const float* bias, int M, int N, int K, float alpha, int relu,
                     int splits, float* workspace, const coclr_gemm_epilogue* ep, void* stream);

int coclr_l2norm_fwd(const float* x, float* y, float* inv_norm, int rows, int D, float eps,
                     void* stream);
int coclr_l2norm_bwd(const float* dy, const float* y, const float* inv_norm, float* dx, int rows,
                     int D, void* stream);

int coclr_nce_logits_fwd(const float* q, const float* k, const float* queue, float* logits, int B,
                         int D, int K, float T, void* stream);
int coclr_nce_logits_bwd(const float* dlogits, const float* k, const float* queue, float* dq,
                         float* workspace, int B, int D, int K, float T, int splits, void* stream);

int coclr_momentum_update(const int64_t* table, int nchunks, float m, float one_minus_m,
                          void* stream);

int coclr_queue_enqueue(float* queue, const float* keys, int D, int K, int BW, const int64_t* ptr,
                        void* stream);
int coclr_queue_fill_i64(int64_t* queue, const int64_t* vals, int64_t const_val, int K, int BW,
                         const int64_t* ptr, void* stream);
int coclr_queue_advance(int64_t* ptr, int BW, int K, void* stream);

int coclr_positive_mask(const float* sim, const int64_t* src, const int64_t* names, uint8_t* mask,
                        int B, int K, int topk, void* stream);

int coclr_mine_positives(const float* kf, const float* queue_second, const int64_t* src,
                         const int64_t* names, uint8_t* mask, float* cand_val, int32_t* cand_idx,
                         int32_t* counters, float* sim_out, int B, int D, int K, int topk,
                         void* stream);

int coclr_gather_rows(const float* in, const int64_t* idx, float* out, int rows, int64_t row_elems,
                      int64_t in_row_stride, void* stream);

int coclr_pull_rows(const int64_t* row_ptrs, float* out, int rows, int64_t row_elems, void* stream);

int coclr_relu_fwd(const float* x, float* y, int64_t n, void* stream);
int coclr_relu_bwd(const float* dy, const float* y, float* dx, int64_t n, void* stream);
int coclr_colsum(const float* x, float* out, int rows, int cols, void* stream);

int coclr_sigmoid_fwd(const float* s, float* w, int64_t n, void* stream);
int coclr_sigmoid_bwd(const float* dw, const float* w, float* ds, int64_t n, void* stream);
int coclr_plane_scale(const float* a, const float* gain, const float* bias, float* out, int N, int C,
                      int64_t S, int64_t a_nstride, int64_t out_nstride, int accumulate,
                      void* stream);
int coclr_plane_dot(const float* a, const float* b, float* out, int N, int C, int64_t S,
                    int64_t a_nstride, int64_t b_nstride, void* stream);


int coclr_adam_step(const int64_t* table, int nchunks, const double* hyper, float* steps,
                    const int32_t* groups, int ngroups, float mom_m, float mom_1m, void* stream);

int coclr_sgd_step(const int64_t* table, int nchunks, const double* hyper, void* stream);

int coclr_nce_loss_fwd(const float* logits, const uint8_t* mask, const int64_t* target,
                       float* rowstats, uint8_t* flags, float* scalars, int B, int N1, int mode,
                       int drop_self, int k1, int k2, void* stream);
int coclr_nce_loss_bwd(const float* logits, const uint8_t* mask, const int64_t* target,
                       const float* rowstats, const uint8_t* flags, const float* dloss,
                       float* dlogits, int B, int N1, int mode, void* stream);

int coclr_stage_clips(const void* frames, int from_u8, float* out, int B, int C, int S, int64_t THW,
                      const float* mean, const float* std, void* stream);


int coclr_colstats_workspace(int rows, int cols, int64_t* elems);
int coclr_bn1d_stats(const float* x, float* stats, float* workspace, int rows, int cols,
                     void* stream);
int coclr_center_rows(const float* x, float* out, float* workspace, int rows, int cols,
                      void* stream);
int coclr_retrieval_hits(const float* sim, const int64_t* train_label, const int64_t* test_label,
                         const int32_t* ks, int nk, float* hits, int32_t* topidx, int B, int N,
                         int kmax, void* stream);

int coclr_segment_softmax_accum(const float* logits, const int32_t* segs, const float* weight, float* out,
                                int R, int C, int S, int V, void* stream);
int coclr_segment_accum(const float* x, const int32_t* segs, const float* weight, float* out, int R, int C,
                        int S, int V, void* stream);

int coclr_abi_version(void);

#ifdef __cplusplus
}
#endif
#endif
```

Measured before the change: 1167.

## Batch large-map BatchNorm finalize/apply and backward into multi-unit kernel launches

Adds large-map multi-unit BatchNorm kernels. Finalize can either fold the per-tile partial sums directly inside the apply kernel or run as a separate multi-unit finalize launch, and backward reduce and apply each cover several units in one grid. Large feature-map BN units that previously went through per-unit launches are now grouped. Lazy-apply deferral is restricted to conv1 of separable blocks whose conv2 has temporal kernel 7. The aim is fewer kernel launches and less per-unit overhead, at the cost of table-dispatch branching and possibly redundant partial-sum folding per block.

```diff
diff --git a/coclr_amd/_lib.py b/coclr_amd/_lib.py
--- a/coclr_amd/_lib.py
+++ b/coclr_amd/_lib.py
@@ -70,6 +70,8 @@
                                 vp, vp, i32, i64, i64, i64, i32, vp],
     "coclr_bn_finalize_apply_multi": [_P(BnFwdCall), i32, vp],
     "coclr_bn_act_backward_multi": [_P(BnBwdCall), i32, vp],
+    "coclr_bn_finalize_apply_large_multi": [_P(BnFwdCall), i32, i32, vp],
+    "coclr_bn_act_backward_large_multi": [_P(BnBwdCall), i32, vp],
     "coclr_bn_eval_affine": [vp, vp, vp, vp, f32, i32, vp, vp, vp, vp, vp],
     "coclr_bn_act_apply": [vp, vp, vp, vp, vp, i32, i32, i64, i64, i64, i64, i32, vp],
     "coclr_bn_backward_workspace": [i32, i32, _P(i64)],
diff --git a/coclr_amd/backbone/s3dg.py b/coclr_amd/backbone/s3dg.py
--- a/coclr_amd/backbone/s3dg.py
+++ b/coclr_amd/backbone/s3dg.py
@@ -75,7 +75,8 @@
         return engine.conv_bn_act(run, mid, self.conv2, self.bn2, relu=True, out=out)
 
     def _emit_gen(self, run, x, out=None):
-        mid = yield from engine.conv_bn_act_gen(run, x, self.conv1, self.bn1, relu=True)
+        mid = yield from engine.conv_bn_act_gen(run, x, self.conv1, self.bn1, relu=True,
+                                                may_defer=self.conv2.kernel_size[0] == 7)
         return (yield from engine.conv_bn_act_gen(run, mid, self.conv2, self.bn2, relu=True, out=out))
 
 
diff --git a/coclr_amd/csrc/bn.hip b/coclr_amd/csrc/bn.hip
--- a/coclr_amd/csrc/bn.hip
+++ b/coclr_amd/csrc/bn.hip
@@ -4,19 +4,28 @@
 namespace {
 
 
-__global__ void __launch_bounds__(256)
-bn_finalize_kernel(const float* __restrict__ sum, const float* __restrict__ sumsq, int C,
-                   int ntiles, double count,
-                   const float* __restrict__ gamma, const float* __restrict__ beta,
-                   float* running_mean, float* running_var, int64_t* num_batches_tracked,
-                   float momentum, float eps, float* mean_out, float* invstd_out,
-                   float* scale_out, float* shift_out) {
+__device__ __forceinline__ void bn_fold_partials(const float* __restrict__ ps, const float* __restrict__ pq,
+                                                 int ntiles, double& s, double& q) {
+  int i = threadIdx.x;
+  for (; i + 7 * 256 < ntiles; i += 8 * 256) {
+    float a[8], b[8];
+#pragma unroll
+    for (int k = 0; k < 8; ++k) { a[k] = ps[i + k * 256]; b[k] = pq[i + k * 256]; }
+#pragma unroll
+    for (int k = 0; k < 8; ++k) { s += (double)a[k]; q += (double)b[k]; }
+  }
+  for (; i < ntiles; i += 256) { s += (double)ps[i]; q += (double)pq[i]; }
+}
+
+__device__ __forceinline__ void
+bn_finalize_body(const int c, const float* __restrict__ sum, const float* __restrict__ sumsq, int ntiles,
+                 double count, const float* __restrict__ gamma, const float* __restrict__ beta,
+                 float* running_mean, float* running_var, int64_t* num_batches_tracked, float momentum,
+                 float eps, float* mean_out, float* invstd_out, float* scale_out, float* shift_out,
+                 const bool write, float* coef) {
   __shared__ double red[4];
-  const int c = blockIdx.x;
-  const float* ps = sum + (long)c * ntiles;
-  const float* pq = sumsq + (long)c * ntiles;
   double s = 0.0, q = 0.0;
-  for (int i = threadIdx.x; i < ntiles; i += 256) { s += (double)ps[i]; q += (double)pq[i]; }
+  bn_fold_partials(sum + (long)c * ntiles, sumsq + (long)c * ntiles, ntiles, s, q);
   s = block256_sum_d(s, red);
   q = block256_sum_d(q, red);
   if (threadIdx.x == 0) {
@@ -25,18 +34,32 @@
     if (var < 0.0) var = 0.0;
     const float invstd = (float)(1.0 / sqrt(var + (double)eps));
     const float g = gamma ? gamma[c] : 1.f, b = beta ? beta[c] : 0.f;
-    const float sc = g * invstd;
-    mean_out[c] = (float)mean;
-    invstd_out[c] = invstd;
-    scale_out[c] = sc;
-    shift_out[c] = b - (float)mean * sc;
-    if (running_mean) {
-      const double unbiased = count > 1.0 ? var * count / (count - 1.0) : var;
-      running_mean[c] = (1.f - momentum) * running_mean[c] + momentum * (float)mean;
-      running_var[c] = (1.f - momentum) * running_var[c] + momentum * (float)unbiased;
-    }
-    if (c == 0 && num_batches_tracked) *num_batches_tracked += 1;
-  }
+    const float sc = g * invstd, sf = b - (float)mean * sc;
+    if (coef) { coef[0] = sc; coef[1] = sf; }
+    if (write) {
+      mean_out[c] = (float)mean;
+      invstd_out[c] = invstd;
+      scale_out[c] = sc;
+      shift_out[c] = sf;
+      if (running_mean) {
+        const double unbiased = count > 1.0 ? var * count / (count - 1.0) : var;
+        running_mean[c] = (1.f - momentum) * running_mean[c] + momentum * (float)mean;
+        running_var[c] = (1.f - momentum) * running_var[c] + momentum * (float)unbiased;
+      }
+      if (c == 0 && num_batches_tracked) *num_batches_tracked += 1;
+    }
+  }
+}
+
+__global__ void __launch_bounds__(256)
+bn_finalize_kernel(const float* __restrict__ sum, const float* __restrict__ sumsq, int C,
+                   int ntiles, double count,
+                   const float* __restrict__ gamma, const float* __restrict__ beta,
+                   float* running_mean, float* running_var, int64_t* num_batches_tracked,
+                   float momentum, float eps, float* mean_out, float* invstd_out,
+                   float* scale_out, float* shift_out) {
+  bn_finalize_body((int)blockIdx.x, sum, sumsq, ntiles, count, gamma, beta, running_mean, running_var,
+                   num_batches_tracked, momentum, eps, mean_out, invstd_out, scale_out, shift_out, true, nullptr);
 }
 
 __global__ void bn_eval_affine_kernel(const float* __restrict__ gamma, const float* __restrict__ beta,
@@ -77,21 +100,19 @@
   }
 }
 
-template <bool VEC, bool NT = false>
-__global__ void __launch_bounds__(256)
-bn_act_apply_kernel(const float* __restrict__ y, const float* __restrict__ scale,
-                    const float* __restrict__ shift, const float* __restrict__ res, float* z,
-                    int N, int C, int S, long y_nstride, long z_nstride, long res_nstride,
-                    int relu) {
-  const int c = blockIdx.y % C, sg = blockIdx.y / C, nsg = gridDim.y / C;
-  const float sc = scale[c], sf = shift[c];
+template <bool VEC, bool NT>
+__device__ __forceinline__ void
+bn_act_apply_body(const float* __restrict__ y, const float sc, const float sf, const float* __restrict__ res,
+                  float* z, int N, int C, int S, long y_nstride, long z_nstride, long res_nstride, int relu,
+                  const int bx, const int gx, const int by, const int gy) {
+  const int c = by % C, sg = by / C, nsg = gy / C;
   for (int n = sg; n < N; n += nsg) {
     const float* yp = y + (long)n * y_nstride + (long)c * S;
     float* zp = z + (long)n * z_nstride + (long)c * S;
     const float* rp = res ? res + (long)n * res_nstride + (long)c * S : nullptr;
     if (VEC) {
-      const int S4 = S >> 2, stride = gridDim.x * 256;
-      for (int i0 = blockIdx.x * 256 + threadIdx.x; i0 < S4; i0 += 4 * stride) {
+      const int S4 = S >> 2, stride = gx * 256;
+      for (int i0 = bx * 256 + threadIdx.x; i0 < S4; i0 += 4 * stride) {
         float4 v[4], r[4];
 #pragma unroll
         for (int k = 0; k < 4; ++k) {
@@ -128,7 +149,7 @@
         }
       }
     } else {
-      for (int i = blockIdx.x * 256 + threadIdx.x; i < S; i += gridDim.x * 256) {
+      for (int i = bx * 256 + threadIdx.x; i < S; i += gx * 256) {
         float v = fmaf(yp[i], sc, sf);
         if (rp) v += rp[i];
         if (relu) v = fmaxf(v, 0.f);
@@ -138,21 +159,32 @@
   }
 }
 
+template <bool VEC, bool NT = false>
+__global__ void __launch_bounds__(256)
+bn_act_apply_kernel(const float* __restrict__ y, const float* __restrict__ scale,
+                    const float* __restrict__ shift, const float* __restrict__ res, float* z,
+                    int N, int C, int S, long y_nstride, long z_nstride, long res_nstride,
+                    int relu) {
+  const int c = blockIdx.y % C;
+  bn_act_apply_body<VEC, NT>(y, scale[c], shift[c], res, z, N, C, S, y_nstride, z_nstride, res_nstride, relu,
+                             (int)blockIdx.x, (int)gridDim.x, (int)blockIdx.y, (int)gridDim.y);
+}
+
 
 template <bool VEC>
-__global__ void __launch_bounds__(256)
-bn_act_bwd_reduce_kernel(const float* __restrict__ dz, const float* __restrict__ y,
-                         const float* __restrict__ z, const float* __restrict__ scale,
-                         const float* __restrict__ shift, const float* __restrict__ mean,
-                         const float* __restrict__ invstd, double* sums, int N, int C, int S,
-                         long dz_nstride, long y_nstride, long z_nstride, int relu_nt) {
+__device__ __forceinline__ void
+bn_act_bwd_reduce_body(const float* __restrict__ dz, const float* __restrict__ y,
+                       const float* __restrict__ z, const float* __restrict__ scale,
+                       const float* __restrict__ shift, const float* __restrict__ mean,
+                       const float* __restrict__ invstd, double* sums, int N, int S,
+                       long dz_nstride, long y_nstride, long z_nstride, int relu_nt,
+                       const int c, const int grp, const int groups) {
   __shared__ double red[4];
   const int relu = relu_nt & 1;
   const bool nt = (relu_nt & 2) != 0;
-  const int c = blockIdx.x;
   const float sc = scale[c], sf = shift[c], mu = mean[c], is = invstd[c];
   double sg = 0.0, sgx = 0.0;
-  for (int n = blockIdx.y; n < N; n += gridDim.y) {
+  for (int n = grp; n < N; n += groups) {
     const float* dzp = dz + (long)n * dz_nstride + (long)c * S;
     const float* yp = y + (long)n * y_nstride + (long)c * S;
     const float* zp = z ? z + (long)n * z_nstride + (long)c * S : nullptr;
@@ -207,9 +239,20 @@
   sg = block256_sum_d(sg, red);
   sgx = block256_sum_d(sgx, red);
   if (threadIdx.x == 0) {
-    sums[((long)c * gridDim.y + blockIdx.y) * 2] = sg;
-    sums[((long)c * gridDim.y + blockIdx.y) * 2 + 1] = sgx;
-  }
+    sums[((long)c * groups + grp) * 2] = sg;
+    sums[((long)c * groups + grp) * 2 + 1] = sgx;
+  }
+}
+
+template <bool VEC>
+__global__ void __launch_bounds__(256)
+bn_act_bwd_reduce_kernel(const float* __restrict__ dz, const float* __restrict__ y,
+                         const float* __restrict__ z, const float* __restrict__ scale,
+                         const float* __restrict__ shift, const float* __restrict__ mean,
+                         const float* __restrict__ invstd, double* sums, int N, int C, int S,
+                         long dz_nstride, long y_nstride, long z_nstride, int relu_nt) {
+  bn_act_bwd_reduce_body<VEC>(dz, y, z, scale, shift, mean, invstd, sums, N, S, dz_nstride, y_nstride, z_nstride,
+                              relu_nt, (int)blockIdx.x, (int)blockIdx.y, (int)gridDim.y);
 }
 
 __global__ void __launch_bounds__(256)
@@ -233,19 +276,20 @@
 }
 
 template <bool VEC>
-__global__ void __launch_bounds__(256)
-bn_act_bwd_apply_kernel(const float* __restrict__ dz, const float* __restrict__ y,
-                        const float* __restrict__ z, const float* __restrict__ scale,
-                        const float* __restrict__ shift, const float* __restrict__ mean,
-                        const float* __restrict__ invstd, const double* __restrict__ sums,
-                        int groups, double count, int training, float* dgamma, float* dbeta,
-                        float* dy, float* dres, int N, int C, int S, long dz_nstride,
-                        long y_nstride, long dy_nstride, long z_nstride, long dres_nstride,
-                        int relu_nt, int dres_accumulate) {
+__device__ __forceinline__ void
+bn_act_bwd_apply_body(const float* __restrict__ dz, const float* __restrict__ y,
+                      const float* __restrict__ z, const float* __restrict__ scale,
+                      const float* __restrict__ shift, const float* __restrict__ mean,
+                      const float* __restrict__ invstd, const double* __restrict__ sums,
+                      int groups, double count, int training, float* dgamma, float* dbeta,
+                      float* dy, float* dres, int N, int C, int S, long dz_nstride,
+                      long y_nstride, long dy_nstride, long z_nstride, long dres_nstride,
+                      int relu_nt, int dres_accumulate,
+                      const int bx, const int gx, const int by, const int gy) {
   __shared__ double tot[2];
   const int relu = relu_nt & 1;
   const bool nt = (relu_nt & 2) != 0;
-  const int c = blockIdx.y % C, sgrp = blockIdx.y / C, nsg = gridDim.y / C;
+  const int c = by % C, sgrp = by / C, nsg = gy / C;
   if (threadIdx.x < 64) {
     double a0 = 0.0, a1 = 0.0;
     for (int g = threadIdx.x; g < groups; g += 64) {
@@ -265,7 +309,7 @@
     B = -sc * invstd[c] * mgx;
     D = sc * (mean[c] * invstd[c] * mgx - mg);
   }
-  if (sgrp == 0 && blockIdx.x == 0 && threadIdx.x == 0) {
+  if (sgrp == 0 && bx == 0 && threadIdx.x == 0) {
     if (dgamma) dgamma[c] = (float)sgx;
     if (dbeta) dbeta[c] = (float)sg;
   }
@@ -276,8 +320,8 @@
     float* dyp = dy + (long)n * dy_nstride + (long)c * S;
     float* drp = dres ? dres + (long)n * dres_nstride + (long)c * S : nullptr;
     if (VEC) {
-      const int S4 = S >> 2, stride = gridDim.x * 256;
-      for (int i0 = blockIdx.x * 256 + threadIdx.x; i0 < S4; i0 += 2 * stride) {
+      const int S4 = S >> 2, stride = gx * 256;
+      for (int i0 = bx * 256 + threadIdx.x; i0 < S4; i0 += 2 * stride) {
         float4 dd[2], vv[2], zq[2];
         bool ok[2];
 #pragma unroll
@@ -321,7 +365,7 @@
         }
       }
     } else {
-      for (int i = blockIdx.x * 256 + threadIdx.x; i < S; i += gridDim.x * 256) {
+      for (int i = bx * 256 + threadIdx.x; i < S; i += gx * 256) {
         float g = dzp[i];
         const float v = yp[i];
         if (relu) g = (zp ? zp[i] > 0.f : fmaf(v, sc, sf) > 0.f) ? g : 0.f;
@@ -330,6 +374,22 @@
       }
     }
   }
+}
+
+template <bool VEC>
+__global__ void __launch_bounds__(256)
+bn_act_bwd_apply_kernel(const float* __restrict__ dz, const float* __restrict__ y,
+                        const float* __restrict__ z, const float* __restrict__ scale,
+                        const float* __restrict__ shift, const float* __restrict__ mean,
+                        const float* __restrict__ invstd, const double* __restrict__ sums,
+                        int groups, double count, int training, float* dgamma, float* dbeta,
+                        float* dy, float* dres, int N, int C, int S, long dz_nstride,
+                        long y_nstride, long dy_nstride, long z_nstride, long dres_nstride,
+                        int relu_nt, int dres_accumulate) {
+  bn_act_bwd_apply_body<VEC>(dz, y, z, scale, shift, mean, invstd, sums, groups, count, training, dgamma, dbeta,
+                             dy, dres, N, C, S, dz_nstride, y_nstride, dy_nstride, z_nstride, dres_nstride,
+                             relu_nt, dres_accumulate, (int)blockIdx.x, (int)gridDim.x, (int)blockIdx.y,
+                             (int)gridDim.y);
 }
 
 __global__ void __launch_bounds__(64)
@@ -632,7 +692,123 @@
 #undef COCLR_BN_BWD_UNIT
 }
 
-constexpr long kSmallChannel = 32768;
+
+__global__ void __launch_bounds__(256)
+bn_finalize_multi_kernel(const BnFwdTable t) {
+  int c = (int)blockIdx.x;
+#define COCLR_BN_FIN_UNIT(k)                                                                              \
+  if (k < t.n) {                                                                                         \
+    if (c < t.u[k].C) {                                                                                  \
+      bn_finalize_body(c, t.u[k].sum, t.u[k].sumsq, t.u[k].ntiles, t.u[k].count, t.u[k].gamma,           \
+                       t.u[k].beta, t.u[k].running_mean, t.u[k].running_var, t.u[k].nbt,                 \
+                       t.u[k].momentum, t.u[k].eps, t.u[k].mean, t.u[k].invstd, t.u[k].scale,            \
+                       t.u[k].shift, true, nullptr);                                                     \
+      return;                                                                                            \
+    }                                                                                                    \
+    c -= t.u[k].C;                                                                                       \
+  }
+  COCLR_BN_FIN_UNIT(0)
+  COCLR_BN_FIN_UNIT(1)
+  COCLR_BN_FIN_UNIT(2)
+  COCLR_BN_FIN_UNIT(3)
+#undef COCLR_BN_FIN_UNIT
+}
+
+struct BnApplyTable { BnFwdUnit u[4]; int gx[4], gy[4], fold[4]; int n; };
+
+template <bool VEC, bool NT>
+__global__ void __launch_bounds__(256)
+bn_apply_multi_kernel(const BnApplyTable t) {
+  __shared__ float coef[2];
+  int b = (int)blockIdx.x;
+#define COCLR_BN_APPLY_UNIT(k)                                                                            \
+  if (k < t.n) {                                                                                         \
+    const int nb = t.gx[k] * t.gy[k];                                                                    \
+    if (b < nb) {                                                                                        \
+      const int bx = b % t.gx[k], by = b / t.gx[k], c = by % t.u[k].C;                                   \
+      float sc, sf;                                                                                      \
+      if (t.fold[k]) {                                                                                   \
+        bn_finalize_body(c, t.u[k].sum, t.u[k].sumsq, t.u[k].ntiles, t.u[k].count, t.u[k].gamma,         \
+                         t.u[k].beta, t.u[k].running_mean, t.u[k].running_var, t.u[k].nbt,               \
+                         t.u[k].momentum, t.u[k].eps, t.u[k].mean, t.u[k].invstd, t.u[k].scale,          \
+                         t.u[k].shift, bx == 0 && by < t.u[k].C, coef);                                  \
+        __syncthreads();                                                                                 \
+        sc = coef[0]; sf = coef[1];                                                                      \
+      } else {                                                                                           \
+        sc = t.u[k].scale[c]; sf = t.u[k].shift[c];                                                      \
+      }                                                                                                  \
+      bn_act_apply_body<VEC, NT>(t.u[k].y, sc, sf, nullptr, t.u[k].z, t.u[k].N, t.u[k].C, t.u[k].S,      \
+                                 t.u[k].y_nstride, t.u[k].z_nstride, 0L, t.u[k].relu, bx, t.gx[k], by,   \
+                                 t.gy[k]);                                                               \
+      return;                                                                                            \
+    }                                                                                                    \
+    b -= nb;                                                                                             \
+  }
+  COCLR_BN_APPLY_UNIT(0)
+  COCLR_BN_APPLY_UNIT(1)
+  COCLR_BN_APPLY_UNIT(2)
+  COCLR_BN_APPLY_UNIT(3)
+#undef COCLR_BN_APPLY_UNIT
+}
+
+struct BnBwdLargeTable { BnBwdUnit u[4]; double* sums[4]; int groups[4], gx[4], gy[4]; int n; };
+
+template <bool VEC>
+__global__ void __launch_bounds__(256)
+bn_bwd_reduce_multi_kernel(const BnBwdLargeTable t) {
+  int b = (int)blockIdx.x;
+  const float* noz = nullptr;
+#define COCLR_BN_RED_UNIT(k)                                                                              \
+  if (k < t.n) {                                                                                         \
+    const int nb = t.u[k].C * t.groups[k];                                                               \
+    if (b < nb) {                                                                                        \
+      bn_act_bwd_reduce_body<VEC>(t.u[k].dz, t.u[k].y, noz, t.u[k].scale, t.u[k].shift, t.u[k].mean,     \
+                                  t.u[k].invstd, t.sums[k], t.u[k].N, t.u[k].S, t.u[k].dz_nstride,       \
+                                  t.u[k].y_nstride, 0L, t.u[k].relu, b % t.u[k].C, b / t.u[k].C,         \
+                                  t.groups[k]);                                                          \
+      return;                                                                                            \
+    }                                                                                                    \
+    b -= nb;                                                                                             \
+  }
+  COCLR_BN_RED_UNIT(0)
+  COCLR_BN_RED_UNIT(1)
+  COCLR_BN_RED_UNIT(2)
+  COCLR_BN_RED_UNIT(3)
+#undef COCLR_BN_RED_UNIT
+}
+
+template <bool VEC>
+__global__ void __launch_bounds__(256)
+bn_bwd_apply_multi_kernel(const BnBwdLargeTable t) {
+  int b = (int)blockIdx.x;
+  const float* noz = nullptr;
+  float* nod = nullptr;
+#define COCLR_BN_BAPPLY_UNIT(k)                                                                           \
+  if (k < t.n) {                                                                                         \
+    const int nb = t.gx[k] * t.gy[k];                                                                    \
+    if (b < nb) {                                                                                        \
+      bn_act_bwd_apply_body<VEC>(t.u[k].dz, t.u[k].y, noz, t.u[k].scale, t.u[k].shift, t.u[k].mean,      \
+                                 t.u[k].invstd, t.sums[k], t.groups[k],                                  \
+                                 (double)t.u[k].N * (double)t.u[k].S, t.u[k].training, t.u[k].dgamma,    \
+                                 t.u[k].dbeta, t.u[k].dy, nod, t.u[k].N, t.u[k].C, t.u[k].S,             \
+                                 t.u[k].dz_nstride, t.u[k].y_nstride, t.u[k].dy_nstride, 0L, 0L,         \
+                                 t.u[k].relu, 0, b % t.gx[k], t.gx[k], b / t.gx[k], t.gy[k]);            \
+      return;                                                                                            \
+    }                                                                                                    \
+    b -= nb;                                                                                             \
+  }
+  COCLR_BN_BAPPLY_UNIT(0)
+  COCLR_BN_BAPPLY_UNIT(1)
+  COCLR_BN_BAPPLY_UNIT(2)
+  COCLR_BN_BAPPLY_UNIT(3)
+#undef COCLR_BN_BAPPLY_UNIT
+}
+
+inline long small_channel() {
+  const char* e = getenv("COCLR_BN_SMALL_CHANNEL");
+  return e ? atol(e) : 32768L;
+}
+const long kSmallChannel = small_channel();
 
 inline dim3 plane_grid(int N, int C, int S) {
   int gx = cdiv(S >> 2 ? S >> 2 : S, 256 * 4);
@@ -727,7 +903,7 @@
       u.mean = c.mean; u.invstd = c.invstd; u.scale = c.scale; u.shift = c.shift;
       u.y = c.y; u.z = c.z; u.count = c.count;
       u.y_nstride = (long)c.y_nstride; u.z_nstride = (long)c.z_nstride;
-      u.C = c.C; u.ntiles = c.ntiles; u.N = c.N; u.S = (int)c.S; u.relu = c.relu;
+      u.C = c.C; u.ntiles = c.ntiles; u.N = c.N; u.S = (int)c.S; u.relu = c.relu ? 1 : 0;
       u.momentum = c.momentum; u.eps = c.eps;
       blocks += c.C;
     }
@@ -891,12 +1067,12 @@
     hipLaunchKernelGGL(bn_act_bwd_apply_kernel<true>, grid, dim3(256), 0, stream, c.dz, c.y, nof, c.scale,
                        c.shift, c.mean, c.invstd, c.sums_ws, 1, count, c.training, c.dgamma, c.dbeta, c.dy, nod,
                        c.N, c.C, (int)c.S, (long)c.dz_nstride, (long)c.y_nstride, (long)c.dy_nstride, 0L, 0L,
-                       c.relu, 0);
+                       c.relu ? 1 : 0, 0);
   else
     hipLaunchKernelGGL(bn_act_bwd_apply_kernel<false>, grid, dim3(256), 0, stream, c.dz, c.y, nof, c.scale,
                        c.shift, c.mean, c.invstd, c.sums_ws, 1, count, c.training, c.dgamma, c.dbeta, c.dy, nod,
                        c.N, c.C, (int)c.S, (long)c.dz_nstride, (long)c.y_nstride, (long)c.dy_nstride, 0L, 0L,
-                       c.relu, 0);
+                       c.relu ? 1 : 0, 0);
   COCLR_LAUNCH_CHECK();
   return 0;
 }
@@ -927,7 +1103,7 @@
       u.dz = c.dz; u.y = c.y; u.scale = c.scale; u.shift = c.shift; u.mean = c.mean; u.invstd = c.invstd;
       u.dgamma = c.dgamma; u.dbeta = c.dbeta; u.dy = c.dy;
       u.dz_nstride = (long)c.dz_nstride; u.y_nstride = (long)c.y_nstride; u.dy_nstride = (long)c.dy_nstride;
-      u.C = c.C; u.N = c.N; u.S = (int)c.S; u.relu = c.relu; u.training = c.training;
+      u.C = c.C; u.N = c.N; u.S = (int)c.S; u.relu = c.relu ? 1 : 0; u.training = c.training;
       blocks += c.C;
     }
     if (t.n >= 2) {
@@ -954,3 +1130,114 @@
   }
   return 0;
 }
+
+extern "C" int coclr_bn_finalize_apply_large_multi(const coclr_bn_fwd_call* calls, int n, int fold_max_tiles,
+                                                   void* stream_) {
+  hipStream_t stream = (hipStream_t)stream_;
+  if (!calls || n < 1) return COCLR_EINVAL;
+  static const long nt_bytes = bn_nt_bytes();
+  int i = 0;
+  while (i < n) {
+    BnFwdTable fin;
+    BnApplyTable app;
+    fin.n = app.n = 0;
+    long fin_blocks = 0, app_blocks = 0;
+    bool vec0 = false, nt0 = false;
+    int j = i;
+    for (; j < n && j < i + 4; ++j) {
+      const coclr_bn_fwd_call& c = calls[j];
+      if (c.C <= 0 || c.ntiles <= 0 || c.N <= 0 || c.S <= 0 || (c.z && !c.y)) return COCLR_EINVAL;
+      const bool vec = (c.S % 4 == 0) && (c.y_nstride % 4 == 0) && (c.z_nstride % 4 == 0);
+      const bool nt = vec && nt_bytes >= 0 && (long)c.N * c.C * c.S * 4 >= nt_bytes;
+      if (c.z) {
+        if (app.n == 0) { vec0 = vec; nt0 = nt; }
+        else if (vec != vec0 || nt != nt0) break;
+      }
+      BnFwdUnit u;
+      u.sum = c.sum; u.sumsq = c.sumsq; u.gamma = c.gamma; u.beta = c.beta;
+      u.running_mean = c.running_mean; u.running_var = c.running_var; u.nbt = c.num_batches_tracked;
+      u.mean = c.mean; u.invstd = c.invstd; u.scale = c.scale; u.shift = c.shift;
+      u.y = c.y; u.z = c.z; u.count = c.count;
+      u.y_nstride = (long)c.y_nstride; u.z_nstride = (long)c.z_nstride;
+      u.C = c.C; u.ntiles = c.ntiles; u.N = c.N; u.S = (int)c.S; u.relu = c.relu ? 1 : 0;
+      u.momentum = c.momentum; u.eps = c.eps;
+      const bool fold = c.z && c.ntiles <= fold_max_tiles;
+      if (!fold) {
+        fin.u[fin.n++] = u;
+        fin_blocks += c.C;
+      }
+      if (c.z) {
+        const dim3 g = plane_grid(c.N, c.C, (int)c.S);
+        const int k = app.n++;
+        app.u[k] = u;
+        app.gx[k] = (int)g.x; app.gy[k] = (int)g.y; app.fold[k] = fold ? 1 : 0;
+        app_blocks += (long)g.x * g.y;
+      }
+    }
+    if (fin.n) {
+      hipLaunchKernelGGL(bn_finalize_multi_kernel, dim3((unsigned)fin_blocks), dim3(256), 0, stream, fin);
+      COCLR_LAUNCH_CHECK();
+    }
+    if (app.n) {
+      const dim3 grid((unsigned)app_blocks);
+      if (vec0 && nt0)
+        hipLaunchKernelGGL((bn_apply_multi_kernel<true, true>), grid, dim3(256), 0, stream, app);
+      else if (vec0)
+        hipLaunchKernelGGL((bn_apply_multi_kernel<true, false>), grid, dim3(256), 0, stream, app);
+      else
+        hipLaunchKernelGGL((bn_apply_multi_kernel<false, false>), grid, dim3(256), 0, stream, app);
+      COCLR_LAUNCH_CHECK();
+    }
+    i = j;
+  }
+  return 0;
+}
+
+extern "C" int coclr_bn_act_backward_large_multi(const coclr_bn_bwd_call* calls, int n, void* stream_) {
+  hipStream_t stream = (hipStream_t)stream_;
+  if (!calls || n < 1) return COCLR_EINVAL;
+  static const long nt_bytes = bn_nt_bytes();
+  int i = 0;
+  while (i < n) {
+    BnBwdLargeTable t;
+    t.n = 0;
+    long red_blocks = 0, app_blocks = 0;
+    bool vec0 = false;
+    int j = i;
+    for (; j < n && t.n < 4; ++j) {
+      const coclr_bn_bwd_call& c = calls[j];
+      if (c.N <= 0 || c.C <= 0 || c.S <= 0 || !c.dz || !c.y || !c.dy || !c.sums_ws || c.part[0])
+        return COCLR_EINVAL;
+      const bool vec = (c.S % 4 == 0) && (c.dz_nstride % 4 == 0) && (c.y_nstride % 4 == 0) &&
+                       (c.dy_nstride % 4 == 0);
+      if (t.n == 0) vec0 = vec;
+      else if (vec != vec0) break;
+      const int k = t.n++;
+      BnBwdUnit& u = t.u[k];
+      u.dz = c.dz; u.y = c.y; u.scale = c.scale; u.shift = c.shift; u.mean = c.mean; u.invstd = c.invstd;
+      u.dgamma = c.dgamma; u.dbeta = c.dbeta; u.dy = c.dy;
+      u.dz_nstride = (long)c.dz_nstride; u.y_nstride = (long)c.y_nstride; u.dy_nstride = (long)c.dy_nstride;
+      u.C = c.C; u.N = c.N; u.S = (int)c.S; u.training = c.training;
+      u.relu = c.relu ? 1 : 0;
+      if (nt_bytes >= 0 && vec && (long)c.N * c.C * c.S * 4 >= nt_bytes) u.relu |= 2;
+      const dim3 g = plane_grid(c.N, c.C, (int)c.S);
+      t.sums[k] = c.sums_ws;
+      t.groups[k] = reduce_groups(c.N, (int)c.S);
+      t.gx[k] = (int)g.x; t.gy[k] = (int)g.y;
+      red_blocks += (long)c.C * t.groups[k];
+      app_blocks += (long)g.x * g.y;
+    }
+    if (vec0) {
+      hipLaunchKernelGGL(bn_bwd_reduce_multi_kernel<true>, dim3((unsigned)red_blocks), dim3(256), 0, stream, t);
+      COCLR_LAUNCH_CHECK();
+      hipLaunchKernelGGL(bn_bwd_apply_multi_kernel<true>, dim3((unsigned)app_blocks), dim3(256), 0, stream, t);
+    } else {
+      hipLaunchKernelGGL(bn_bwd_reduce_multi_kernel<false>, dim3((unsigned)red_blocks), dim3(256), 0, stream, t);
+      COCLR_LAUNCH_CHECK();
+      hipLaunchKernelGGL(bn_bwd_apply_multi_kernel<false>, dim3((unsigned)app_blocks), dim3(256), 0, stream, t);
+    }
+    COCLR_LAUNCH_CHECK();
+    i = j;
+  }
+  return 0;
+}
diff --git a/coclr_amd/engine.py b/coclr_amd/engine.py
--- a/coclr_amd/engine.py
+++ b/coclr_amd/engine.py
@@ -447,12 +447,16 @@
                          accumulate=c.get("accumulate", False))
         return stats, nt
     if kind == "bn_fwd":
-        if len(c) > 1:
-            ops.bn_finalize_apply_multi(c)
-            return None
         u = c[0]
         gamma, beta, rm, rv, nbt, momentum, eps = u["bn"]
         mean, invstd, scale, shift = u["small"]
+        if len(c) == 1 and u["z"] is None:
+            ops.bn_finalize(u["stats"], u["C"], u["ntiles"], u["count"], gamma, beta, rm, rv, nbt, momentum, eps,
+                            mean, invstd, scale, shift, c0=u.get("c0", 0), c_total=u.get("c_total"))
+            return None
+        if len(c) > 1 or ops.bn_large(u["y"]):
+            ops.bn_finalize_apply_multi(c)
+            return None
         ops.bn_finalize_apply(u["stats"], u["C"], u["ntiles"], u["count"], gamma, beta, rm, rv, nbt, momentum,
                               eps, mean, invstd, scale, shift, u["y"], u["z"], u["relu"], c0=u.get("c0", 0),
                               c_total=u.get("c_total"))
@@ -563,7 +567,7 @@
     return _drive(conv_bn_act_gen(run, x, conv, bn, relu=relu, out=out, residual=residual, n_index=n_index))
 
 
-def conv_bn_act_gen(run, x, conv, bn, relu=True, out=None, residual=None, n_index=None):
+def conv_bn_act_gen(run, x, conv, bn, relu=True, out=None, residual=None, n_index=None, may_defer=True):
     w = conv.weight
     k = tuple(w.shape[2:])
     s, p = _triple(conv.stride), _triple(conv.padding)
@@ -615,15 +619,17 @@
             if training and last:
                 stats, ntiles = res
         count = N * odim[0] * odim[1] * odim[2]
-        lazy = LAZY_APPLY and residual is None and lazy_ok and count > ops.SMALL_CHANNEL
+        lazy = LAZY_APPLY and residual is None and lazy_ok and count > ops.SMALL_CHANNEL and \
+            (may_defer or not ops.BN_MULTI_LARGE)
         if training:
             if bn.momentum is None:
                 raise NotImplementedError("coclr_amd: cumulative-average BatchNorm momentum")
-            if residual is None and not lazy:
+            if residual is None and (not lazy or ops.BN_MULTI_LARGE):
                 yield ("bn_fwd", [dict(stats=stats, C=Cout, ntiles=ntiles, count=count,
                                        bn=(bn.weight, bn.bias, bn.running_mean, bn.running_var,
                                            bn.num_batches_tracked, float(bn.momentum), float(bn.eps)),
-                                       small=(mean, invstd, scale, shift), y=y, z=zv, relu=relu)])
+                                       small=(mean, invstd, scale, shift), y=y, z=None if lazy else zv,
+                                       relu=relu)])
             else:
                 ops.bn_finalize(stats, Cout, ntiles, count, bn.weight, bn.bias,
                                 bn.running_mean, bn.running_var, bn.num_batches_tracked,
@@ -1001,7 +1007,7 @@
             tuple(p.data_ptr() for p in params), tuple(bool(p.requires_grad) for p in params), slots,
             tuple((m.training, m.momentum, m.eps, m.running_mean.data_ptr()) for m in bns),
             tuple(x.stride()), WGRAD_STREAM, DEFER_JOIN, PAIR_UNITS, FUSE_BN_REDUCE, LAZY_APPLY, POOLED_BACKWARD,
-        BATCH_PACK, tuple(id(p) in _SLOTS_VERIFIED for p in params))
+        BATCH_PACK, ops.BN_MULTI_LARGE, tuple(id(p) in _SLOTS_VERIFIED for p in params))
 
 
 def _plan_drop(ent):
@@ -1199,7 +1205,7 @@
 def _infer_signature(module, x, params, bns):
     return (x.dtype, x.device, tuple(p.data_ptr() for p in params),
             tuple((m.momentum, m.eps, m.running_mean.data_ptr(), m.running_var.data_ptr()) for m in bns),
-            PAIR_UNITS, LAZY_APPLY, IN_AFFINE, BATCH_PACK)
+            PAIR_UNITS, LAZY_APPLY, IN_AFFINE, BATCH_PACK, ops.BN_MULTI_LARGE)
 
 
 def _infer_record(ent, module, x):
diff --git a/coclr_amd/ops.py b/coclr_amd/ops.py
--- a/coclr_amd/ops.py
+++ b/coclr_amd/ops.py
@@ -412,7 +412,28 @@
         _chk5(z, "z"), int(relu), _stream()), "bn_finalize_apply")
 
 
+def bn_large(y):
+    N, _, T, H, W = y.shape
+    return BN_MULTI_LARGE and N * T * H * W > SMALL_CHANNEL
+
+
+def _runs(units):
+    runs = []
+    for u in units:
+        large = bn_large(u["y"]) and not u.get("partials")
+        if runs and runs[-1][0] == large:
+            runs[-1][1].append(u)
+        else:
+            runs.append((large, [u]))
+    return runs
+
+
 def bn_finalize_apply_multi(units):
+    for large, run in _runs(units):
+        _bn_finalize_apply_multi(run, large)
+
+
+def _bn_finalize_apply_multi(units, large):
     n = len(units)
     arr = (BnFwdCall * n)()
     for a, u in zip(arr, units):
@@ -429,16 +450,27 @@
         a.gamma, a.beta, a.running_mean, a.running_var = _p(gamma), _p(beta), _p(rm), _p(rv)
         a.num_batches_tracked = _p(nbt, torch.int64)
         a.mean, a.invstd, a.scale, a.shift = _p(mean), _p(invstd), _p(scale), _p(shift)
+        if z is None and not large:
+            raise ValueError("coclr_amd: a BatchNorm unit without an output takes the large-map launches")
         a.y, a.z = _p(y), _p(z)
         a.count = float(u["count"])
         a.S = T * H * W
-        a.y_nstride, a.z_nstride = _chk5(y, "y"), _chk5(z, "z")
+        a.y_nstride, a.z_nstride = _chk5(y, "y"), _chk5(z, "z") if z is not None else 0
         a.C, a.ntiles, a.N, a.relu = C_, ntiles, N, int(u["relu"])
         a.momentum, a.eps = momentum, eps
-    _lib.check(_L().coclr_bn_finalize_apply_multi(arr, n, _stream()), "bn_finalize_apply_multi")
+    if large:
+        _lib.check(_L().coclr_bn_finalize_apply_large_multi(arr, n, BN_FOLD_TILES, _stream()),
+                   "bn_finalize_apply_large_multi")
+    else:
+        _lib.check(_L().coclr_bn_finalize_apply_multi(arr, n, _stream()), "bn_finalize_apply_multi")
 
 
 def bn_act_backward_multi(units):
+    for large, run in _runs(units):
+        _bn_act_backward_multi(run, large)
+
+
+def _bn_act_backward_multi(units, large):
     n = len(units)
     arr = (BnBwdCall * n)()
     for a, u in zip(arr, units):
@@ -462,10 +494,15 @@
                     raise ValueError("coclr_amd: partial sums do not match the unit's channels")
                 a.part[i] = _p(st)
                 a.part_ntiles[i] = nt
-    _lib.check(_L().coclr_bn_act_backward_multi(arr, n, _stream()), "bn_act_backward_multi")
-
-
-SMALL_CHANNEL = 32768
+    if large:
+        _lib.check(_L().coclr_bn_act_backward_large_multi(arr, n, _stream()), "bn_act_backward_large_multi")
+    else:
+        _lib.check(_L().coclr_bn_act_backward_multi(arr, n, _stream()), "bn_act_backward_multi")
+
+
+SMALL_CHANNEL = int(os.environ.get("COCLR_BN_SMALL_CHANNEL", "32768"))
+BN_MULTI_LARGE = os.environ.get("COCLR_BN_MULTI_LARGE", "1") != "0"
+BN_FOLD_TILES = int(os.environ.get("COCLR_BN_FOLD_TILES", "256"))
 
 
 def bn_eval_affine(gamma, beta, running_mean, running_var, eps, C_, mean, invstd, scale, shift):
diff --git a/include/coclr_hip.h b/include/coclr_hip.h
--- a/include/coclr_hip.h
+++ b/include/coclr_hip.h
@@ -157,6 +157,9 @@
 int coclr_bn_finalize_apply_multi(const coclr_bn_fwd_call* calls, int n, void* stream);
 int coclr_bn_act_backward_multi(const coclr_bn_bwd_call* calls, int n, void* stream);
 
+int coclr_bn_finalize_apply_large_multi(const coclr_bn_fwd_call* calls, int n, int fold_max_tiles, void* stream);
+int coclr_bn_act_backward_large_multi(const coclr_bn_bwd_call* calls, int n, void* stream);
+
 int coclr_bn_act_backward_pooled(const coclr_pool_desc* d, const float* pool_dy,
                                  const int32_t* pool_idx, const float* y, const float* scale,
                                  const float* shift, const float* mean, const float* invstd,
```

Result: no change. 1168, median of 3 (+0.1%).
